# SheffieldML/GPy

Hardware: AMD Instinct MI355X
Metric: exact-GP log_lik+grad iters/sec (higher is better)
Workload: dtype f64; 1 GPU; BASELINE configs[2]: matern52 ARD exact GP, one GPRegression.parameters_changed, N=16384 D=32 Dy=1 per GPU; N=16384, D=32, kernel=matern52, ARD=True, parallelism=replicas x1

## Files before the change

gpy_amd/_lib.py:

```python
import ctypes
import os
import subprocess

import numpy as np
from numpy.ctypeslib import ndpointer

_HERE = os.path.dirname(os.path.abspath(__file__))
LIB_PATH = os.environ.get("MI355GP_LIB") or os.path.join(_HERE, "libmi355gp.so")
CSRC = os.path.join(_HERE, "csrc")

KIND_IDS = {"rbf": 0, "matern52": 1, "matern32": 2, "exponential": 3, "white": 4, "bias": 5, "ratquad": 6, "stdperiodic": 7,
            "coregionalize": 8, "linear": 9, "mlp": 10, "poly": 11}


def ard_id(kind, ARD):
    if kind == "coregionalize":
        return int(ARD)
    return int(ARD) & 3 if kind == "stdperiodic" else int(bool(ARD))


class Part(ctypes.Structure):
    _fields_ = [("kind", ctypes.c_int), ("ard", ctypes.c_int), ("n_active", ctypes.c_int),
                ("active_dims", ctypes.POINTER(ctypes.c_int)), ("theta", ctypes.POINTER(ctypes.c_double)),
                ("term", ctypes.c_int)]


def make_parts(specs):
    arr = (Part * len(specs))()
    keep, ntheta = [], 0
    for i, spec in enumerate(specs):
        kind, ARD, theta, dims = spec[:4]
        arr[i].term = int(spec[4]) if len(spec) > 4 else 0
        th = np.ascontiguousarray(theta, dtype=np.float64)
        keep.append(th)
        arr[i].kind = KIND_IDS[kind]
        arr[i].ard = ard_id(kind, ARD)
        arr[i].theta = th.ctypes.data_as(ctypes.POINTER(ctypes.c_double))
        if dims is None:
            arr[i].n_active = 0
            arr[i].active_dims = None
        else:
            d = np.ascontiguousarray(dims, dtype=np.int32)
            keep.append(d)
            arr[i].n_active = d.size
            arr[i].active_dims = d.ctypes.data_as(ctypes.POINTER(ctypes.c_int))
        ntheta += th.size
    return arr, keep, ntheta
FETCH_L, FETCH_KINV, FETCH_DLDK, FETCH_K = 0, 1, 2, 3
EP_BERNOULLI_PROBIT = 0
OUT_LML, OUT_LOGDET, OUT_DATAFIT, OUT_DNOISE, OUT_TRKINV, NUM_OUT = 0, 1, 2, 3, 4, 8
STAGE_NAMES = ("kbuild", "potrf", "trtri", "lauum", "solve", "grad", "total")
NUM_T = 8
PROFILE_FAMILIES = ("update_nt", "trtri", "lauum", "diag128", "trsm128", "update_nt64", "potrf_persist", "trtri_early")

_lib = None


class MI355GPError(RuntimeError):
    pass


DIAG_LIB_PATH = os.path.join(_HERE, "libmi355gp_diag.so")


def build(force=False):
    srcs = [os.path.join(CSRC, f) for f in os.listdir(CSRC) if f.endswith((".hip", ".h")) or f == "Makefile"]
    srcs.append(os.path.join(_HERE, "..", "include", "mi355gp.h"))
    srcs.append(os.path.join(_HERE, "..", "include", "mi355gp_debug.h"))
    product = os.path.join(_HERE, "libmi355gp.so")
    if not force and os.path.exists(product) and os.path.exists(DIAG_LIB_PATH):
        t = min(os.path.getmtime(product), os.path.getmtime(DIAG_LIB_PATH))
        if all(os.path.getmtime(s) <= t for s in srcs if os.path.exists(s)):
            return product
    r = subprocess.run(["make", "-C", CSRC, "-j8", "all", "diag"], capture_output=True, text=True)
    if r.returncode != 0 or not os.path.exists(product) or not os.path.exists(DIAG_LIB_PATH):
        raise MI355GPError("building libmi355gp.so failed:\n" + r.stdout[-4000:] + r.stderr[-4000:])
    return product


_dp = ndpointer(dtype=np.float64, flags="C_CONTIGUOUS")
_c_dp = ctypes.POINTER(ctypes.c_double)


def _opt(a):
    return None if a is None else a.ctypes.data_as(_c_dp)


def lib():
    global _lib
    if _lib is not None:
        return _lib
    if not os.path.exists(LIB_PATH):
        build()
    L = ctypes.CDLL(LIB_PATH)
    i64, ci, cd, vp = ctypes.c_int64, ctypes.c_int, ctypes.c_double, ctypes.c_void_p
    L.mi355gp_last_error.restype = ctypes.c_char_p
    L.mi355gp_version.restype = ctypes.c_char_p
    L.mi355gp_device_count.argtypes = [ctypes.POINTER(ci)]
    L.mi355gp_device_synchronize.argtypes = [ci]
    L.mi355gp_create.argtypes = [ci, ctypes.POINTER(vp)]
    L.mi355gp_destroy.argtypes = [vp]
    L.mi355gp_set_data.argtypes = [vp, _dp, i64, ci, _dp, ci]
    L.mi355gp_set_targets.argtypes = [vp, _dp, ci]
    L.mi355gp_kern_K.argtypes = [ci, ci, ci, _dp, _dp, i64, _c_dp, i64, ci, _dp]
    L.mi355gp_kern_Kdiag.argtypes = [ci, _dp, i64, _dp]
    L.mi355gp_update_gradients_full.argtypes = [ci, ci, ci, _dp, _dp, _dp, i64, _c_dp, i64, ci, _dp]
    L.mi355gp_gradients_X.argtypes = [ci, ci, ci, _dp, _dp, _dp, i64, _c_dp, i64, ci, _dp]
    L.mi355gp_exact_inference.argtypes = [vp, ci, ci, _dp, _dp, i64, cd, cd, _dp, _c_dp, _c_dp, _c_dp, _c_dp]
    L.mi355gp_exact_inference_sum.argtypes = [vp, ci, ctypes.POINTER(Part), _dp, i64, cd, cd, _dp, _c_dp, _c_dp, _c_dp,
                                              _c_dp]
    L.mi355gp_exact_studentt_sum.argtypes = [vp, ci, ctypes.POINTER(Part), cd, cd, cd, _dp, _c_dp, _c_dp, _c_dp]
    L.mi355gp_covariance_between_points.argtypes = [vp, ci, ctypes.POINTER(Part), _dp, i64, _dp, i64, _dp]
    L.mi355gp_predictive_gradients_sum.argtypes = [vp, ci, ctypes.POINTER(Part), _dp, i64, _c_dp, _c_dp]
    L.mi355gp_predict_sum.argtypes = [vp, ci, ctypes.POINTER(Part), _dp, i64, _c_dp, _c_dp, ci]
    L.mi355gp_laplace_begin.argtypes = [vp, ci, ctypes.POINTER(Part)]
    L.mi355gp_laplace_newton.argtypes = [vp, _dp, _dp, cd, _dp, _dp, _c_dp]
    L.mi355gp_laplace_finish.argtypes = [vp, _dp, cd, _dp, _c_dp]
    L.mi355gp_laplace_gradients.argtypes = [vp, _dp, _dp, _dp]
    L.mi355gp_laplace_implicit.argtypes = [vp, _dp, _dp]
    L.mi355gp_laplace_predict.argtypes = [vp, ci, ctypes.POINTER(Part), _dp, i64, _dp, _c_dp, _c_dp, ci]
    L.mi355gp_ep_recompute.argtypes = [vp, _dp, _dp, cd, cd, ci, _dp, _dp, _c_dp, _c_dp]
    L.mi355gp_ep_sweep.argtypes = [vp, ci, ndpointer(dtype=np.int64, flags="C_CONTIGUOUS"), _dp, cd, cd, _dp, _dp, _dp, _dp, _dp, _dp,
                                   _dp, _c_dp]
    L.mi355gp_inference_given_K.argtypes = [vp, _dp, _dp, i64, cd, cd, _dp, _c_dp, _c_dp, _c_dp]
    L.mi355gp_fetch.argtypes = [vp, ci, _dp, ci]
    L.mi355gp_predict.argtypes = [vp, ci, ci, _dp, _dp, i64, _c_dp, _c_dp, ci]
    L.mi355gp_potrf.argtypes = [ci, _dp, i64, _c_dp]
    L.mi355gp_pdinv.argtypes = [ci, _dp, i64, _c_dp, _c_dp, _c_dp, _c_dp]
    L.mi355gp_pdinv_full.argtypes = [ci, _dp, i64, _c_dp, _c_dp, _c_dp, _c_dp, _c_dp]
    L.mi355gp_set_option.argtypes = [vp, ci, ci]
    L.mi355gp_get_option.argtypes = [vp, ci, ctypes.POINTER(ci)]
    L.mi355gp_sparse_get_profile.argtypes = [vp, _dp]
    L.mi355gp_dbg_comm_selftest.argtypes = [ci, ctypes.c_char_p, ci, ci, ci, ci, i64, ci, _dp]
    L.mi355gp_dbg_comm_selftest.restype = ci
    L.mi355gp_bench_factor.argtypes = [ci, i64, ci, _c_dp, _c_dp, _c_dp]
    L.mi355gp_bench_factor.restype = ci
    L.mi355gp_get_profile.argtypes = [vp, _dp, _dp, ndpointer(dtype=np.int32, flags="C_CONTIGUOUS")]
    L.mi355gp_grid_unique_id.argtypes = [ctypes.c_char_p]
    L.mi355gp_grid_create.argtypes = [ci, ci, ci, ci, ci, ci, ctypes.c_char_p, ctypes.POINTER(vp)]
    L.mi355gp_grid_destroy.argtypes = [vp]
    L.mi355gp_grid_set_data.argtypes = [vp, _dp, i64, ci, _dp, ci]
    L.mi355gp_grid_exact_inference.argtypes = [vp, ci, ci, _dp, _dp, i64, cd, cd, _dp, _c_dp, _c_dp, _c_dp, _c_dp]
    L.mi355gp_grid_fetch.argtypes = [vp, ci, _dp]
    L.mi355gp_grid_set_option.argtypes = [vp, ci, ci]
    L.mi355gp_grid_coll_log.argtypes = [vp, ci, _dp]
    L.mi355gp_grid_coll_log.restype = ci
    L.mi355gp_dbg_grid_multi.argtypes = [ci, ci, ci, ci, _dp]
    L.mi355gp_dbg_update_nt.argtypes = [ci, ci, ctypes.POINTER(ci), ci, ci, _dp]
    L.mi355gp_dbg_update_rect.argtypes = [ci, ci, ci, ctypes.POINTER(ci), ci, ci, _dp]
    L.mi355gp_grid_get_option.argtypes = [vp, ci, ctypes.POINTER(ci)]
    L.mi355gp_sparse_create.argtypes = [ci, ctypes.POINTER(vp)]
    L.mi355gp_sparse_destroy.argtypes = [vp]
    L.mi355gp_sparse_set_data.argtypes = [vp, _dp, i64, ci, _dp, ci]
    L.mi355gp_vardtc_inference.argtypes = [vp, ci, ci, _dp, _dp, i64, cd, cd, _dp, _c_dp, _c_dp, _c_dp, _c_dp]
    L.mi355gp_sparse_fetch.argtypes = [vp, ci, _dp]
    L.mi355gp_vardtc_inference_sum.argtypes = [vp, ci, ctypes.POINTER(Part), _dp, i64, _dp, i64, cd, _dp, _c_dp, _c_dp, _c_dp,
                                               _c_dp, _c_dp, _c_dp]
    L.mi355gp_sparse_set_input_variance.argtypes = [vp, _dp, i64, ci]
    L.mi355gp_vardtc_inference_uncertain.argtypes = [vp, ci, ctypes.POINTER(Part), _dp, i64, _dp, i64, cd, _dp, _c_dp, _c_dp,
                                                     _c_dp, _c_dp, _c_dp, _c_dp]
    L.mi355gp_sparse_predict.argtypes = [vp, ci, ctypes.POINTER(Part), _dp, i64, _c_dp, _c_dp, ci]
    L.mi355gp_sparse_fetch_dLdKnm.argtypes = [vp, i64, i64, _dp]
    L.mi355gp_sparse_attach_loopback.argtypes = [vp, ci, ci, ci]
    L.mi355gp_sparse_attach_comm.argtypes = [vp, ci, ci, ctypes.c_char_p]
    L.mi355gp_rbf_psi.argtypes = [ci, cd, _dp, ci, _dp, i64, _dp, _dp, i64, ci, _c_dp, _c_dp, _c_dp]
    L.mi355gp_rbf_psi_grad.argtypes = [ci, cd, _dp, ci, _dp, i64, _dp, _dp, i64, ci, _c_dp, _c_dp, _c_dp, _c_dp, _dp, _dp, _dp,
                                       _dp, _dp]
    L.mi355gp_dbg_mfma.argtypes = [ci, _dp, _dp, _dp]
    L.mi355gp_dbg_gemm.argtypes = [ci, ci, ci, i64, i64, i64, _dp, _dp, _dp, cd, cd, ci, _c_dp]
    L.mi355gp_dbg_peaks.argtypes = [ci, _dp]
    L.mi355gp_dbg_pipe_share.argtypes = [ci, _dp]
    L.mi355gp_dbg_graph_factor.argtypes = [ci, i64, ci, _dp]
    L.mi355gp_dbg_gemm_clock.argtypes = [_c_dp, _c_dp]
    L.mi355gp_dbg_mask_probe.argtypes = [ci, ci, ci, _dp]
    L.mi355gp_dbg_lauum_plan.argtypes = [ci, ctypes.POINTER(ci), ci, ctypes.POINTER(ci)]
    L.mi355gp_dbg_lauum_plan.restype = ci
    L.mi355gp_dbg_persist_owners.argtypes = [ci, ci, ci, ctypes.POINTER(ci), ctypes.POINTER(ci)]
    L.mi355gp_dbg_persist_owners.restype = ci
    L.mi355gp_dbg_persist.argtypes = [ci, i64, ci, ci, _dp]
    L.mi355gp_dbg_ipc_selftest.argtypes = [ctypes.c_char_p, ci, ci, ci, ci, i64, _dp]
    for name in ("device_count", "create", "destroy", "set_data", "set_targets", "kern_K", "kern_Kdiag",
                 "update_gradients_full", "exact_inference", "inference_given_K", "fetch", "predict", "potrf",
                 "pdinv", "dbg_mfma", "dbg_gemm", "dbg_peaks", "set_option", "get_profile", "grid_unique_id",
                 "grid_create", "grid_destroy", "grid_set_data", "grid_exact_inference", "grid_fetch", "grid_set_option",
                 "grid_get_option", "sparse_create",
                 "sparse_destroy", "sparse_set_data", "vardtc_inference", "sparse_fetch", "gradients_X", "sparse_attach_comm", "exact_inference_sum",
                 "predict_sum", "dbg_gemm_clock", "covariance_between_points", "exact_studentt_sum", "dbg_mask_probe",
                 "vardtc_inference_sum", "sparse_predict", "sparse_fetch_dLdKnm", "sparse_attach_loopback",
                 "predictive_gradients_sum", "dbg_pipe_share", "pdinv_full", "dbg_graph_factor", "get_option",
                 "sparse_get_profile", "dbg_persist", "dbg_grid_multi", "dbg_update_nt", "dbg_update_rect",
                 "dbg_ipc_selftest", "laplace_begin", "laplace_newton", "laplace_finish", "laplace_gradients",
                 "laplace_implicit", "laplace_predict", "ep_recompute", "ep_sweep", "rbf_psi", "rbf_psi_grad",
                 "sparse_set_input_variance", "vardtc_inference_uncertain"):
        getattr(L, "mi355gp_" + name).restype = ci
    _lib = L
    return L


EXPORTED = ("mi355gp_last_error", "mi355gp_version", "mi355gp_device_count", "mi355gp_device_synchronize", "mi355gp_create", "mi355gp_destroy",
            "mi355gp_set_data", "mi355gp_set_targets", "mi355gp_kern_K", "mi355gp_kern_Kdiag",
            "mi355gp_update_gradients_full", "mi355gp_exact_inference", "mi355gp_inference_given_K",
            "mi355gp_fetch", "mi355gp_predict", "mi355gp_potrf", "mi355gp_pdinv", "mi355gp_bench_factor",
            "mi355gp_set_option", "mi355gp_get_profile", "mi355gp_grid_unique_id", "mi355gp_grid_create",
            "mi355gp_grid_destroy", "mi355gp_grid_set_data", "mi355gp_grid_exact_inference", "mi355gp_grid_fetch",
            "mi355gp_grid_set_option", "mi355gp_grid_get_option",
            "mi355gp_sparse_create", "mi355gp_sparse_destroy", "mi355gp_sparse_set_data", "mi355gp_vardtc_inference",
            "mi355gp_sparse_fetch", "mi355gp_gradients_X", "mi355gp_sparse_attach_comm",
            "mi355gp_exact_inference_sum", "mi355gp_predict_sum", "mi355gp_dbg_gemm_clock",
            "mi355gp_covariance_between_points", "mi355gp_exact_studentt_sum", "mi355gp_vardtc_inference_sum",
            "mi355gp_sparse_predict", "mi355gp_sparse_fetch_dLdKnm", "mi355gp_sparse_attach_loopback",
            "mi355gp_predictive_gradients_sum", "mi355gp_dbg_pipe_share", "mi355gp_pdinv_full", "mi355gp_dbg_graph_factor",
            "mi355gp_dbg_mfma", "mi355gp_dbg_gemm", "mi355gp_dbg_peaks", "mi355gp_dbg_mask_probe", "mi355gp_get_option",
            "mi355gp_sparse_get_profile", "mi355gp_dbg_persist", "mi355gp_dbg_grid_multi", "mi355gp_dbg_update_nt", "mi355gp_dbg_update_rect",
            "mi355gp_dbg_ipc_selftest", "mi355gp_grid_coll_log", "mi355gp_dbg_lauum_plan", "mi355gp_dbg_persist_owners",
            "mi355gp_laplace_begin", "mi355gp_laplace_newton", "mi355gp_laplace_finish", "mi355gp_laplace_gradients",
            "mi355gp_laplace_implicit", "mi355gp_laplace_predict", "mi355gp_ep_recompute", "mi355gp_ep_sweep",
            "mi355gp_rbf_psi", "mi355gp_rbf_psi_grad", "mi355gp_sparse_set_input_variance",
            "mi355gp_vardtc_inference_uncertain")


OPTIONS = {"profile": 0, "lookahead": 1, "tri_overlap": 2, "tri_min_nt": 3, "tri_h": 4, "tri_wgs": 5, "tri_half": 6,
           "part1_on_panel": 7, "nbo": 8, "solve_overlap": 9, "diag_excl_first": 10, "graph": 11, "persist": 12, "agg2": 13,
           "persist_test": 14, "persist_aborts": 15, "persist_skip": 16, "persist_sched": 17}


def last_error():
    return lib().mi355gp_last_error().decode()


def check(rc, what):
    if rc < 0:
        raise MI355GPError("%s failed (rc=%d): %s" % (what, rc, last_error()))
    return rc


def device_count():
    n = ctypes.c_int(0)
    lib().mi355gp_device_count(ctypes.byref(n))
    return n.value


def device_synchronize(device=0):
    require_device(device)
    check(lib().mi355gp_device_synchronize(int(device)), "mi355gp_device_synchronize")


def require_device(device=0):
    n = device_count()
    if device >= n:
        raise MI355GPError("no MI355X visible to HIP (device %d requested, %d present): the gpy_amd backend has "
                           "no CPU fallback" % (device, n))


def f64(a):
    return np.ascontiguousarray(a, dtype=np.float64)


def theta_vec(variance, lengthscale, ARD, D):
    ls = np.atleast_1d(np.asarray(lengthscale, dtype=np.float64)).ravel()
    if ARD:
        if ls.size == 1:
            ls = np.full(D, ls[0])
        assert ls.size == D, "ARD kernel needs one lengthscale per input dimension"
    else:
        assert ls.size == 1, "isotropic kernel has a single lengthscale"
    return np.concatenate([[float(np.asarray(variance).ravel()[0])], ls])


def _exact_result(out, ms, **arrays):
    res = dict(lml=out[OUT_LML], logdet=out[OUT_LOGDET], datafit=out[OUT_DATAFIT], dnoise=out[OUT_DNOISE],
               trKinv=out[OUT_TRKINV], **arrays)
    if ms is not None:
        res["stage_ms"] = dict(zip(STAGE_NAMES, ms[:len(STAGE_NAMES)]))
    return res


def _predict(entry, head, Xnew, D, Dy, full_cov, want_var, between=()):
    Xnew = f64(Xnew)
    M = Xnew.shape[0]
    assert Xnew.shape[1] == D
    mu = np.empty((M, Dy))
    var = (np.empty((M, M)) if full_cov else np.empty(M)) if want_var else None
    check(getattr(lib(), entry)(*(tuple(head) + (Xnew, M) + tuple(between) + (mu.ctypes.data_as(_c_dp), _opt(var),
                                                                              int(bool(full_cov))))), entry)
    if var is not None and not full_cov:
        var = var[:, None]
    return mu, var


class Context(object):

    def __init__(self, device=0):
        require_device(device)
        self._h = ctypes.c_void_p()
        check(lib().mi355gp_create(device, ctypes.byref(self._h)), "mi355gp_create")
        self.device = device
        self.N = self.D = self.Dy = 0

    def close(self):
        if getattr(self, "_h", None) is not None and self._h.value:
            lib().mi355gp_destroy(self._h)
            self._h = ctypes.c_void_p()

    def __del__(self):
        try:
            self.close()
        except Exception:
            pass

    def set_data(self, X, R):
        X, R = f64(X), f64(R)
        assert X.ndim == 2 and R.ndim == 2 and X.shape[0] == R.shape[0]
        self.N, self.D = X.shape
        self.Dy = R.shape[1]
        check(lib().mi355gp_set_data(self._h, X, self.N, self.D, R, self.Dy), "mi355gp_set_data")

    def set_targets(self, R):
        R = f64(R)
        check(lib().mi355gp_set_targets(self._h, R, R.shape[1]), "mi355gp_set_targets")

    def _exact(self, entry, head, ntheta, noise, jitter, extra_jitter, want_alpha, want_diag, want_stage_ms):
        noise = f64(np.atleast_1d(noise))
        out = np.zeros(NUM_OUT)
        alpha = np.empty((self.N, self.Dy)) if want_alpha else None
        dtheta = np.zeros(ntheta)
        diag = np.empty(self.N) if want_diag else None
        ms = np.zeros(NUM_T) if want_stage_ms else None
        rc = check(getattr(lib(), entry)(self._h, *(tuple(head) + (noise, noise.size, jitter, extra_jitter, out, _opt(alpha),
                                                                   _opt(dtheta), _opt(diag), _opt(ms)))), entry)
        return rc, _exact_result(out, ms, alpha=alpha, dtheta=dtheta, diag_dL_dK=diag)

    def exact_inference(self, kind, ARD, theta, noise, jitter=1e-8, extra_jitter=0.0, want_alpha=True,
                        want_diag=False, want_stage_ms=False):
        theta = f64(theta)
        return self._exact("mi355gp_exact_inference", (KIND_IDS[kind], ard_id(kind, ARD), theta), theta.size, noise, jitter,
                           extra_jitter, want_alpha, want_diag, want_stage_ms)

    def exact_inference_sum(self, specs, noise, jitter=1e-8, extra_jitter=0.0, want_alpha=True, want_diag=False,
                            want_stage_ms=False):
        arr, keep, ntheta = make_parts(specs)
        return self._exact("mi355gp_exact_inference_sum", (len(specs), arr), ntheta, noise, jitter, extra_jitter, want_alpha,
                           want_diag, want_stage_ms)

    def predict_sum(self, specs, Xnew, full_cov=False, want_var=True):
        arr, keep, _ = make_parts(specs)
        return _predict("mi355gp_predict_sum", (self._h, len(specs), arr), Xnew, self.D, self.Dy, full_cov, want_var)

    def exact_studentt_sum(self, specs, nu, jitter=1e-8, extra_jitter=0.0):
        arr, keep, ntheta = make_parts(specs)
        out = np.zeros(NUM_OUT)
        alpha = np.empty((self.N, self.Dy))
        dtheta = np.zeros(ntheta)
        rc = check(lib().mi355gp_exact_studentt_sum(self._h, len(specs), arr, float(nu), jitter, extra_jitter, out,
                                                    _opt(alpha), _opt(dtheta), None), "mi355gp_exact_studentt_sum")
        return rc, dict(lml=out[OUT_LML], logdet=out[OUT_LOGDET], beta=out[OUT_DATAFIT], scale=out[5], alpha=alpha,
                        dtheta=dtheta)

    def predictive_gradients(self, specs, Xnew, want_var=True):
        arr, keep, _ = make_parts(specs)
        Xnew = f64(Xnew)
        M = Xnew.shape[0]
        assert Xnew.shape[1] == self.D
        dmu = np.empty((M, self.D, self.Dy))
        dvar = np.empty((M, self.D)) if want_var else None
        check(lib().mi355gp_predictive_gradients_sum(self._h, len(specs), arr, Xnew, M, dmu.ctypes.data_as(_c_dp), _opt(dvar)),
              "mi355gp_predictive_gradients_sum")
        return dmu, dvar

    def covariance_between_points(self, specs, X1, X2):
        arr, keep, _ = make_parts(specs)
        X1, X2 = f64(X1), f64(X2)
        out = np.empty((X1.shape[0], X2.shape[0]))
        check(lib().mi355gp_covariance_between_points(self._h, len(specs), arr, X1, X1.shape[0], X2, X2.shape[0], out),
              "mi355gp_covariance_between_points")
        return out

# ... 254 lines not shown
    if X2 is None:
        M, p2 = N, None
    else:
        X2 = f64(X2)
        M, p2 = X2.shape[0], X2.ctypes.data_as(_c_dp)
    G = f64(dL_dK)
    assert G.shape == (N, M), "dL_dK must be N x M"
    theta = f64(theta)
    out = np.zeros(theta.size)
    check(lib().mi355gp_update_gradients_full(device, KIND_IDS[kind], ard_id(kind, ARD), theta, G, X, N, p2, M, D, out),
          "mi355gp_update_gradients_full")
    return out


def gradients_X(kind, ARD, theta, dL_dK, X, X2=None, device=0):
    require_device(device)
    X = f64(X)
    N, D = X.shape
    if X2 is None:
        M, p2 = N, None
    else:
        X2 = f64(X2)
        M, p2 = X2.shape[0], X2.ctypes.data_as(_c_dp)
    G = f64(dL_dK)
    assert G.shape == (N, M), "dL_dK must be N x M"
    out = np.zeros((N, D))
    check(lib().mi355gp_gradients_X(device, KIND_IDS[kind], ard_id(kind, ARD), f64(theta), G, X, N, p2, M, D, out),
          "mi355gp_gradients_X")
    return out


def _psi_args(variance, lengthscale, ARD, Z, mu, S, weights):
    Z, mu, S = f64(Z), f64(mu), f64(S)
    N, D = mu.shape
    assert S.shape == mu.shape and Z.ndim == 2 and Z.shape[1] == D, "Z is M x D, mu and S are N x D"
    ls = theta_vec(variance, lengthscale, ARD, D)[1:]
    w = None if weights is None else f64(np.ravel(weights))
    assert w is None or w.size == N
    return (float(np.ravel(variance)[0]), f64(ls), int(bool(ARD)), Z, Z.shape[0], mu, S, N, D, _opt(w)), w


def rbf_psi(variance, lengthscale, ARD, Z, mu, S, weights=None, want_psi1=True, want_psi2=True, device=0):
    require_device(device)
    args, keep = _psi_args(variance, lengthscale, ARD, Z, mu, S, weights)
    M, N = args[4], args[7]
    p1 = np.empty((N, M)) if want_psi1 else None
    p2 = np.empty((M, M)) if want_psi2 else None
    check(lib().mi355gp_rbf_psi(device, *(args + (_opt(p1), _opt(p2)))), "mi355gp_rbf_psi")
    return p1, p2


def rbf_psi_grad(variance, lengthscale, ARD, Z, mu, S, dL_dpsi0=None, dL_dpsi1=None, dL_dpsi2=None, weights=None, device=0):
    require_device(device)
    args, keep = _psi_args(variance, lengthscale, ARD, Z, mu, S, weights)
    M, N, D = args[4], args[7], args[8]
    d0 = None if dL_dpsi0 is None else f64(np.ravel(dL_dpsi0))
    d1 = None if dL_dpsi1 is None else f64(dL_dpsi1)
    d2 = None if dL_dpsi2 is None else f64(dL_dpsi2)
    assert d0 is None or d0.size == N
    assert d1 is None or d1.shape == (N, M), "dL_dpsi1 must be N x M"
    assert d2 is None or d2.shape == (M, M), "dL_dpsi2 must be M x M"
    dvar, dl = np.zeros(1), np.zeros(D if ARD else 1)
    dZ, dmu, dS = np.zeros((M, D)), np.zeros((N, D)), np.zeros((N, D))
    check(lib().mi355gp_rbf_psi_grad(device, *(args + (_opt(d0), _opt(d1), _opt(d2), dvar, dl, dZ, dmu, dS))),
          "mi355gp_rbf_psi_grad")
    return dvar[0], dl, dZ, dmu, dS


def potrf(A, device=0):
    require_device(device)
    L = f64(A).copy()
    ms = ctypes.c_double(0.0)
    info = check(lib().mi355gp_potrf(device, L, L.shape[0], ctypes.byref(ms)), "mi355gp_potrf")
    return L, info, ms.value


def pdinv(A, device=0):
    require_device(device)
    A = f64(A)
    n = A.shape[0]
    Ai, L = np.empty((n, n)), np.empty((n, n))
    ld, ms = ctypes.c_double(0.0), ctypes.c_double(0.0)
    info = check(lib().mi355gp_pdinv(device, A, n, Ai.ctypes.data_as(_c_dp), L.ctypes.data_as(_c_dp),
                                     ctypes.byref(ld), ctypes.byref(ms)), "mi355gp_pdinv")
    return Ai, L, ld.value, info, ms.value


def pdinv_full(A, device=0):
    require_device(device)
    A = f64(A)
    n = A.shape[0]
    Ai, L, Li = np.empty((n, n)), np.empty((n, n)), np.empty((n, n))
    ld, ms = ctypes.c_double(0.0), ctypes.c_double(0.0)
    info = check(lib().mi355gp_pdinv_full(device, A, n, Ai.ctypes.data_as(_c_dp), L.ctypes.data_as(_c_dp),
                                          Li.ctypes.data_as(_c_dp), ctypes.byref(ld), ctypes.byref(ms)), "mi355gp_pdinv_full")
    return Ai, L, Li, ld.value, info


def bench_factor(N, reps=3, device=0):
    require_device(device)
    p, t, l = ctypes.c_double(0.0), ctypes.c_double(0.0), ctypes.c_double(0.0)
    check(lib().mi355gp_bench_factor(device, N, reps, ctypes.byref(p), ctypes.byref(t), ctypes.byref(l)),
          "mi355gp_bench_factor")
    fl = float(N) ** 3 / 3.0
    return {"potrf_ms": p.value, "trtri_ms": t.value, "lauum_ms": l.value,
            "potrf_tflops": fl / p.value / 1e9, "trtri_tflops": fl / t.value / 1e9, "lauum_tflops": fl / l.value / 1e9}


def dbg_persist(N, reps=3, kcap=0, device=0):
    require_device(device)
    nt = (int(N) + 127) // 128
    out = np.zeros(8 + 32 * nt)
    check(lib().mi355gp_dbg_persist(device, int(N), int(reps), int(kcap), out), "mi355gp_dbg_persist")
    st = out[8:8 + 8 * nt].reshape(nt, 8)
    near = out[8 + 8 * nt:8 + 20 * nt].reshape(nt, 3, 4)
    far = out[8 + 20 * nt:].reshape(nt, 12)
    return dict(ms_steps=out[0], ms_persist=out[1], mismatches=int(out[2]), info=int(out[3]), abort=int(out[4]), nt=nt,
                steps=(st - st[0, 0]) / 100.0, near=(near - st[0, 0]) / 100.0, far=(far - st[0, 0]) / 100.0)


def dbg_mask_probe(pct=75, order=0, device=0):
    require_device(device)
    out = np.zeros(3)
    check(lib().mi355gp_dbg_mask_probe(device, pct, order, out), "mi355gp_dbg_mask_probe")
    return out


def dbg_mfma(a, b, device=0):
    require_device(device)
    d = np.zeros(256)
    check(lib().mi355gp_dbg_mfma(device, f64(a), f64(b), d), "dbg_mfma")
    return d.reshape(64, 4)


def dbg_gemm(A, B, C, a_mcontig, b_ncontig, alpha=1.0, beta=0.0, reps=0, device=0):
    require_device(device)
    A, B, C = f64(A), f64(B), f64(C).copy()
    M, K = (A.shape[1], A.shape[0]) if a_mcontig else A.shape
    N = B.shape[1] if b_ncontig else B.shape[0]
    ms = ctypes.c_double(0.0)
    check(lib().mi355gp_dbg_gemm(device, int(a_mcontig), int(b_ncontig), M, N, K, A, B, C, alpha, beta, reps,
                                 ctypes.byref(ms)), "dbg_gemm")
    return C, ms.value


def dbg_gemm_clock():
    mhz, cyc = ctypes.c_double(0.0), ctypes.c_double(0.0)
    check(lib().mi355gp_dbg_gemm_clock(ctypes.byref(mhz), ctypes.byref(cyc)), "dbg_gemm_clock")
    return mhz.value, cyc.value


def dbg_peaks(device=0):
    require_device(device)
    out = np.zeros(8)
    check(lib().mi355gp_dbg_peaks(device, out), "dbg_peaks")
    return dict(mfma_f64_tflops=out[0], valu_f64_tflops=out[1], hbm_copy_gbs=out[2], hbm_fill_gbs=out[3],
                mfma_cycles_per_inst_1wave=out[4], shader_mhz_under_load=out[5], mfma_1wave_tflops=out[6],
                mfma_cycles_per_inst_loaded=out[7])


def dbg_grid_multi(T, nb=512, reps=3, device=0):
    require_device(device)
    out = np.zeros(5)
    check(lib().mi355gp_dbg_grid_multi(device, int(T), int(nb), int(reps), out), "mi355gp_dbg_grid_multi")
    return out


def dbg_update_nt(nt, ks, reps=5, device=0):
    require_device(device)
    ka = (ctypes.c_int * len(ks))(*[int(k) for k in ks])
    out = np.zeros(len(ks))
    check(lib().mi355gp_dbg_update_nt(device, int(nt), ka, len(ks), int(reps), out), "mi355gp_dbg_update_nt")
    return out


def dbg_update_rect(ntr, ntc, ks, reps=5, device=0):
    require_device(device)
    ka = (ctypes.c_int * len(ks))(*[int(k) for k in ks])
    out = np.zeros(len(ks))
    check(lib().mi355gp_dbg_update_rect(device, int(ntr), int(ntc), ka, len(ks), int(reps), out), "mi355gp_dbg_update_rect")
    return out


def persist_owners(nt, nw, tune=0):
    owner = (ctypes.c_int * (nt * nt))()
    out4 = (ctypes.c_int * 4)()
    dup = lib().mi355gp_dbg_persist_owners(nt, nw, tune, owner, out4)
    return np.frombuffer(owner, dtype=np.int32, count=nt * nt).reshape(nt, nt).copy(), out4[0], out4[1], out4[2], out4[3], dup


def lauum_plan(nt):
    out4 = (ctypes.c_int * 4)()
    lib().mi355gp_dbg_lauum_plan(nt, None, 0, out4)
    n = out4[0]
    buf = (ctypes.c_int * (6 * max(n, 1)))()
    check(lib().mi355gp_dbg_lauum_plan(nt, buf, n, out4), "mi355gp_dbg_lauum_plan")
    return np.frombuffer(buf, dtype=np.int32, count=6 * n).reshape(n, 6).copy(), out4[1], out4[2], out4[3]
```

gpy_amd/csrc/api.hip:

```cpp
#include <functional>
#include <algorithm>
#include <cmath>
#include <cstdarg>
#include <cstdio>
#include <climits>
#include <cstring>
#include <string>
#include <vector>

#include "../../include/mi355gp.h"
#include "../../include/mi355gp_debug.h"
#include "internal.h"
#include "parts.h"

int run_peaks(int device, double* out4);

static thread_local std::string g_err;

void mi355gp_set_error(const char* fmt, ...) {
    char buf[1024];
    va_list ap;
    va_start(ap, fmt);
    vsnprintf(buf, sizeof(buf), fmt, ap);
    va_end(ap);
    g_err = buf;
}

#define LOG_2_PI 1.8378770664093454836

#include "ctx.h"

static void apply_options(mi355gp_ctx* c) {
    FactorWs& w = c->ws;
    auto set = [&](int o, int* field) { if (c->opt[o] != INT_MIN) *field = c->opt[o]; };
    set(MI355GP_OPT_LOOKAHEAD, &w.lookahead);
    set(MI355GP_OPT_TRI_OVERLAP, &w.tri_overlap);
    set(MI355GP_OPT_TRI_MIN_NT, &w.tri_min_nt);
    set(MI355GP_OPT_TRI_H, &w.tri_h_override);
    set(MI355GP_OPT_TRI_WGS, &w.tri_wgs);
    set(MI355GP_OPT_TRI_HALF, &w.tri_half_ok);
    set(MI355GP_OPT_PART1_ON_PANEL, &w.part1_on_panel);
    set(MI355GP_OPT_NBO, &w.nbo_override);
    set(MI355GP_OPT_SOLVE_OVERLAP, &w.solve_overlap);
    set(MI355GP_OPT_DIAG_EXCL_FIRST, &w.diag_excl_first);
    set(MI355GP_OPT_PERSIST, &w.persist);
    set(MI355GP_OPT_AGG2, &w.agg2);
    if (c->opt[MI355GP_OPT_GRAPH] != INT_MIN) c->graph_enabled = c->opt[MI355GP_OPT_GRAPH] ? 1 : 0;
}

static void drop_graph(mi355gp_ctx* c) {
    if (c->fgraph) (void)hipGraphExecDestroy(c->fgraph);
    c->fgraph = nullptr;
    c->fgraph_calls = 0;
}

static void free_data(mi355gp_ctx* c) {
    drop_graph(c);
    c->parts.clear();
    double** ptrs[] = {&c->dX, &c->dR, &c->dNoise, &c->A, &c->B, &c->C, &c->Mbuf,
                       &c->dTmp, &c->dTrmvPart, &c->dGradPart, &c->dGradOut, &c->dPack, &c->dCoregPart};
    for (auto p : ptrs) {
        if (*p) (void)hipFree(*p);
        *p = nullptr;
    }
    if (c->hPack) (void)hipHostFree(c->hPack);
    c->hPack = nullptr;
    c->dAlpha = c->dScal = c->dDiag = c->dGradOutAll = nullptr;
    c->hIdx.clear();
    c->hIdxCol = -1;
    laplace_session_free(c->lap);
    c->lap = nullptr;
    c->lap_stage = 0;
    factor_ws_free(&c->ws);
    c->have_factor = c->have_kernel = false;
}

extern "C" {

const char* mi355gp_last_error(void) { return g_err.c_str(); }
const char* mi355gp_version(void) { return "mi355gp 0.1 (gfx950)"; }

int mi355gp_device_synchronize(int device) {
    HIP_CHECK(hipSetDevice(device));
    HIP_CHECK(hipDeviceSynchronize());
    return 0;
}

int mi355gp_device_count(int* count) {
    int n = 0;
    hipError_t e = hipGetDeviceCount(&n);
    if (e != hipSuccess) {
        (void)hipGetLastError();
        n = 0;
    }
    *count = n;
    return 0;
}

int mi355gp_create(int device, mi355gp_ctx** out) {
    int n = 0;
    mi355gp_device_count(&n);
    if (device < 0 || device >= n) {
        mi355gp_set_error("mi355gp_create: device %d not available (%d HIP devices visible)", device, n);
        return -2;
    }
    HIP_CHECK(hipSetDevice(device));
    mi355gp_ctx* c = new mi355gp_ctx();
    c->device = device;
    for (int& o : c->opt) o = INT_MIN;
    if (factor_engine(device, &c->st, nullptr, nullptr) != 0) return -2;
    for (auto& e : c->ev) HIP_CHECK(hipEventCreate(&e));
    {
        const char* e = PRODUCT_ENV("GRAPH");
        if (e && *e) c->graph_enabled = atoi(e) ? 1 : 0;
    }
    *out = c;
    return 0;
}

int mi355gp_destroy(mi355gp_ctx* c) {
    if (!c) return 0;
    (void)hipSetDevice(c->device);
    (void)hipStreamSynchronize(c->st);
    free_data(c);
    for (auto& e : c->ev)
        if (e) (void)hipEventDestroy(e);
    if (c->st) (void)hipStreamSynchronize(c->st);
    delete c;
    return 0;
}

int mi355gp_set_data(mi355gp_ctx* c, const double* X, int64_t N, int D, const double* R, int Dy) {
    ARG_CHECK(c && X && R && N > 0 && D > 0 && Dy > 0, "mi355gp_set_data: bad arguments");
    HIP_CHECK(hipSetDevice(c->device));
    EngineShared gate(c->device);
    HIP_CHECK(hipStreamSynchronize(c->st));
    free_data(c);
    c->n = N;
    c->npad = round_up(N, NB);
    c->D = D;
    c->Dy = Dy;
    const long np = c->npad;
    HIP_CHECK(hipMalloc(&c->dX, sizeof(double) * N * D));
    HIP_CHECK(hipMalloc(&c->dR, sizeof(double) * N * Dy));
    HIP_CHECK(hipMalloc(&c->dNoise, sizeof(double) * N));
    HIP_CHECK(hipMalloc(&c->A, sizeof(double) * np * np));
    HIP_CHECK(hipMalloc(&c->B, sizeof(double) * np * np));
    HIP_CHECK(hipMalloc(&c->C, sizeof(double) * np * np));
    if (factor_ws_alloc(&c->ws, np) != 0) return -3;
    c->ws.can_calibrate = 1;
    {
        const int lookahead = c->ws.lookahead;
        const char* e = PRODUCT_ENV("GRAPH");
        c->graph_enabled = (e && *e) ? (atoi(e) ? 1 : 0) : 1;
        apply_options(c);
        if (c->opt[MI355GP_OPT_LOOKAHEAD] == INT_MIN) c->ws.lookahead = lookahead;
    }
    HIP_CHECK(hipMalloc(&c->dTmp, sizeof(double) * N * Dy));
    const long nchunks = (N + trmv_chunk_rows(N) - 1) / trmv_chunk_rows(N);
    HIP_CHECK(hipMalloc(&c->dTrmvPart, sizeof(double) * nchunks * N * Dy));
    const int groups = (D + 31) / 32;
    c->gradPartDoubles = 2L * groups * 2048 * GP_STRIDE;
    HIP_CHECK(hipMalloc(&c->dGradPart, sizeof(double) * c->gradPartDoubles));
    HIP_CHECK(hipMalloc(&c->dGradOut, sizeof(double) * groups * GP_STRIDE));
    c->offGrad = 8;
    c->offExt = c->offGrad + (size_t)16 * groups * GP_STRIDE;
    c->offAlpha = c->offExt + (size_t)16 * groups * GP_STRIDE;
    c->offDiag = c->offAlpha + (size_t)N * Dy;
    c->offCoreg = c->offDiag + (size_t)N;
    c->packDoubles = c->offCoreg + (size_t)16 * COREG_REC;
    HIP_CHECK(hipMalloc(&c->dPack, sizeof(double) * c->packDoubles));
    HIP_CHECK(hipHostMalloc(&c->hPack, sizeof(double) * c->packDoubles, hipHostMallocDefault));
    c->dScal = c->dPack;
    c->dGradOutAll = c->dPack + c->offGrad;
    c->dAlpha = c->dPack + c->offAlpha;
    c->dDiag = c->dPack + c->offDiag;
    HIP_CHECK(hipMemcpy(c->dX, X, sizeof(double) * N * D, hipMemcpyHostToDevice));
    HIP_CHECK(hipMemcpy(c->dR, R, sizeof(double) * N * Dy, hipMemcpyHostToDevice));
    return 0;
}

int mi355gp_set_targets(mi355gp_ctx* c, const double* R, int Dy) {
    ARG_CHECK(c && R && c->n > 0 && Dy == c->Dy, "mi355gp_set_targets: set_data first / Dy mismatch");
    HIP_CHECK(hipSetDevice(c->device));
    EngineShared gate(c->device);
    HIP_CHECK(hipStreamSynchronize(c->st));
    HIP_CHECK(hipMemcpy(c->dR, R, sizeof(double) * c->n * Dy, hipMemcpyHostToDevice));
    return 0;
}

}

static int run_pipeline(mi355gp_ctx* c, EngineShared* gate, bool with_kernel_grads, double* out_scalars, double* alpha_out,
                        double* dtheta_out, double* diag_out, double* stage_ms,
                        const std::function<int()>& rebuild, double studentt_nu = 0.0, int attempt = 0) {
    hipStream_t st = c->st;
    const long n = c->n, np = c->npad;
    c->lap_stage = 0;
    c->ws.prof.reset();
// ... 754 lines not shown
    HIP_CHECK(dPart.alloc(2 * 2048 * GP_STRIDE * ((D + 31) / 32)));
    HIP_CHECK(dCol.alloc(64 * mp * (D + 1)));
    HIP_CHECK(dHX.alloc(mp * (D + 1)));
    if (dvar_out) {
        HIP_CHECK(hipMemsetAsync(dU, 0, sizeof(double) * np * mp, st));
        emit_cross(st, c->parts, c->terms, training_points(c), xs, dU, mp, nullptr, true, 0);
        launch_trmm_lower(st, c->B, np, dU, mp, dT, mp, (int)(np / NB), (int)(mp / NB));
        launch_trmm_lower_T(st, c->B, np, dT, mp, dU, mp, (int)(np / NB), (int)(mp / NB));
    }
    const size_t hx = (size_t)M * (D + 1);
    std::vector<double> HX(hx);
    const int npass = (dmu_out ? (int)Dy : 0) + (dvar_out ? 1 : 0);
    if (dmu_out) std::fill(dmu_out, dmu_out + (size_t)M * D * Dy, 0.0);
    if (dvar_out) std::fill(dvar_out, dvar_out + (size_t)M * D, 0.0);
    for (int pass = 0; pass < npass; ++pass) {
        const bool is_var = dvar_out && pass == npass - 1;
        const double* W = dU;
        if (!is_var) {
            const long cnt = n * M;
            hipLaunchKernelGGL(k_fill_rows, dim3((unsigned)((cnt + 255) / 256)), dim3(256), 0, st, (double*)dG, mp, n, (long)M,
                               c->dAlpha + pass, (int)Dy);
            W = dG;
        }
        auto add = [&](long m, int q, double g) {
            if (is_var) dvar_out[m * D + q] += -2.0 * g;
            else dmu_out[((size_t)m * D + q) * Dy + pass] += g;
        };
        for (size_t pi = 0; pi < c->parts.size(); ++pi) {
            const mi355gp_ctx::Part& pt = c->parts[pi];
            if (pt.is_static()) continue;
            if (pt.linear()) {
                const int ns = launch_colreduce_multi(st, W, mp, n, M, pt.dXt, 1, np, (int)D, 0, dCol);
                launch_sum_splits(st, dCol, (long)M * D, ns, 0, dHX);
                HIP_CHECK(hipMemcpyAsync(HX.data(), dHX, sizeof(double) * M * D, hipMemcpyDeviceToHost, st));
                HIP_CHECK(hipStreamSynchronize(st));
                gradx_linear(pt.inv_ls, M, (int)D, HX.data(), add);
                if (is_var)
                    for (long m = 0; m < M; ++m)
                        for (size_t a = 0; a < pt.dims.size(); ++a)
                            dvar_out[m * D + pt.dims[a]] += 2.0 * pt.theta[pt.kp.ard ? a : 0] * Xnew[m * D + pt.dims[a]];
                continue;
            }
            const double* xt = xs.points(st, pt);
            if (pt.kp.kind == MI355GP_STDPERIODIC) {
                launch_periodic_gradx(st, pt.kp, xt, xs.ld, M, pt.dXt, np, n, W, mp, 1, dHX);
                HIP_CHECK(hipMemcpyAsync(HX.data(), dHX, sizeof(double) * M * D, hipMemcpyDeviceToHost, st));
                HIP_CHECK(hipStreamSynchronize(st));
                gradx_periodic(pt.pw, M, (int)D, HX.data(), add);
                continue;
            }
            launch_grad_generic(st, pt.kp, pt.dXt, np, n, xt, xs.ld, M, 0, W, mp, dPart, GP_STRIDE, dH, mp);
            const int ns = launch_colreduce_multi(st, dH, mp, n, M, pt.dXt, 1, np, (int)D, 1, dCol);
            launch_sum_splits(st, dCol, (long)hx, ns, 0, dHX);
            HIP_CHECK(hipMemcpyAsync(HX.data(), dHX, sizeof(double) * hx, hipMemcpyDeviceToHost, st));
            HIP_CHECK(hipStreamSynchronize(st));
            if (pt.mlp()) {
                gradx_mlp(Xnew, M, (int)D, pt.inv_ls, pt.kp.bias, HX.data(), add);
                if (is_var)
                    for (long m = 0; m < M; ++m) {
                        const double cd = mlp_dkdiag_factor(pt, Xnew + m * D);
                        for (size_t a = 0; a < pt.dims.size(); ++a)
                            dvar_out[m * D + pt.dims[a]] += 2.0 * cd * pt.theta[1 + (pt.kp.ard ? a : 0)] * Xnew[m * D + pt.dims[a]];
                    }
                continue;
            }
            gradx_stationary(Xnew, M, (int)D, pt.inv_ls, HX.data(), add);
        }
    }
    HIP_CHECK(hipStreamSynchronize(st));
    HIP_CHECK(hipGetLastError());
    return 0;
}

int mi355gp_covariance_between_points(mi355gp_ctx* c, int nparts, const mi355gp_part* parts, const double* X1,
                                      int64_t M1, const double* X2, int64_t M2, double* out) {
    ARG_CHECK(c && c->n > 0 && c->have_factor, "mi355gp_covariance_between_points: run an inference call first");
    ARG_CHECK(X1 && X2 && M1 > 0 && M2 > 0 && out, "mi355gp_covariance_between_points: bad arguments");
    HIP_CHECK(hipSetDevice(c->device));
    EngineShared gate(c->device);
    if (int rc = prepare_parts(c, nparts, parts)) return rc;
    if (int rc = coreg_check_points(c, X1, M1, "X1")) return rc;
    if (int rc = coreg_check_points(c, X2, M2, "X2")) return rc;
    hipStream_t st = c->st;
    const long np = c->npad, m1p = round_up(M1, NB), m2p = round_up(M2, NB);
    c->have_kernel = true;
    scale_parts(c);
    PointSet x1, x2;
    DevBuf dK1, dK2, dT1, dT2, dC;
    if (int rc = x1.load(st, X1, M1, c->D)) return rc;
    if (int rc = x2.load(st, X2, M2, c->D)) return rc;
    HIP_CHECK(dK1.alloc(np * m1p));
    HIP_CHECK(dK2.alloc(np * m2p));
    HIP_CHECK(dT1.alloc(np * m1p));
    HIP_CHECK(dT2.alloc(np * m2p));
    HIP_CHECK(dC.alloc(m1p * m2p));
    HIP_CHECK(hipMemsetAsync(dK1, 0, sizeof(double) * np * m1p, st));
    HIP_CHECK(hipMemsetAsync(dK2, 0, sizeof(double) * np * m2p, st));
    HIP_CHECK(hipMemsetAsync(dC, 0, sizeof(double) * m1p * m2p, st));
    DevBuf dS1, dS2, dS3;
    if (has_product(c->terms)) {
        HIP_CHECK(dS1.alloc(np * m1p));
        HIP_CHECK(dS2.alloc(np * m2p));
        HIP_CHECK(dS3.alloc(m1p * m2p));
    }
    emit_cross(st, c->parts, c->terms, training_points(c), x1, dK1, m1p, dS1, true, 0);
    emit_cross(st, c->parts, c->terms, training_points(c), x2, dK2, m2p, dS2, true, 0);
    emit_cross(st, c->parts, c->terms, x1, x2, dC, m2p, dS3, true, 0);
    launch_trmm_lower(st, c->B, np, dK1, m1p, dT1, m1p, (int)(np / NB), (int)(m1p / NB));
    launch_trmm_lower(st, c->B, np, dK2, m2p, dT2, m2p, (int)(np / NB), (int)(m2p / NB));
    launch_gemm(st, 1, 1, m1p, m2p, np, dT1, m1p, dT2, m2p, dC, m2p, -1.0, 1.0);
    HIP_CHECK(hipMemcpy2DAsync(out, sizeof(double) * M2, dC, sizeof(double) * m2p, sizeof(double) * M2, M1,
                               hipMemcpyDeviceToHost, st));
    HIP_CHECK(hipStreamSynchronize(st));
    HIP_CHECK(hipGetLastError());
    return 0;
}

int mi355gp_predict(mi355gp_ctx* c, int kind, int ard, const double* theta, const double* Xnew, int64_t M,
                    double* mu_out, double* var_out, int full_cov) {
    if (int rc = check_kind(kind, KS_STATIONARY | KS_EXT | KS_LINEAR | KS_DOT, "mi355gp_predict")) return rc;
    const mi355gp_part part{kind, ard, 0, nullptr, theta};
    return mi355gp_predict_sum(c, 1, &part, Xnew, M, mu_out, var_out, full_cov);
}

int mi355gp_set_option(mi355gp_ctx* c, int option, int value) {
    ARG_CHECK(c != nullptr, "mi355gp_set_option: NULL context");
    if (option == MI355GP_OPT_PROFILE) {
        c->ws.prof.on = (value != 0);
        c->ws.prof.mask = (value == 1) ? 0xffu : (unsigned)value >> 1;
        return 0;
    }
    if (option == MI355GP_OPT_PERSIST_TEST) {
#ifndef MI355GP_DIAG
        if (value != 0) {
            mi355gp_set_error("mi355gp_set_option: MI355GP_OPT_PERSIST_TEST is a test hook of the diagnostics build (libmi355gp_diag.so)");
            return -1;
        }
#endif
        c->ws.persist_test = value;
        if (value) c->ws.persist_skip = 0;
        drop_graph(c);
        return 0;
    }
    if (option < 0 || option >= MI355GP_OPT_NUM || option == MI355GP_OPT_PERSIST_ABORTS || option == MI355GP_OPT_PERSIST_SKIP ||
        option == MI355GP_OPT_PERSIST_SCHED) {
        mi355gp_set_error("mi355gp_set_option: unknown or read-only option %d", option);
        return -1;
    }
    if (option == MI355GP_OPT_LOOKAHEAD) value = (value == 0) ? 0 : 1;
    if (option == MI355GP_OPT_NBO && value > 0 && value % NB != 0) {
        mi355gp_set_error("mi355gp_set_option: NBO must be a multiple of %d", NB);
        return -1;
    }
    c->opt[option] = (value < 0) ? INT_MIN : value;
    if (value < 0) {
        FactorWs d;
#define env(name, dflt) diag_env_int(DIAG_ENV(name), dflt)
#define penv(name, dflt) diag_env_int(PRODUCT_ENV(name), dflt)
        switch (option) {
            case MI355GP_OPT_LOOKAHEAD: c->ws.lookahead = d.lookahead; break;
            case MI355GP_OPT_TRI_OVERLAP: c->ws.tri_overlap = penv("TRI_OVERLAP", d.tri_overlap) ? 1 : 0; break;
            case MI355GP_OPT_TRI_MIN_NT: c->ws.tri_min_nt = env("TRI_MIN_NT", d.tri_min_nt); break;
            case MI355GP_OPT_TRI_H: c->ws.tri_h_override = env("TRI_H", d.tri_h_override); break;
            case MI355GP_OPT_TRI_WGS: c->ws.tri_wgs = env("TRI_WGS", d.tri_wgs); break;
            case MI355GP_OPT_TRI_HALF: c->ws.tri_half_ok = env("TRI_HALF", d.tri_half_ok) ? 1 : 0; break;
            case MI355GP_OPT_PART1_ON_PANEL: c->ws.part1_on_panel = env("PART1_ON_PANEL", d.part1_on_panel) ? 1 : 0; break;
            case MI355GP_OPT_NBO: c->ws.nbo_override = env("NBO", d.nbo_override); break;
            case MI355GP_OPT_SOLVE_OVERLAP: c->ws.solve_overlap = env("SOLVE_OVERLAP", d.solve_overlap) ? 1 : 0; break;
            case MI355GP_OPT_DIAG_EXCL_FIRST: c->ws.diag_excl_first = env("DIAG_EXCL_FIRST", d.diag_excl_first) ? 1 : 0; break;
            case MI355GP_OPT_PERSIST: c->ws.persist = penv("PERSIST", d.persist); break;
            case MI355GP_OPT_AGG2: c->ws.agg2 = env("AGG2", d.agg2) ? 1 : 0; break;
            case MI355GP_OPT_GRAPH: c->graph_enabled = penv("GRAPH", 1) ? 1 : 0; break;
            default: break;
        }
#undef env
#undef penv
    }
    if (option == MI355GP_OPT_PERSIST) {
        c->ws.persist_auto_off = 0;
        c->ws.sched_force_steps = 0;
        c->ws.sched_np = c->ws.sched_ns = 0;
        c->ws.sched_state = (value < 0) ? 0 : 2;
    }
    apply_options(c);
    drop_graph(c);
    return 0;
}

int mi355gp_get_option(mi355gp_ctx* c, int option, int* value) {
    ARG_CHECK(c && value && option > MI355GP_OPT_PROFILE && option < MI355GP_OPT_NUM, "mi355gp_get_option: bad arguments");
    const FactorWs& w = c->ws;
    const int v[MI355GP_OPT_NUM] = {0, w.lookahead, w.tri_overlap, w.tri_min_nt, w.tri_h_override, w.tri_wgs, w.tri_half_ok,
                                    w.part1_on_panel, w.nbo_override, w.solve_overlap, w.diag_excl_first, c->graph_enabled,
                                    w.persist, w.agg2, w.persist_test, w.persist_aborts, w.persist_skip,
                                    w.sched_state == 2 ? ((w.persist_auto_off || !w.persist) ? 2 : 1) : 0};
    *value = v[option];
    return 0;
}

int mi355gp_get_profile(mi355gp_ctx* c, double* ms, double* flops, int* launches) {
    ARG_CHECK(c && ms && flops && launches, "mi355gp_get_profile: NULL argument");
    HIP_CHECK(hipSetDevice(c->device));
    HIP_CHECK(hipStreamSynchronize(c->st));
    if (c->ws.st_panel) HIP_CHECK(hipStreamSynchronize(c->ws.st_panel));
    if (c->ws.prof.collect(ms, flops, launches) != 0) {
        mi355gp_set_error("mi355gp_get_profile: event timing failed");
        return -5;
    }
    return 0;
}

int mi355gp_bench_factor(int device, int64_t N, int reps, double* ms_potrf, double* ms_trtri, double* ms_lauum) {
    ARG_CHECK(N >= NB && reps >= 1 && ms_potrf && ms_trtri && ms_lauum, "mi355gp_bench_factor: N >= 128, reps >= 1");
    HIP_CHECK(hipSetDevice(device));
    const long np = round_up(N, NB);
    const int D = 4;
    std::vector<double> X((size_t)N * D);
    unsigned long long state = 0x9E3779B97F4A7C15ull;
    for (double& v : X) {
        state = state * 6364136223846793005ull + 1442695040888963407ull;
        v = ((double)(state >> 11) / 9007199254740992.0 - 0.5) * 4.0;
    }
    DevBuf dX, dXt, dIl, dNoise, A, B, C;
    HIP_CHECK(dX.alloc(N * D));
    HIP_CHECK(dXt.alloc(D * np));
    HIP_CHECK(dIl.alloc(D));
    HIP_CHECK(dNoise.alloc(1));
    HIP_CHECK(A.alloc(np * np));
    HIP_CHECK(B.alloc(np * np));
    HIP_CHECK(C.alloc(np * np));
    const double il[4] = {0.7, 0.7, 0.7, 0.7}, noise = 0.1;
    HIP_CHECK(hipMemcpy(dX, X.data(), sizeof(double) * N * D, hipMemcpyHostToDevice));
    HIP_CHECK(hipMemcpy(dIl, il, sizeof(il), hipMemcpyHostToDevice));
    HIP_CHECK(hipMemcpy(dNoise, &noise, sizeof(double), hipMemcpyHostToDevice));
    hipStream_t st;
    if (factor_engine(device, &st, nullptr, nullptr) != 0) return -2;
    FactorWs ws;
    if (factor_ws_alloc(&ws, np) != 0) return -3;
    ws.scratchX = B;
    ws.scratchT = C;
    hipEvent_t e[4];
    for (auto& ev : e) HIP_CHECK(hipEventCreate(&ev));
    const KernParams kp{MI355GP_RBF, 0, D, 1.0};
    launch_scale_inputs(st, dX, N, D, dIl, 0, dXt, np);
    double acc[3] = {0.0, 0.0, 0.0};
    int info = 0, first_info = 0, redone = 0;
    for (int r = -1; r < reps; ++r) {
        launch_kbuild_sym(st, kp, dXt, np, N, np, A, dNoise, 1, 1e-8, 1, 1);
        HIP_CHECK(hipEventRecord(e[0], st));
        potrf_device(st, A, np, &ws);
        HIP_CHECK(hipEventRecord(e[1], st));
        trtri_device(st, A, B, C, np, &ws);
        HIP_CHECK(hipEventRecord(e[2], st));
        lauum_device(st, B, C, np, &ws);
        HIP_CHECK(hipEventRecord(e[3], st));
        HIP_CHECK(hipStreamSynchronize(st));
        HIP_CHECK(hipMemcpy(&info, ws.info, sizeof(int), hipMemcpyDeviceToHost));
        bool clean = false;
        if (potrf_persist_aborted(info, &ws, &clean)) {
            if (++redone > reps + 2) {
                mi355gp_set_error("mi355gp_bench_factor: the persistent launch kept being called off");
                for (auto& ev : e) (void)hipEventDestroy(ev);
                factor_ws_free(&ws);
                return -6;
            }
            --r;
            continue;
        }
        if (info > 0 && first_info == 0) first_info = info;
        if (r < 0) continue;
        for (int i = 0; i < 3; ++i) {
            float ms;
            HIP_CHECK(hipEventElapsedTime(&ms, e[i], e[i + 1]));
            acc[i] += ms;
        }
    }
    info = first_info;
    *ms_potrf = acc[0] / reps;
    *ms_trtri = acc[1] / reps;
    *ms_lauum = acc[2] / reps;
    for (auto& ev : e) (void)hipEventDestroy(ev);
    factor_ws_free(&ws);
    HIP_CHECK(hipGetLastError());
    return info > 0 ? info : 0;
}

__global__ void k_count_lower_mismatch(const double* __restrict__ a, const double* __restrict__ b, long n, long ld,
                                       unsigned long long* __restrict__ count) {
    unsigned long long c = 0;
    for (long idx = (long)blockIdx.x * blockDim.x + threadIdx.x; idx < n * n; idx += (long)gridDim.x * blockDim.x) {
        const long i = idx / n, j = idx - i * n;
        if (j <= i && __double_as_longlong(a[i * ld + j]) != __double_as_longlong(b[i * ld + j])) ++c;
    }
    if (c) atomicAdd(count, c);
}

int mi355gp_dbg_persist(int device, int64_t N, int reps, int kcap, double* out) {
    ARG_CHECK(N >= 2 * NB && reps >= 1 && out, "mi355gp_dbg_persist: N >= 256, reps >= 1");
    HIP_CHECK(hipSetDevice(device));
    const long np = round_up(N, NB);
    const int nt = (int)(np / NB), D = 4;
    std::vector<double> X((size_t)N * D);
    unsigned long long state = 0x9E3779B97F4A7C15ull;
    for (double& v : X) {
        state = state * 6364136223846793005ull + 1442695040888963407ull;
        v = ((double)(state >> 11) / 9007199254740992.0 - 0.5) * 4.0;
    }
    DevBuf dX, dXt, dIl, dNoise, A, B, dStamp, dCount;
    HIP_CHECK(dX.alloc(N * D));
    HIP_CHECK(dXt.alloc(D * np));
    HIP_CHECK(dIl.alloc(D));
    HIP_CHECK(dNoise.alloc(1));
    HIP_CHECK(A.alloc(np * np));
    HIP_CHECK(B.alloc(np * np));
    HIP_CHECK(dStamp.alloc(32 * nt));
    HIP_CHECK(dCount.alloc(1));
    const double il[4] = {0.7, 0.7, 0.7, 0.7}, noise = 0.1;
    HIP_CHECK(hipMemcpy(dX, X.data(), sizeof(double) * N * D, hipMemcpyHostToDevice));
    HIP_CHECK(hipMemcpy(dIl, il, sizeof(il), hipMemcpyHostToDevice));
    HIP_CHECK(hipMemcpy(dNoise, &noise, sizeof(double), hipMemcpyHostToDevice));
    HIP_CHECK(hipMemset(dStamp, 0, sizeof(double) * 32 * nt));
    HIP_CHECK(hipMemset(dCount, 0, sizeof(double)));
    hipStream_t st;
    if (factor_engine(device, &st, nullptr, nullptr) != 0) return -2;
    EngineShared gate(device);
    FactorWs ws;
    if (factor_ws_alloc(&ws, np) != 0) return -3;
    ws.tri_overlap = 0;
    if (kcap > 0) ws.persist_kcap = kcap;
    ws.persist_max_nt = 64;
    hipEvent_t e[2];
    ws.persist = 1;
    for (auto& ev : e) HIP_CHECK(hipEventCreate(&ev));
    const KernParams kp{MI355GP_RBF, 0, D, 1.0};
    launch_scale_inputs(st, dX, N, D, dIl, 0, dXt, np);
    for (int i = 0; i < 8 + 32 * nt; ++i) out[i] = 0.0;
    int info[4] = {0, 0, 0, 0};
    for (int mode = 0; mode < 2; ++mode) {
        double* M = mode == 0 ? (double*)B : (double*)A;
        ws.persist = mode;
        if (mode == 1 && !potrf_persist_eligible(np, &ws)) {
            mi355gp_set_error("mi355gp_dbg_persist: N = %ld is not eligible for the persistent factorisation", (long)N);
            for (auto& ev : e) (void)hipEventDestroy(ev);
            factor_ws_free(&ws);
            return -1;
        }
        double acc = 0.0;
        for (int r = -1; r < reps; ++r) {
// ... 284 lines not shown
```

gpy_amd/csrc/common.h:

```cpp
#pragma once
#include <hip/hip_runtime.h>
#include <stdint.h>

typedef double d4 __attribute__((ext_vector_type(4)));
typedef double d2 __attribute__((ext_vector_type(2)));

#define NB 128
#define NBO 512
#define FACTOR_NBO_SMALL_N 0
#define FACTOR_NBO_SMALL 256
#define FACTOR_DEFAULT_TRI_OVERLAP 1
#define FACTOR_DEFAULT_PERSIST 1
#define FACTOR_PERSIST_MAX_NT 64
#define PS_ABORT_INFO (1 << 30)
#define PS_ABORT_CLEAN ((1 << 30) + 1)
#define PS_SKIP_AFTER_CLEAN 16
#define FACTOR_DEFAULT_DIAG_EXCL_FIRST 1
#define GEMM_DEFAULT_TRI64_MAX 512
#define GEMM_DEFAULT_LAUUM64_MAX 528
#define LAUUM_SPLIT_MAX_NT 44
#define GEMM_DEFAULT_UPD64_MAX 128

__device__ __forceinline__ d4 mfma_f64(double a, double b, d4 c) {
    return __builtin_amdgcn_mfma_f64_16x16x4f64(a, b, c, 0, 0, 0);
}

void mi355gp_set_error(const char* fmt, ...);
#define HIP_CHECK(expr)                                                                          \
    do {                                                                                         \
        hipError_t _e = (expr);                                                                  \
        if (_e != hipSuccess) {                                                                  \
            mi355gp_set_error("%s failed: %s (%s:%d)", #expr, hipGetErrorString(_e), __FILE__,  \
                              __LINE__);                                                         \
            return -(1000 + (int)_e);                                                            \
        }                                                                                        \
    } while (0)
#define ARG_CHECK(cond, msg)              \
    do {                                  \
        if (!(cond)) {                    \
            mi355gp_set_error("%s", msg); \
            return -1;                    \
        }                                 \
    } while (0)

struct DevBuf {
    double* p = nullptr;
    DevBuf() = default;
    DevBuf(DevBuf&& o) noexcept : p(o.p) { o.p = nullptr; }
    DevBuf(const DevBuf&) = delete;
    DevBuf& operator=(const DevBuf&) = delete;
    ~DevBuf() {
        if (p) (void)hipFree(p);
    }
    hipError_t alloc(size_t doubles) { return hipMalloc(&p, sizeof(double) * (doubles ? doubles : 1)); }
    operator double*() const { return p; }
};

static inline int64_t round_up(int64_t n, int64_t m) { return (n + m - 1) / m * m; }

#include <cstdlib>
#define PRODUCT_ENV(name) getenv("MI355GP_" name)
#ifdef MI355GP_DIAG
#define DIAG_ENV(name) getenv("MI355GP_" name)
#else
#define DIAG_ENV(name) ((const char*)nullptr)
#endif
static inline int diag_env_int(const char* v, int dflt) { return (v && *v) ? atoi(v) : dflt; }
```

gpy_amd/csrc/factor.hip:

```cpp
#include <cstdlib>
#include <mutex>
#include <vector>

#include "internal.h"

void KernelProf::begin(hipStream_t st, int fam, double flops) {
    open = on && ((mask >> fam) & 1u);
    if (!open) return;
    const size_t e0 = 2 * recs.size();
    while (pool.size() < e0 + 2) {
        hipEvent_t e;
        (void)hipEventCreate(&e);
        pool.push_back(e);
    }
    recs.push_back(Rec{fam, flops, e0});
    (void)hipEventRecord(pool[e0], st);
}

void KernelProf::end(hipStream_t st) {
    if (!open) return;
    open = false;
    (void)hipEventRecord(pool[recs.back().e0 + 1], st);
}

int KernelProf::collect(double* ms, double* flops, int* launches) {
    for (int f = 0; f < PF_NUM; ++f) { ms[f] = 0.0; flops[f] = 0.0; launches[f] = 0; }
    for (const Rec& r : recs) {
        float t = 0.f;
        if (hipEventElapsedTime(&t, pool[r.e0], pool[r.e0 + 1]) != hipSuccess) return -1;
        ms[r.fam] += t;
        flops[r.fam] += r.flops;
        launches[r.fam] += 1;
    }
    return 0;
}

void KernelProf::destroy() {
    for (hipEvent_t e : pool) (void)hipEventDestroy(e);
    pool.clear();
    recs.clear();
}

struct FactorEngine {
    hipStream_t main = nullptr, panel = nullptr, tri = nullptr, tri_half = nullptr;
    int tri_pct = 0;
    bool ready = false;
};
static FactorEngine g_engine[16];
static std::mutex g_engine_mutex;
static std::shared_mutex g_engine_gate[16];
std::shared_mutex& engine_gate(int device) { return g_engine_gate[device & 15]; }

int factor_engine(int device, hipStream_t* main, hipStream_t* panel, hipStream_t* tri, hipStream_t* tri_half) {
    if (device < 0 || device >= 16) return -1;
    std::lock_guard<std::mutex> lock(g_engine_mutex);
    FactorEngine& e = g_engine[device];
    if (!e.ready) {
        int least = 0, greatest = 0;
        HIP_CHECK(hipDeviceGetStreamPriorityRange(&least, &greatest));
        HIP_CHECK(hipStreamCreateWithFlags(&e.main, hipStreamNonBlocking));
        HIP_CHECK(hipStreamCreateWithPriority(&e.panel, hipStreamNonBlocking, greatest));
        const char* envc = DIAG_ENV("TRI_CU_PCT");
        e.tri_pct = (envc && *envc) ? atoi(envc) : 75;
        hipDeviceProp_t prop;
        HIP_CHECK(hipGetDeviceProperties(&prop, device));
        const int ncu = prop.multiProcessorCount, nx = 8;
        if (e.tri_pct > 0 && e.tri_pct < 100 && ncu % nx == 0) {
            const int per = ncu / nx, keep = (per * e.tri_pct + 50) / 100;
            std::vector<uint32_t> mask((size_t)(ncu + 31) / 32, 0u);
            const char* envm = DIAG_ENV("TRI_MASK_MODE");
            const int mode = (envm && *envm) ? atoi(envm) : 0;
            for (int cu = 0; cu < ncu; ++cu) {
                const int idx = cu / nx;
                bool on = idx < keep;
                if (mode == 1) on = (idx % 4) != 3;
                if (mode == 2) on = idx >= per - keep;
                if (on) mask[cu / 32] |= 1u << (cu % 32);
            }
            if (hipExtStreamCreateWithCUMask(&e.tri, (uint32_t)mask.size(), mask.data()) != hipSuccess) {
                (void)hipGetLastError();
                e.tri = nullptr;
            }
        }
        if (!e.tri) HIP_CHECK(hipStreamCreateWithPriority(&e.tri, hipStreamNonBlocking, least));
        if (ncu % nx == 0) {
            const int per = ncu / nx, keep = per / 2;
            std::vector<uint32_t> mask((size_t)(ncu + 31) / 32, 0u);
            for (int cu = 0; cu < ncu; ++cu)
                if (cu / nx < keep) mask[cu / 32] |= 1u << (cu % 32);
            if (hipExtStreamCreateWithCUMask(&e.tri_half, (uint32_t)mask.size(), mask.data()) != hipSuccess) {
                (void)hipGetLastError();
                e.tri_half = nullptr;
            }
        }
        {
            void* touch = nullptr;
            if (hipMalloc(&touch, 256) == hipSuccess) {
                hipStream_t order[4] = {e.main, e.panel, e.tri, e.tri_half};
                for (hipStream_t s : order)
                    if (s) {
                        (void)hipMemsetAsync(touch, 0, 256, s);
                        (void)hipStreamSynchronize(s);
                    }
                (void)hipFree(touch);
            }
        }
        e.ready = true;
    }
    if (main) *main = e.main;
    if (panel) *panel = e.panel;
    if (tri) *tri = e.tri;
    if (tri_half) *tri_half = e.tri_half;
    return 0;
}

static bool lauum_plan_wanted(const FactorWs* ws, int nt);
static bool lauum_plan_build(FactorWs* ws, int nt);
int factor_ws_alloc(FactorWs* ws, long npad) {
    ws->nblk = npad / NB;
    HIP_CHECK(hipMalloc(&ws->dinv, sizeof(double) * ws->nblk * 8 * 256));
    HIP_CHECK(hipMalloc(&ws->logsum, sizeof(double) * ws->nblk));
    HIP_CHECK(hipMalloc(&ws->info, sizeof(int) * 4));
    int least = 0, greatest = 0;
    HIP_CHECK(hipDeviceGetStreamPriorityRange(&least, &greatest));
    int dev = 0;
    HIP_CHECK(hipGetDevice(&dev));
    if (factor_engine(dev, nullptr, &ws->st_panel, &ws->st_tri, &ws->st_tri_half) != 0) return -1;
    {
        const char* envo = PRODUCT_ENV("TRI_OVERLAP");
        if (envo && *envo) ws->tri_overlap = atoi(envo) ? 1 : 0;
        const char* envn2 = DIAG_ENV("TRI_MIN_NT");
        if (envn2 && *envn2) ws->tri_min_nt = atoi(envn2);
        const char* envw2 = DIAG_ENV("TRI_WGS");
        if (envw2 && *envw2) ws->tri_wgs = atoi(envw2);
        ws->tri_cu_pct = g_engine[dev].tri_pct > 0 && g_engine[dev].tri_pct <= 100 ? g_engine[dev].tri_pct : 75;
        HIP_CHECK(hipEventCreateWithFlags(&ws->ev_tri, hipEventDisableTiming));
        HIP_CHECK(hipEventCreateWithFlags(&ws->ev_tri_lead, hipEventDisableTiming));
        HIP_CHECK(hipMalloc(&ws->tri_counter, sizeof(int) * 4));
        const char* envh = DIAG_ENV("TRI_H");
        if (envh && *envh) ws->tri_h_override = atoi(envh);
    }
    const char* envp1 = DIAG_ENV("PART1_ON_PANEL");
    if (envp1 && *envp1) ws->part1_on_panel = atoi(envp1) ? 1 : 0;
    ws->sched_state = ws->sched_force_steps = ws->persist_auto_off = 0;
    ws->sched_np = ws->sched_ns = 0;
    ws->evals_done = ws->early_pending = 0;
    const char* envpa = PRODUCT_ENV("PERSIST_AUTO");
    if (envpa && *envpa) ws->persist_auto = atoi(envpa) ? 1 : 0;
    const char* envls = DIAG_ENV("LAUUM_SPLIT");
    if (envls && *envls) ws->lauum_split = atoi(envls) > 0 ? atoi(envls) : 0;
    const char* envptri = DIAG_ENV("PERSIST_TRI");
    if (envptri && *envptri) ws->persist_tri = atoi(envptri) ? 1 : 0;
    const char* envptn = DIAG_ENV("PERSIST_TRI_MIN_NT");
    if (envptn && *envptn) ws->persist_tri_min_nt = atoi(envptn);
#ifdef MI355GP_DIAG
    const char* envuq = DIAG_ENV("DBG_UPD_QUEUE");
    if (envuq && *envuq && atoi(envuq)) {
        ws->upd_queue_probe = 1;
        HIP_CHECK(hipMalloc(&ws->upd_tasks, sizeof(UpdTask) * 64 + 64));
    }
#endif
    const char* envag = DIAG_ENV("AGG2");
    if (envag && *envag) ws->agg2 = atoi(envag) ? 1 : 0;
    const char* envnbo = DIAG_ENV("NBO");
    if (envnbo && *envnbo) ws->nbo_override = atoi(envnbo);
    const char* envso = DIAG_ENV("SOLVE_OVERLAP");
    if (envso && *envso) ws->solve_overlap = atoi(envso) ? 1 : 0;
    const char* envth = DIAG_ENV("TRI_HALF");
    if (envth && *envth) ws->tri_half_ok = atoi(envth) ? 1 : 0;
    const char* envps = PRODUCT_ENV("PERSIST");
    if (envps && *envps) ws->persist = atoi(envps);
    const char* envpm = DIAG_ENV("PERSIST_MAX_NT");
    if (envpm && *envpm) ws->persist_max_nt = atoi(envpm);
    const char* envpt = DIAG_ENV("PERSIST_TUNE");
    if (envpt && *envpt) ws->persist_tune = atoi(envpt);
    const char* envpk = DIAG_ENV("PERSIST_KCAP");
    if (envpk && *envpk) ws->persist_kcap = atoi(envpk) > 0 ? atoi(envpk) : 1;
    {
        hipDeviceProp_t prop;
        HIP_CHECK(hipGetDeviceProperties(&prop, dev));
        ws->persist_cus = prop.multiProcessorCount;
        const char* envpc = DIAG_ENV("PERSIST_WGS");
        if (envpc && *envpc && atoi(envpc) >= 2 && atoi(envpc) <= ws->persist_cus) ws->persist_cus = atoi(envpc);
        HIP_CHECK(hipMalloc(&ws->persist_sync, sizeof(int) * potrf_persist_sync_ints()));
        HIP_CHECK(hipMalloc(&ws->persist_hs, sizeof(double) * (size_t)(ws->nblk < 64 ? ws->nblk : 64) * NB * NB));
    }
    const char* envx = DIAG_ENV("DIAG_EXCL_FIRST");
    if (envx && *envx) ws->diag_excl_first = atoi(envx) ? 1 : 0;
    HIP_CHECK(hipEventCreateWithFlags(&ws->ev_fork, hipEventDisableTiming));
    HIP_CHECK(hipEventCreateWithFlags(&ws->ev_early_pre, hipEventDisableTiming));
    if (lauum_plan_wanted(ws, (int)ws->nblk)) (void)lauum_plan_build(ws, (int)ws->nblk);
    const size_t nouter = (size_t)(npad + NB - 1) / NB + 2;
    ws->ev_panel.resize(nouter);
    ws->ev_cols.resize(nouter);
    for (size_t i = 0; i < nouter; ++i) {
        HIP_CHECK(hipEventCreateWithFlags(&ws->ev_panel[i], hipEventDisableTiming));
        HIP_CHECK(hipEventCreateWithFlags(&ws->ev_cols[i], hipEventDisableTiming));
    }
    return 0;
}

void factor_ws_free(FactorWs* ws) {
    if (ws->dinv) (void)hipFree(ws->dinv);
    if (ws->logsum) (void)hipFree(ws->logsum);
    if (ws->info) (void)hipFree(ws->info);
    ws->dinv = ws->logsum = nullptr;
    ws->info = nullptr;
    for (hipEvent_t e : ws->ev_panel) (void)hipEventDestroy(e);
    for (hipEvent_t e : ws->ev_cols) (void)hipEventDestroy(e);
    ws->ev_panel.clear();
    ws->ev_cols.clear();
    if (ws->ev_fork) (void)hipEventDestroy(ws->ev_fork);
    ws->ev_fork = nullptr;
    if (ws->ev_early_pre) (void)hipEventDestroy(ws->ev_early_pre);
    ws->ev_early_pre = nullptr;
    ws->st_panel = nullptr;
    ws->st_tri = nullptr;
    ws->st_tri_half = ws->st_tri_cur = nullptr;
    if (ws->ev_tri) (void)hipEventDestroy(ws->ev_tri);
    ws->ev_tri = nullptr;
    if (ws->ev_tri_lead) (void)hipEventDestroy(ws->ev_tri_lead);
    ws->ev_tri_lead = nullptr;
    if (ws->tri_counter) (void)hipFree(ws->tri_counter);
    ws->tri_counter = nullptr;
    if (ws->upd_tasks) (void)hipFree(ws->upd_tasks);
    ws->upd_tasks = nullptr;
    if (ws->lauum_plan_dev) (void)hipFree(ws->lauum_plan_dev);
    ws->lauum_plan_dev = nullptr;
    if (ws->lauum_part) (void)hipFree(ws->lauum_part);
    ws->lauum_part = nullptr;
    ws->lauum_plan_nt = 0;
    if (ws->persist_sync) (void)hipFree(ws->persist_sync);
    ws->persist_sync = nullptr;
    if (ws->persist_hs) (void)hipFree(ws->persist_hs);
    ws->persist_hs = nullptr;
    ws->prof.destroy();
}

static double syrk_flops(double n, double K) { return K * n * (n + 1.0); }
static double gemm_flops(double m, double n, double K) { return 2.0 * m * n * K; }

static void factor_panel(hipStream_t s, double* A, long npad, long K0, long W, FactorWs* ws) {
    const long ld = npad;
    for (long j = 0; j < W; j += NB) {
        const long c = K0 + j, blk = c / NB;
        double* dv = ws->dinv + blk * 8 * 256;
        ws->prof.begin(s, PF_DIAG, (double)NB * NB * NB / 3.0);
        launch_diag128(s, A, ld, c, dv, ws->logsum + blk, ws->info,
                       ws->diag_excl_first && c == K0 && ws->lookahead == 1 && ws->excl_first_ok);
        ws->prof.end(s);
        const long below = npad - (c + NB);
        if (below <= 0) continue;
        ws->prof.begin(s, PF_TRSM, (double)below * NB * NB);
        launch_trsm128(s, A, ld, c, c + NB, below, dv);
        ws->prof.end(s);
        const long cd = c + NB, ncols = K0 + W - cd;
        if (ncols <= 0) continue;
        const double* P = A + cd * ld + c;
        ws->prof.begin(s, update_nt_uses_64((int)(below / NB), (int)(ncols / NB), (int)(cd / NB), (int)(cd / NB)) ? PF_UPDATE64 : PF_UPDATE,
                       syrk_flops((double)ncols, (double)NB) + gemm_flops((double)(below - ncols), (double)ncols, (double)NB));
        launch_update_nt(s, A + cd * ld + cd, ld, P, ld, P, ld, NB, (int)(below / NB), (int)(ncols / NB), (int)(cd / NB), (int)(cd / NB));
        ws->prof.end(s);
    }
}

static void update_cols(hipStream_t s, double* A, long npad, long K0, long W, long c0, long c1, FactorWs* ws) {
    if (c1 <= c0) return;
    const long ld = npad, rows = npad - c0, cols = c1 - c0;
    const double* P = A + c0 * ld + K0;
    ws->prof.begin(s, update_nt_uses_64((int)(rows / NB), (int)(cols / NB), (int)(c0 / NB), (int)(c0 / NB)) ? PF_UPDATE64 : PF_UPDATE,
                   syrk_flops((double)cols, (double)W) + gemm_flops((double)(rows - cols), (double)cols, (double)W));
    launch_update_nt(s, A + c0 * ld + c0, ld, P, ld, P, ld, (int)W, (int)(rows / NB), (int)(cols / NB), (int)(c0 / NB),
                     (int)(c0 / NB));
    ws->prof.end(s);
}

static void potrf_serial(hipStream_t st, double* A, long npad, FactorWs* ws) {
    (void)hipMemsetAsync(ws->info, 0, sizeof(int) * 4, st);
    const long nbo = ws->nbo_for(npad);
    const long P = (npad + nbo - 1) / nbo;
    auto pcol = [&](long p) { return (p * nbo < npad) ? p * nbo : npad; };
    for (long p = 0; p < P; ++p) {
        factor_panel(st, A, npad, pcol(p), pcol(p + 1) - pcol(p), ws);
        update_cols(st, A, npad, pcol(p), pcol(p + 1) - pcol(p), pcol(p + 1), npad, ws);
    }
}

static void early_inverse(hipStream_t sq, double* A, long npad, int h, FactorWs* ws, bool gated, int gate_gives_up = 0) {
    const int ntl = (int)(npad / NB);
    (void)hipMemsetAsync(ws->tri_counter, 0, sizeof(int) * 4, sq);
    if (gated) launch_wait_persist_rows(sq, ws, 0, h, 0, gate_gives_up);
    ws->prof.begin(sq, PF_TRTRI_EARLY, 0.0);
    launch_inv128(sq, A, ws->scratchX, npad, h, ws->dinv);
// ... 76 lines not shown
            const double t_lead = lead * lead * lead / 3.0 / 45e12;
            const double t_tail = rest * rest * rest / 3.0 / 50e12 + rest / (double)nbo * 0.45e-3 * ((double)nbo / NBO);
            if (t_lead <= t_tail) break;
        }
        if (ws->tri_h_override > 0) h = ws->tri_h_override;
        if (h >= 8 && h < ntl && (h & (h - 1)) == 0) ovl_h = h;
        if (ovl_h > 0) {
            const double lead = (double)ovl_h * NB, rest = (double)npad - lead, right = rest < lead ? rest : lead;
            const double t_early = (lead * lead * lead / 3.0 + lead * lead * right) / 60e12;
            const double t_tail = rest * rest * rest / 3.0 / 50e12 + rest / (double)nbo * 0.45e-3 * ((double)nbo / NBO);
            ws->st_tri_cur = (ws->st_tri_half && ws->tri_half_ok && t_early < 0.8 * t_tail) ? ws->st_tri_half : ws->st_tri;
            ws->tri_cur_pct = (ws->st_tri_cur == ws->st_tri_half) ? 50 : ws->tri_cu_pct;
        }
    }
    ws->ovl_h = 0;
    ws->excl_first_ok = (ovl_h == 0 && ntl < ws->tri_min_nt) ? 1 : 0;
#ifdef MI355GP_DIAG
    const bool uq = ws->upd_queue_probe && ws->upd_tasks && ws->part1_on_panel && ntl >= ws->tri_min_nt && !ws->agg2 && P <= 64;
#else
    const bool uq = false;
#endif
#ifdef MI355GP_DIAG
    if (uq) {
        std::vector<UpdTask> tasks;
        for (long p = 0; p + 2 < P; ++p) {
            const long c0 = pcol(p + 2), ntr = (npad - c0) / NB;
            tasks.push_back(UpdTask{c0 * npad + c0, c0 * npad + pcol(p), ntr * (ntr + 1) / 2, (int)(pcol(p + 1) - pcol(p)), (int)ntr});
        }
        int* counter = reinterpret_cast<int*>(ws->upd_tasks + 64);
        (void)hipMemcpyAsync(ws->upd_tasks, tasks.data(), sizeof(UpdTask) * tasks.size(), hipMemcpyHostToDevice, su);
        (void)hipMemsetAsync(counter, 0, sizeof(int), su);
        ws->prof.begin(su, PF_UPDATE, 0.0);
        launch_update_nt_queue(su, A, npad, ws->upd_tasks, (int)tasks.size(), counter, 512);
        ws->prof.end(su);
    }
#endif
    for (long p = 0; p + 1 < P; ++p) {
        const long K0 = pcol(p), W = pcol(p + 1) - K0;
        (void)hipEventRecord(ws->ev_panel[p], sp);
        if (ovl_h > 0 && pcol(p + 1) == (long)ovl_h * NB) {
            hipStream_t sq = ws->st_tri_cur ? ws->st_tri_cur : ws->st_tri;
            (void)hipStreamWaitEvent(sq, ws->ev_panel[p], 0);
            early_inverse(sq, A, npad, ovl_h, ws, false);
            ws->ovl_h = ovl_h;
        }
        if (ws->part1_on_panel && ntl >= ws->tri_min_nt) {
            if (p > 0 && !uq) (void)hipStreamWaitEvent(sp, ws->ev_cols[p], 0);
            update_cols(sp, A, npad, K0, W, pcol(p + 1), pcol(p + 2), ws);
            factor_panel(sp, A, npad, pcol(p + 1), pcol(p + 2) - pcol(p + 1), ws);
            if (uq) continue;
            (void)hipStreamWaitEvent(su, ws->ev_panel[p], 0);
            if (!ws->agg2) {
                update_cols(su, A, npad, K0, W, pcol(p + 2), npad, ws);
                (void)hipEventRecord(ws->ev_cols[p + 1], su);
                continue;
            }
            if ((p & 1) == 0) {
                if (p + 2 < P) {
                    update_cols(su, A, npad, K0, W, pcol(p + 2), pcol(p + 3), ws);
                } else {
                    update_cols(su, A, npad, K0, W, pcol(p + 2), npad, ws);
                }
                (void)hipEventRecord(ws->ev_cols[p + 1], su);
            } else {
                const long K1 = pcol(p - 1), W2 = pcol(p + 1) - K1;
                update_cols(su, A, npad, K1, W2, pcol(p + 2), pcol(p + 3), ws);
                (void)hipEventRecord(ws->ev_cols[p + 1], su);
                update_cols(su, A, npad, K1, W2, pcol(p + 3), npad, ws);
            }
            continue;
        }
        (void)hipStreamWaitEvent(su, ws->ev_panel[p], 0);
        update_cols(su, A, npad, K0, W, pcol(p + 1), pcol(p + 2), ws);
        (void)hipEventRecord(ws->ev_cols[p + 1], su);
        (void)hipStreamWaitEvent(sp, ws->ev_cols[p + 1], 0);
        factor_panel(sp, A, npad, pcol(p + 1), pcol(p + 2) - pcol(p + 1), ws);
        update_cols(su, A, npad, K0, W, pcol(p + 2), npad, ws);
    }
    (void)hipEventRecord(ws->ev_panel[P], sp);
    (void)hipStreamWaitEvent(st, ws->ev_panel[P], 0);
}

void trtri_device(hipStream_t st, const double* L, double* X, double* T, long npad, FactorWs* ws) {
    const int nt = (int)(npad / NB);
    ws->prof.begin(st, PF_TRTRI, (double)npad * npad * npad / 3.0);
    const int h = ws->ovl_h;
    ws->ovl_h = 0;
    ws->evals_done += 1;
    ws->early_pending = 0;
    if (h > 0 && X == ws->scratchX && T == ws->scratchT && h < nt) {
        int lev = 0;
        while ((1 << lev) < h) ++lev;
        const long off = (long)h * NB * npad + (long)h * NB;
        launch_inv128(st, L + off, X + off, npad, nt - h, ws->dinv + (long)h * 8 * 256);
        for (int level = 0; level < lev; ++level) launch_trtri_level(st, L + off, X + off, T + off, npad, nt - h, level);
        if (nt > 2 * h) {
            const long off2 = (long)2 * h * NB * npad + (long)2 * h * NB;
            launch_trtri_level(st, L + off2, X + off2, T + off2, npad, nt - 2 * h, lev);
        }
        const int nt_pair = nt < 2 * h ? nt : 2 * h;
        (void)hipStreamWaitEvent(st, ws->ev_tri_lead, 0);
        launch_trtri_stage1_steal(st, L, X, T, npad, nt_pair, lev, ws->tri_counter, 512);
        (void)hipStreamWaitEvent(st, ws->ev_tri, 0);
        launch_trtri_level(st, L, X, T, npad, nt_pair, lev, 2);
        for (int level = lev + 1; (1 << level) < nt; ++level) launch_trtri_level(st, L, X, T, npad, nt, level);
    } else {
        if (h > 0) (void)hipStreamWaitEvent(st, ws->ev_tri, 0);
        launch_inv128(st, L, X, npad, nt, ws->dinv);
        for (int level = 0; (1 << level) < nt; ++level) launch_trtri_level(st, L, X, T, npad, nt, level);
    }
    ws->prof.end(st);
}

static bool lauum_plan_wanted(const FactorWs* ws, int nt) {
    return ws->lauum_split && nt <= (ws->lauum_split > 1 ? ws->lauum_split : LAUUM_SPLIT_MAX_NT) && (long)nt * NB > 1024;
}
static bool lauum_plan_build(FactorWs* ws, int nt) {
    std::vector<LauumItem> items;
    std::vector<LauumSum> sums;
    int nparts = 0;
    lauum_split_plan(nt, items, sums, &nparts);
    if (ws->lauum_plan_dev) (void)hipFree(ws->lauum_plan_dev);
    if (ws->lauum_part) (void)hipFree(ws->lauum_part);
    ws->lauum_plan_dev = nullptr;
    ws->lauum_part = nullptr;
    ws->lauum_plan_nt = 0;
    const size_t bi = sizeof(LauumItem) * items.size(), bs = sizeof(LauumSum) * sums.size();
    if (hipMalloc(&ws->lauum_plan_dev, bi + bs + 16) == hipSuccess &&
        hipMalloc(&ws->lauum_part, sizeof(double) * (size_t)lauum_split_tile(nt) * lauum_split_tile(nt) * (size_t)(nparts + 1)) ==
            hipSuccess) {
        (void)hipMemcpy(ws->lauum_plan_dev, items.data(), bi, hipMemcpyHostToDevice);
        if (bs) (void)hipMemcpy((char*)ws->lauum_plan_dev + bi, sums.data(), bs, hipMemcpyHostToDevice);
        ws->lauum_plan_nt = nt;
        ws->lauum_nitems = (int)items.size();
        ws->lauum_nsums = (int)sums.size();
        return true;
    }
    (void)hipGetLastError();
    return false;
}

void lauum_device(hipStream_t st, const double* X, double* W, long npad, FactorWs* ws) {
    const int nt = (int)(npad / NB);
    ws->prof.begin(st, PF_LAUUM, (double)npad * npad * npad / 3.0);
    bool split = lauum_plan_wanted(ws, nt);
    if (split && ws->lauum_plan_nt != nt) {
        hipStreamCaptureStatus cap = hipStreamCaptureStatusNone;
        if (hipStreamIsCapturing(st, &cap) != hipSuccess) (void)hipGetLastError();
        split = (cap == hipStreamCaptureStatusNone) && lauum_plan_build(ws, nt);
    }
    if (split && ws->lauum_plan_nt == nt)
        launch_lauum_split(st, X, W, npad, nt, (const LauumItem*)ws->lauum_plan_dev, ws->lauum_nitems,
                           (const LauumSum*)((const char*)ws->lauum_plan_dev + sizeof(LauumItem) * ws->lauum_nitems), ws->lauum_nsums,
                           ws->lauum_part);
    else
        launch_lauum(st, X, W, npad, nt);
    ws->prof.end(st);
}
```

gpy_amd/csrc/gemm.hip:

```cpp
#include "gemm_tile.h"
#include "internal.h"

#define LDS_OPT_IN(kernel)                                                                              \
    do {                                                                                                \
        static bool done = false;                                                                       \
        if (!done) {                                                                                    \
            (void)hipFuncSetAttribute(reinterpret_cast<const void*>(kernel),                            \
                                      hipFuncAttributeMaxDynamicSharedMemorySize, GT_LDS_BYTES);        \
            done = true;                                                                                \
        }                                                                                               \
    } while (0)

#include <algorithm>
#include <cstdlib>
#include <vector>
#define env_int(name, dflt) diag_env_int(DIAG_ENV(name), dflt)
#define LB(NW) __launch_bounds__((NW) * 64, (NW) / 2)

template <int NW, bool PRE>
__global__ LB(NW) void k_update_nt(double* __restrict__ C, long ldc,
                                                      const double* __restrict__ A, long lda,
                                                      const double* __restrict__ B, long ldb, int K, int ntc,
                                                      int row0t, int col0t, int tri, long ntiles) {
    extern __shared__ __attribute__((aligned(16))) double smem[];
    for (long bid = blockIdx.x; bid < ntiles; bid += gridDim.x) {
        int ti, tj;
        if (tri) {
            ti = (int)((sqrtf(8.0f * (float)bid + 1.0f) - 1.0f) * 0.5f);
            while ((long)ti * (ti + 1) / 2 > bid) --ti;
            while ((long)(ti + 1) * (ti + 2) / 2 <= bid) ++ti;
            tj = (int)(bid - (long)ti * (ti + 1) / 2);
        } else {
            ti = (int)(bid / ntc);
            tj = (int)(bid - (long)ti * ntc);
            if (col0t + tj > row0t + ti) continue;
        }
        d4 acc[4][GTCfg<NW>::NI];
        double* Ct = C + (long)ti * NB * ldc + (long)tj * NB;
        if (PRE) {
            gt_load_buf<NW>(Ct, ldc, acc);
            gemm_tile_128<true, true, NW, true>(A + (long)ti * NB * lda, lda, B + (long)tj * NB * ldb, ldb, K, acc, smem);
            gt_store<0, NW>(Ct, ldc, acc);
        } else {
            gt_zero<NW>(acc);
            gemm_tile_128<true, true, NW>(A + (long)ti * NB * lda, lda, B + (long)tj * NB * ldb, ldb, K, acc, smem);
            gt_store<2, NW>(Ct, ldc, acc);
        }
    }
}

__global__ __launch_bounds__(256) void k_update_nt64(double* __restrict__ C, long ldc, const double* __restrict__ A, long lda,
                                                     const double* __restrict__ B, long ldb, int K, int ntc, int row0t,
                                                     int col0t, int tri) {
    extern __shared__ __attribute__((aligned(16))) double smem[];
    const long bid = blockIdx.x >> 2;
    const int qi = (blockIdx.x >> 1) & 1, qj = blockIdx.x & 1;
    int ti, tj;
    if (tri) {
        ti = (int)((sqrtf(8.0f * (float)bid + 1.0f) - 1.0f) * 0.5f);
        while ((long)ti * (ti + 1) / 2 > bid) --ti;
        while ((long)(ti + 1) * (ti + 2) / 2 <= bid) ++ti;
        tj = (int)(bid - (long)ti * (ti + 1) / 2);
    } else {
        ti = (int)(bid / ntc);
        tj = (int)(bid - (long)ti * ntc);
        if (col0t + tj > row0t + ti) return;
    }
    d4 acc[2][2];
    double* Ct = C + ((long)ti * NB + qi * 64) * ldc + (long)tj * NB + qj * 64;
    gt64_load(Ct, ldc, acc);
    gemm_tile_64_v3<true, true, true>(A + ((long)ti * NB + qi * 64) * lda, lda, B + ((long)tj * NB + qj * 64) * ldb, ldb, K,
                                      acc, smem);
    gt64_store<0>(Ct, ldc, acc);
}

bool update_nt_uses_64(int ntr, int ntc, int row0t, int col0t) {
    static const int upd64_max = env_int("UPD64_MAX", GEMM_DEFAULT_UPD64_MAX);
    const int tri = (row0t == col0t && ntr == ntc) ? 1 : 0;
    const long nblocks = tri ? (long)ntr * (ntr + 1) / 2 : (long)ntr * ntc;
    return nblocks <= upd64_max;
}

void launch_update_nt(hipStream_t st, double* C, long ldc, const double* A, long lda, const double* B, long ldb,
                      int K, int ntr, int ntc, int row0t, int col0t) {
    if (ntr <= 0 || ntc <= 0) return;
    const int tri = (row0t == col0t && ntr == ntc) ? 1 : 0;
    const long nblocks = tri ? (long)ntr * (ntr + 1) / 2 : (long)ntr * ntc;
    if (update_nt_uses_64(ntr, ntc, row0t, col0t)) {
        hipLaunchKernelGGL(k_update_nt64, dim3((unsigned)(4 * nblocks)), dim3(256), GT64_LDS_BYTES, st, C, ldc, A, lda, B, ldb,
                           K, ntc, row0t, col0t, tri);
        return;
    }
    LDS_OPT_IN((k_update_nt<4, true>));
    hipLaunchKernelGGL((k_update_nt<4, true>), dim3((unsigned)nblocks), dim3(256), GT_LDS_BYTES, st, C, ldc, A, lda, B, ldb, K,
                       ntc, row0t, col0t, tri, nblocks);
}

#ifdef MI355GP_DIAG
__global__ LB(4) void k_update_nt_queue(double* __restrict__ A, long ld, const UpdTask* __restrict__ tasks, int ntasks,
                                        int* __restrict__ counter) {
    extern __shared__ __attribute__((aligned(16))) double smem[];
    __shared__ long s_tile;
    for (;;) {
        __syncthreads();
        if (threadIdx.x == 0) s_tile = (long)atomicAdd(counter, 1);
        __syncthreads();
        long bid = s_tile;
        int q = 0;
        while (q < ntasks && bid >= tasks[q].ntiles) bid -= tasks[q++].ntiles;
        if (q >= ntasks) return;
        const UpdTask tk = tasks[q];
        int ti = (int)((sqrtf(8.0f * (float)bid + 1.0f) - 1.0f) * 0.5f);
        while ((long)ti * (ti + 1) / 2 > bid) --ti;
        while ((long)(ti + 1) * (ti + 2) / 2 <= bid) ++ti;
        const int tj = (int)(bid - (long)ti * (ti + 1) / 2);
        d4 acc[4][GTCfg<4>::NI];
        double* Ct = A + tk.c_off + (long)ti * NB * ld + (long)tj * NB;
        const double* P = A + tk.p_off;
        gt_load_buf<4>(Ct, ld, acc);
        gemm_tile_128<true, true, 4, true>(P + (long)ti * NB * ld, ld, P + (long)tj * NB * ld, ld, tk.K, acc, smem);
        gt_store<0, 4>(Ct, ld, acc);
    }
}

void launch_update_nt_queue(hipStream_t st, double* A, long ld, const UpdTask* tasks_dev, int ntasks, int* counter, int wgs) {
    LDS_OPT_IN(k_update_nt_queue);
    hipLaunchKernelGGL(k_update_nt_queue, dim3((unsigned)wgs), dim3(256), GT_LDS_BYTES, st, A, ld, tasks_dev, ntasks, counter);
}
#endif

__host__ __device__ __forceinline__ int trtri_rows_last(int nt, int nbt) {
    const int pairs = (nt + 2 * nbt - 1) / (2 * nbt), right0 = (2 * (pairs - 1) + 1) * nbt;
    const int rows = nt - right0;
    return rows < 0 ? 0 : (rows > nbt ? nbt : rows);
}
__host__ __device__ __forceinline__ long trtri_level_tiles(int nt, int nbt) {
    const int pairs = (nt + 2 * nbt - 1) / (2 * nbt);
    return (long)(pairs - 1) * nbt * nbt + (long)nbt * trtri_rows_last(nt, nbt);
}
template <int STAGE>
__device__ __forceinline__ void trtri_map(int bid, int nt, int nbt, int& p, int& ri, int& cj) {
    const int per = nbt * nbt, pairs = (nt + 2 * nbt - 1) / (2 * nbt), full = (pairs - 1) * per;
    if (bid < full) {
        p = bid / per;
        const int rem = bid - p * per;
        if (STAGE == 1) {
            cj = rem / nbt;
            ri = rem - cj * nbt;
        } else {
            ri = nbt - 1 - rem / nbt;
            cj = rem % nbt;
        }
    } else {
        p = pairs - 1;
        const int rem = bid - full, rows = trtri_rows_last(nt, nbt);
        if (STAGE == 1) {
            cj = rem / rows;
            ri = rem - cj * rows;
        } else {
            ri = rows - 1 - rem / nbt;
            cj = rem % nbt;
        }
    }
}

template <int STAGE, int NW>
__device__ __forceinline__ void trtri_stage_tile(int bid, const double* __restrict__ L, double* __restrict__ X,
                                                 double* __restrict__ T, long ld, int nt, int nbt, double* smem) {
    int p, ri, cj;
    trtri_map<STAGE>(bid, nt, nbt, p, ri, cj);
    const int left0 = 2 * p * nbt, right0 = left0 + nbt;
    const int ti = right0 + ri, tj = left0 + cj;
    if (ti >= nt) return;
    d4 acc[4][GTCfg<NW>::NI];
    gt_zero<NW>(acc);
    if (STAGE == 1) {
        const int K = (right0 - tj) * NB;
        gemm_tile_128<true, false, NW>(L + (long)ti * NB * ld + (long)tj * NB, ld,
                                   X + (long)tj * NB * ld + (long)tj * NB, ld, K, acc, smem);
        gt_store<0, NW>(T + (long)ti * NB * ld + (long)tj * NB, ld, acc);
    } else {
        const int K = (ti - right0 + 1) * NB;
        gemm_tile_128<true, false, NW>(X + (long)ti * NB * ld + (long)right0 * NB, ld,
                                   T + (long)right0 * NB * ld + (long)tj * NB, ld, K, acc, smem);
        gt_store<1, NW>(X + (long)ti * NB * ld + (long)tj * NB, ld, acc);
    }
}

template <int STAGE>
__global__ __launch_bounds__(256) void k_trtri_stage64(const double* __restrict__ L, double* __restrict__ X,
                                                       double* __restrict__ T, long ld, int nt, int nbt) {
    extern __shared__ __attribute__((aligned(16))) double smem[];
    const int bid = blockIdx.x >> 2, qi = (blockIdx.x >> 1) & 1, qj = blockIdx.x & 1;
    int p, ri, cj;
    trtri_map<STAGE>(bid, nt, nbt, p, ri, cj);
    const int left0 = 2 * p * nbt, right0 = left0 + nbt;
    const int ti = right0 + ri, tj = left0 + cj;
    if (ti >= nt) return;
    d4 acc[2][2];
    gt64_zero(acc);
    const long r0 = (long)ti * NB + qi * 64, c0 = (long)tj * NB + qj * 64;
    if (STAGE == 1) {
        const int K = (right0 - tj) * NB;
        gemm_tile_64_v3<true, false>(L + r0 * ld + (long)tj * NB, ld, X + (long)tj * NB * ld + c0, ld, K, acc, smem);
        gt64_store<0>(T + r0 * ld + c0, ld, acc);
    } else {
        const int K = (ti - right0 + 1) * NB;
        gemm_tile_64_v3<true, false>(X + r0 * ld + (long)right0 * NB, ld, T + (long)right0 * NB * ld + c0, ld, K, acc, smem);
        gt64_store<1>(X + r0 * ld + c0, ld, acc);
    }
}

template <int STAGE, int NW>
__global__ LB(NW) void k_trtri_stage(const double* __restrict__ L, double* __restrict__ X,
                                                        double* __restrict__ T, long ld, int nt, int nbt) {
    extern __shared__ __attribute__((aligned(16))) double smem[];
    trtri_stage_tile<STAGE, NW>((int)blockIdx.x, L, X, T, ld, nt, nbt, smem);
}

__global__ LB(4) void k_trtri_stage1_steal(const double* __restrict__ L, double* __restrict__ X, double* __restrict__ T,
                                           long ld, int nt, int nbt, int* __restrict__ counter, int nblocks) {
    extern __shared__ __attribute__((aligned(16))) double smem[];
    __shared__ int s_bid;
    for (;;) {
        if (threadIdx.x == 0) s_bid = atomicAdd(counter, 1);
        __syncthreads();
        const int bid = s_bid;
        __syncthreads();
        if (bid >= nblocks) return;
        trtri_stage_tile<1, 4>(bid, L, X, T, ld, nt, nbt, smem);
    }
}

void launch_trtri_stage1_steal(hipStream_t st, const double* L, double* X, double* T, long ld, int nt, int level,
                               int* counter, int grid) {
    const int nbt = 1 << level;
    if (nbt >= nt) return;
    const int nblocks = (int)trtri_level_tiles(nt, nbt);
    if (nblocks <= 0) return;
    LDS_OPT_IN(k_trtri_stage1_steal);
    if (grid > nblocks) grid = nblocks;
    hipLaunchKernelGGL(k_trtri_stage1_steal, dim3((unsigned)grid), dim3(256), GT_LDS_BYTES, st, L, X, T, ld, nt, nbt,
                       counter, nblocks);
}

template <int NW>
static void launch_trtri_level_t(hipStream_t st, long nblocks, const double* L, double* X, double* T, long ld, int nt,
                                 int nbt, int stages) {
    LDS_OPT_IN((k_trtri_stage<1, NW>));
    LDS_OPT_IN((k_trtri_stage<2, NW>));
    if (stages & 1)
        hipLaunchKernelGGL((k_trtri_stage<1, NW>), dim3((unsigned)nblocks), dim3(NW * 64), GT_LDS_BYTES, st, L, X, T, ld, nt, nbt);
    if (stages & 2)
        hipLaunchKernelGGL((k_trtri_stage<2, NW>), dim3((unsigned)nblocks), dim3(NW * 64), GT_LDS_BYTES, st, L, X, T, ld, nt, nbt);
}

void launch_trtri_level(hipStream_t st, const double* L, double* X, double* T, long ld, int nt, int level, int stages) {
    const int nbt = 1 << level;
    if (nbt >= nt) return;
    const long nblocks = trtri_level_tiles(nt, nbt);
    if (nblocks <= 0) return;
    static const int tri64_max = env_int("TRI64_MAX", GEMM_DEFAULT_TRI64_MAX);
    if (nblocks <= tri64_max) {
        if (stages & 1)
            hipLaunchKernelGGL((k_trtri_stage64<1>), dim3((unsigned)(4 * nblocks)), dim3(256), GT64_LDS_BYTES, st, L, X, T, ld, nt, nbt);
        if (stages & 2)
            hipLaunchKernelGGL((k_trtri_stage64<2>), dim3((unsigned)(4 * nblocks)), dim3(256), GT64_LDS_BYTES, st, L, X, T, ld, nt, nbt);
        return;
    }
    launch_trtri_level_t<4>(st, nblocks, L, X, T, ld, nt, nbt, stages);
}

template <int NW>
__global__ LB(NW) void k_lauum(const double* __restrict__ X, double* __restrict__ W, long ld, int nt) {
    extern __shared__ __attribute__((aligned(16))) double smem[];
    const int bid = blockIdx.x;
    int ti = (int)((sqrtf(8.0f * (float)bid + 1.0f) - 1.0f) * 0.5f);
    while ((long)ti * (ti + 1) / 2 > bid) --ti;
    while ((long)(ti + 1) * (ti + 2) / 2 <= bid) ++ti;
    const int tj = bid - (int)((long)ti * (ti + 1) / 2);
    d4 acc[4][GTCfg<NW>::NI];
    gt_zero<NW>(acc);
    const int K = (nt - ti) * NB;
    gemm_tile_128<false, false, NW>(X + (long)ti * NB * ld + (long)ti * NB, ld, X + (long)ti * NB * ld + (long)tj * NB, ld,
                                K, acc, smem);
    gt_store<0, NW>(W + (long)ti * NB * ld + (long)tj * NB, ld, acc);
}

__global__ __launch_bounds__(256) void k_lauum64(const double* __restrict__ X, double* __restrict__ W, long ld, int nt) {
    extern __shared__ __attribute__((aligned(16))) double smem[];
    const int bid = blockIdx.x >> 2, qi = (blockIdx.x >> 1) & 1, qj = blockIdx.x & 1;
    int ti = (int)((sqrtf(8.0f * (float)bid + 1.0f) - 1.0f) * 0.5f);
    while ((long)ti * (ti + 1) / 2 > bid) --ti;
    while ((long)(ti + 1) * (ti + 2) / 2 <= bid) ++ti;
    const int tj = bid - (int)((long)ti * (ti + 1) / 2);
    d4 acc[2][2];
    gt64_zero(acc);
    const int K = (nt - ti) * NB;
    const long r0 = (long)ti * NB + qi * 64, c0 = (long)tj * NB + qj * 64;
    gemm_tile_64_v3<false, false>(X + (long)ti * NB * ld + r0, ld, X + (long)ti * NB * ld + c0, ld, K, acc, smem);
    gt64_store<0>(W + r0 * ld + c0, ld, acc);
}

#define LAUUM_KC 1024
#define LAUUM_T128_MIN_NT 24
static int lauum_kc_rows_128(int nt) {
    static const int forced = env_int("LAUUM_KC", 0);
    if (forced >= NB) return forced / NB * NB;
    int best = LAUUM_KC;
    double best_us = 1e30;
    for (int kc = 2; kc <= 32 && kc <= nt; ++kc) {
        std::vector<int> len;
        long parts = 0;
        for (int ti = 0; ti < nt; ++ti) {
            const int K = nt - ti, nch = (K + kc - 1) / kc;
            for (int tj = 0; tj <= ti; ++tj)
                for (int c = 0; c < nch; ++c) len.push_back(c + 1 < nch ? kc : K - c * kc);
            if (nch > 1) parts += (long)nch * (ti + 1);
        }
        std::sort(len.begin(), len.end(), [](int a, int b) { return a > b; });
        std::vector<double> slot(512, 0.0);
        std::make_heap(slot.begin(), slot.end(), [](double a, double b) { return a > b; });
        double end = 0.0;
        for (int l : len) {
            std::pop_heap(slot.begin(), slot.end(), [](double a, double b) { return a > b; });
            const double t = slot.back() + 27.4 * l + 8.0;
            slot.back() = t;
            if (t > end) end = t;
            std::push_heap(slot.begin(), slot.end(), [](double a, double b) { return a > b; });
        }
        const double us = end + (double)parts * (NB * NB * 8.0) / 3.0e6;
        if (us < best_us - 0.5) {
            best_us = us;
            best = kc * NB;
        }
    }
    return best;
}
__global__ __launch_bounds__(256) void k_lauum64_items(const double* __restrict__ X, double* __restrict__ W, long ld,
                                                       const LauumItem* __restrict__ items, double* __restrict__ part) {
    extern __shared__ __attribute__((aligned(16))) double smem[];
    const LauumItem it = items[blockIdx.x];
    d4 acc[2][2];
    gt64_zero(acc);
    const long r0 = (long)it.ti * NB + (it.q >> 1) * 64, c0 = (long)it.tj * NB + (it.q & 1) * 64;
    gemm_tile_64_v3<false, false>(X + (long)it.k0 * ld + r0, ld, X + (long)it.k0 * ld + c0, ld, it.klen, acc, smem);
    if (it.part < 0) gt64_store<0>(W + r0 * ld + c0, ld, acc);
    else gt64_store<0>(part + (long)it.part * 4096, 64, acc);
}

__global__ LB(4) void k_lauum128_items(const double* __restrict__ X, double* __restrict__ W, long ld,
                                       const LauumItem* __restrict__ items, double* __restrict__ part) {
    extern __shared__ __attribute__((aligned(16))) double smem[];
    const LauumItem it = items[blockIdx.x];
    d4 acc[4][GTCfg<4>::NI];
    gt_zero<4>(acc);
    const long r0 = (long)it.ti * NB, c0 = (long)it.tj * NB;
    gemm_tile_128<false, false, 4>(X + (long)it.k0 * ld + r0, ld, X + (long)it.k0 * ld + c0, ld, it.klen, acc, smem);
    if (it.part < 0) gt_store<0, 4>(W + r0 * ld + c0, ld, acc);
    else gt_store<0, 4>(part + (long)it.part * (NB * NB), NB, acc);
}

__global__ __launch_bounds__(256) void k_lauum128_reduce(double* __restrict__ W, long ld, const LauumSum* __restrict__ sums,
                                                         const double* __restrict__ part) {
    const LauumSum sm = sums[blockIdx.x];
    const long r0 = (long)sm.ti * NB, c0 = (long)sm.tj * NB;
    for (int e = threadIdx.x; e < NB * NB / 2; e += 256) {
        const int i = e >> 6, j = 2 * (e & 63);
        d2 s = *reinterpret_cast<const d2*>(part + (long)sm.first * (NB * NB) + i * NB + j);
        for (int c = 1; c < sm.n; ++c) s += *reinterpret_cast<const d2*>(part + (long)(sm.first + c) * (NB * NB) + i * NB + j);
        *reinterpret_cast<d2*>(W + (r0 + i) * ld + c0 + j) = s;
    }
}

__global__ __launch_bounds__(256) void k_lauum64_reduce(double* __restrict__ W, long ld, const LauumSum* __restrict__ sums,
                                                        const double* __restrict__ part) {
    const LauumSum sm = sums[blockIdx.x];
    const long r0 = (long)sm.ti * NB + (sm.q >> 1) * 64, c0 = (long)sm.tj * NB + (sm.q & 1) * 64;
    for (int e = threadIdx.x; e < 2048; e += 256) {
        const int i = e >> 5, j = 2 * (e & 31);
        d2 s = *reinterpret_cast<const d2*>(part + (long)sm.first * 4096 + i * 64 + j);
        for (int c = 1; c < sm.n; ++c) s += *reinterpret_cast<const d2*>(part + (long)(sm.first + c) * 4096 + i * 64 + j);
        *reinterpret_cast<d2*>(W + (r0 + i) * ld + c0 + j) = s;
    }
}

int lauum_split_tile(int nt) { return nt >= LAUUM_T128_MIN_NT ? 128 : 64; }

void lauum_split_plan(int nt, std::vector<LauumItem>& items, std::vector<LauumSum>& sums, int* nparts) {
    items.clear();
    sums.clear();
    int np = 0;
    const int nq = lauum_split_tile(nt) == 128 ? 1 : 4;
    static const int kc64 = env_int("LAUUM_KC64", 0) / NB * NB;
    const int kc = (nq == 1) ? lauum_kc_rows_128(nt) : (kc64 >= NB ? kc64 : (nt <= 16 ? 512 : LAUUM_KC));
    for (int ti = 0; ti < nt; ++ti)
        for (int tj = 0; tj <= ti; ++tj)
            for (int q = 0; q < nq; ++q) {
                const int k0 = ti * NB, K = (nt - ti) * NB, nch = (K + kc - 1) / kc;
                if (nch > 1) sums.push_back(LauumSum{ti, tj, q, np, nch});
                for (int c = 0; c < nch; ++c) {
                    const int len = (c + 1 < nch) ? kc : K - c * kc;
                    items.push_back(LauumItem{ti, tj, q, k0 + c * kc, len, nch > 1 ? np++ : -1});
                }
            }
    std::stable_sort(items.begin(), items.end(), [](const LauumItem& a, const LauumItem& b) { return a.klen > b.klen; });
    *nparts = np;
}

void launch_lauum_split(hipStream_t st, const double* X, double* W, long ld, int nt, const LauumItem* items_dev, int nitems,
                        const LauumSum* sums_dev, int nsums, double* part) {
    if (lauum_split_tile(nt) == 128) {
        LDS_OPT_IN(k_lauum128_items);
        hipLaunchKernelGGL(k_lauum128_items, dim3((unsigned)nitems), dim3(256), GT_LDS_BYTES, st, X, W, ld, items_dev, part);
        if (nsums > 0) hipLaunchKernelGGL(k_lauum128_reduce, dim3((unsigned)nsums), dim3(256), 0, st, W, ld, sums_dev, part);
        return;
    }
    hipLaunchKernelGGL(k_lauum64_items, dim3((unsigned)nitems), dim3(256), GT64_LDS_BYTES, st, X, W, ld, items_dev, part);
    if (nsums > 0) hipLaunchKernelGGL(k_lauum64_reduce, dim3((unsigned)nsums), dim3(256), 0, st, W, ld, sums_dev, part);
}

template <int NW>
static void launch_lauum_t(hipStream_t st, long nblocks, const double* X, double* W, long ld, int nt) {
    LDS_OPT_IN((k_lauum<NW>));
    hipLaunchKernelGGL((k_lauum<NW>), dim3((unsigned)nblocks), dim3(NW * 64), GT_LDS_BYTES, st, X, W, ld, nt);
}

bool lauum_uses_64(int nt) {
    static const int lauum64_max = env_int("LAUUM64_MAX", GEMM_DEFAULT_LAUUM64_MAX);
    return (long)nt * (nt + 1) / 2 <= lauum64_max;
}

void launch_lauum(hipStream_t st, const double* X, double* W, long ld, int nt) {
    const long nblocks = (long)nt * (nt + 1) / 2;
    static const int lauum64_max = env_int("LAUUM64_MAX", GEMM_DEFAULT_LAUUM64_MAX);
    if (nblocks <= lauum64_max) {
        hipLaunchKernelGGL(k_lauum64, dim3((unsigned)(4 * nblocks)), dim3(256), GT64_LDS_BYTES, st, X, W, ld, nt);
        return;
    }
    launch_lauum_t<4>(st, nblocks, X, W, ld, nt);
}

template <int NW>
__global__ LB(NW) void k_trmm_lower(const double* __restrict__ X, long ldx,
                                                       const double* __restrict__ B, long ldb,
                                                       double* __restrict__ Out, long ldo, int ntc) {
    extern __shared__ __attribute__((aligned(16))) double smem[];
    const int ti = (int)(gridDim.x / ntc) - 1 - (int)(blockIdx.x / ntc), tj = blockIdx.x % ntc;
    d4 acc[4][GTCfg<NW>::NI];
    gt_zero<NW>(acc);
    gemm_tile_128<true, false, NW>(X + (long)ti * NB * ldx, ldx, B + (long)tj * NB, ldb, (ti + 1) * NB, acc, smem);
    gt_store<0, NW>(Out + (long)ti * NB * ldo + (long)tj * NB, ldo, acc);
}

template <int NW>
__global__ LB(NW) void k_trmm_lower_T(const double* __restrict__ X, long ldx, const double* __restrict__ B, long ldb,
                                      double* __restrict__ Out, long ldo, int ntc, int nt) {
    extern __shared__ __attribute__((aligned(16))) double smem[];
    const int ti = blockIdx.x / ntc, tj = blockIdx.x % ntc;
    d4 acc[4][GTCfg<NW>::NI];
    gt_zero<NW>(acc);
    gemm_tile_128<false, false, NW>(X + (long)ti * NB * ldx + (long)ti * NB, ldx, B + (long)ti * NB * ldb + (long)tj * NB, ldb,
                                    (nt - ti) * NB, acc, smem);
    gt_store<0, NW>(Out + (long)ti * NB * ldo + (long)tj * NB, ldo, acc);
}

void launch_trmm_lower_T(hipStream_t st, const double* X, long ldx, const double* B, long ldb, double* Out, long ldo,
                         int ntr, int ntc) {
    LDS_OPT_IN((k_trmm_lower_T<4>));
    hipLaunchKernelGGL((k_trmm_lower_T<4>), dim3((unsigned)(ntr * ntc)), dim3(256), GT_LDS_BYTES, st, X, ldx, B, ldb, Out,
                       ldo, ntc, ntr);
}

template <int NW>
static void launch_trmm_lower_t(hipStream_t st, const double* X, long ldx, const double* B, long ldb, double* Out,
                                long ldo, int ntr, int ntc) {
    LDS_OPT_IN((k_trmm_lower<NW>));
    hipLaunchKernelGGL((k_trmm_lower<NW>), dim3((unsigned)(ntr * ntc)), dim3(NW * 64), GT_LDS_BYTES, st, X, ldx, B, ldb,
                       Out, ldo, ntc);
}

void launch_trmm_lower(hipStream_t st, const double* X, long ldx, const double* B, long ldb, double* Out, long ldo,
                       int ntr, int ntc) {
    launch_trmm_lower_t<4>(st, X, ldx, B, ldb, Out, ldo, ntr, ntc);
}

template <int MODE>
__global__ __launch_bounds__(256) void k_trmm64(const double* __restrict__ X, long ldx, const double* __restrict__ B, long ldb,
                                                double* __restrict__ Out, long ldo, int nt, int ntother, double alpha) {
    extern __shared__ __attribute__((aligned(16))) double smem[];
    const int q = blockIdx.x & 3, qi = q >> 1, qj = q & 1, bid = blockIdx.x >> 2;
    int ti, tj;
    if (MODE == 0) { ti = nt - 1 - bid / ntother; tj = bid % ntother; }
    else if (MODE == 1) { ti = bid / ntother; tj = bid % ntother; }
    else if (MODE == 2) { tj = nt - 1 - bid / ntother; ti = bid % ntother; }
    else { tj = bid / ntother; ti = bid % ntother; }
    const long r0 = (long)ti * NB + qi * 64, c0 = (long)tj * NB + qj * 64;
    d4 acc[2][2];
    gt64_zero(acc);
    if (MODE == 0) gemm_tile_64_v3<true, false>(X + r0 * ldx, ldx, B + c0, ldb, (ti + 1) * NB, acc, smem);
    else if (MODE == 1) gemm_tile_64_v3<false, false>(X + (long)ti * NB * ldx + r0, ldx, B + (long)ti * NB * ldb + c0, ldb, (nt - ti) * NB, acc, smem);
    else if (MODE == 2) gemm_tile_64_v3<true, true>(B + r0 * ldb, ldb, X + c0 * ldx, ldx, (tj + 1) * NB, acc, smem);
    else gemm_tile_64_v3<true, false>(B + r0 * ldb + (long)tj * NB, ldb, X + (long)tj * NB * ldx + c0, ldx, (nt - tj) * NB, acc, smem);
#pragma unroll
    for (int mi = 0; mi < 2; ++mi)
#pragma unroll
        for (int ni = 0; ni < 2; ++ni) acc[mi][ni] *= alpha;
    gt64_store<0>(Out + r0 * ldo + c0, ldo, acc);
}

void launch_trmm64(hipStream_t st, int mode, const double* X, long ldx, const double* B, long ldb, double* Out, long ldo, int nt,
                   int ntother, double alpha) {
    const unsigned grid = (unsigned)(4 * nt * ntother);
    switch (mode) {
        case 0: hipLaunchKernelGGL((k_trmm64<0>), dim3(grid), dim3(256), GT64_LDS_BYTES, st, X, ldx, B, ldb, Out, ldo, nt, ntother, alpha); break;
        case 1: hipLaunchKernelGGL((k_trmm64<1>), dim3(grid), dim3(256), GT64_LDS_BYTES, st, X, ldx, B, ldb, Out, ldo, nt, ntother, alpha); break;
        case 2: hipLaunchKernelGGL((k_trmm64<2>), dim3(grid), dim3(256), GT64_LDS_BYTES, st, X, ldx, B, ldb, Out, ldo, nt, ntother, alpha); break;
        default: hipLaunchKernelGGL((k_trmm64<3>), dim3(grid), dim3(256), GT64_LDS_BYTES, st, X, ldx, B, ldb, Out, ldo, nt, ntother, alpha); break;
    }
}

void launch_gemm_tn_sq(hipStream_t st, const double* A, long lda, long K, double* C, long ldc, int nt, double alpha,
                       double beta);

__device__ long long g_gemm_clk[2];

template <bool AK, bool BK, int NW>
__global__ LB(NW) void k_gemm_full(const double* __restrict__ A, long lda,
                                                      const double* __restrict__ B, long ldb, double* __restrict__ C,
                                                      long ldc, int K, int ntc, double alpha, double beta, int swz) {
    extern __shared__ __attribute__((aligned(16))) double smem[];
    int bid = blockIdx.x;
    if (swz & 1) {
        const int xcd = bid & 7, loc = bid >> 3;
        const int stiles = ntc >> 3;
        const int sidx = (loc >> 6) * 8 + xcd;
        const int in = loc & 63;
        bid = ((sidx / stiles) * 8 + (in >> 3)) * ntc + (sidx % stiles) * 8 + (in & 7);
    }
    const int ti = bid / ntc, tj = bid % ntc;
    d4 acc[4][GTCfg<NW>::NI];
    gt_zero<NW>(acc);
    const double* Ap = AK ? A + (long)ti * NB * lda : A + (long)ti * NB;
    const double* Bp = BK ? B + (long)tj * NB * ldb : B + (long)tj * NB;
    const long long c0 = clock64(), w0 = wall_clock64();
    gemm_tile_128<AK, BK, NW>(Ap, lda, Bp, ldb, K, acc, smem);
    if (blockIdx.x == 0 && threadIdx.x == 0) {
        g_gemm_clk[0] = clock64() - c0;
        g_gemm_clk[1] = wall_clock64() - w0;
    }
    double* Ct = C + (long)ti * NB * ldc + (long)tj * NB;
    if (beta == 0.0) {
#pragma unroll
        for (int mi = 0; mi < 4; ++mi)
#pragma unroll
            for (int ni = 0; ni < GTCfg<NW>::NI; ++ni) acc[mi][ni] *= alpha;
        gt_store<0, NW>(Ct, ldc, acc);
    } else {
        gt_store<3, NW>(Ct, ldc, acc, alpha, beta);
    }
}

template <bool AK, bool BK>
static void launch_gemm_full(hipStream_t st, unsigned nblocks, const double* A, long lda, const double* B, long ldb,
                             double* C, long ldc, int K, int ntc, double alpha, double beta) {
    static const int dbg_ld0 = env_int("DBG_LD0", 0), dbg_swz = env_int("DBG_SWZ", 0);
    if (dbg_ld0) lda = ldb = 0;
    static const int dbg_1wg = env_int("DBG_1WG", 0);
    const int swz = (dbg_swz && (ntc % 8 == 0) && ((nblocks / ntc) % 8 == 0)) ? 1 : 0;
    const size_t lds = dbg_1wg ? 100 * 1024 : GT_LDS_BYTES;
    (void)hipFuncSetAttribute(reinterpret_cast<const void*>(k_gemm_full<AK, BK, 4>),
                              hipFuncAttributeMaxDynamicSharedMemorySize, (int)lds);
    hipLaunchKernelGGL((k_gemm_full<AK, BK, 4>), dim3(nblocks), dim3(256), lds, st, A, lda, B, ldb, C, ldc, K,
                       ntc, alpha, beta, swz);
}

void launch_dbg_gemm(hipStream_t st, int a_mcontig, int b_ncontig, long M, long N, long K, const double* A,
                     const double* B, double* C, double alpha, double beta) {
    const int ntr = (int)(M / NB), ntc = (int)(N / NB);
    const unsigned grid = (unsigned)(ntr * ntc);
    const long lda = a_mcontig ? M : K, ldb = b_ncontig ? N : K;
    if (!a_mcontig && !b_ncontig) launch_gemm_full<true, true>(st, grid, A, lda, B, ldb, C, N, (int)K, ntc, alpha, beta);
    else if (!a_mcontig && b_ncontig) launch_gemm_full<true, false>(st, grid, A, lda, B, ldb, C, N, (int)K, ntc, alpha, beta);
    else if (a_mcontig && b_ncontig) launch_gemm_full<false, false>(st, grid, A, lda, B, ldb, C, N, (int)K, ntc, alpha, beta);
    else launch_gemm_full<false, true>(st, grid, A, lda, B, ldb, C, N, (int)K, ntc, alpha, beta);
}

void launch_gemm_tn_sq(hipStream_t st, const double* A, long lda, long K, double* C, long ldc, int nt, double alpha,
                       double beta) {
    launch_gemm_full<false, false>(st, (unsigned)(nt * nt), A, lda, A, lda, C, ldc, (int)K, nt, alpha, beta);
}

int gemm_last_clock(double* mhz, double* cycles) {
// ... 43 lines not shown
```

gpy_amd/csrc/gemm_tile.h:

```cpp
#pragma once
#include "common.h"

#define GT_LDS_BYTES 73728

template <int NW>
struct GTCfg {
    static_assert(NW == 4, "the tile kernels run 4-wave workgroups");
    static constexpr int NTHR = NW * 64;
    static constexpr int NI = 4;
    static constexpr int WCOLS = NI * 16;
    static constexpr int WPR = 128 / WCOLS;
};

template <bool AK, bool BK, bool NEGA = false>
__device__ __forceinline__ void gemm_tile_128_v3(const double* __restrict__ A, long lda, const double* __restrict__ B,
                                                 long ldb, int K, d4 (&acc)[4][4], double* smem);

template <bool AK, bool BK, int NW, bool NEGA = false>
__device__ __forceinline__ void gemm_tile_128(const double* __restrict__ A, long lda,
                                              const double* __restrict__ B, long ldb, int K,
                                              d4 (&acc)[4][GTCfg<NW>::NI], double* smem) {
    gemm_tile_128_v3<AK, BK, NEGA>(A, lda, B, ldb, K, acc, smem);
}

template <int NW>
__device__ __forceinline__ void gt_zero(d4 (&acc)[4][GTCfg<NW>::NI]) {
#pragma unroll
    for (int mi = 0; mi < 4; ++mi)
#pragma unroll
        for (int ni = 0; ni < GTCfg<NW>::NI; ++ni) acc[mi][ni] = (d4){0.0, 0.0, 0.0, 0.0};
}

template <int NW>
__device__ __forceinline__ double* gt_cbase(double* C, long ldc) {
    const int t = threadIdx.x, lane = t & 63, w = t >> 6, wr = w / GTCfg<NW>::WPR, wc = w % GTCfg<NW>::WPR;
    return C + (long)(wr * 64 + (lane >> 4)) * ldc + wc * GTCfg<NW>::WCOLS + (lane & 15);
}

template <int NW>
__device__ __forceinline__ void gt_load_buf(const double* Ct, long ldc, d4 (&acc)[4][GTCfg<NW>::NI]) {
    typedef unsigned int u2 __attribute__((ext_vector_type(2)));
    const int t = threadIdx.x, lane = t & 63, w = t >> 6, wr = w / GTCfg<NW>::WPR, wc = w % GTCfg<NW>::WPR;
    __amdgpu_buffer_rsrc_t rs = __builtin_amdgcn_make_buffer_rsrc(const_cast<double*>(Ct), 0, 0x7fffffff, 0x00020000);
    const int ldb = (int)ldc * 8;
    const int voff = (wr * 64 + (lane >> 4)) * ldb + (wc * GTCfg<NW>::WCOLS + (lane & 15)) * 8;
#pragma unroll
    for (int mi = 0; mi < 4; ++mi)
#pragma unroll
        for (int r = 0; r < 4; ++r) {
            const int soff = (mi * 16 + 4 * r) * ldb;
#pragma unroll
            for (int ni = 0; ni < GTCfg<NW>::NI; ++ni) {
                const u2 v = __builtin_amdgcn_raw_buffer_load_b64(rs, voff + ni * 128, soff, 0);
                acc[mi][ni][r] = __builtin_bit_cast(double, v);
            }
        }
}

template <int NW>
__device__ __forceinline__ void gt_load_neg(const double* __restrict__ C, long ldc, d4 (&acc)[4][GTCfg<NW>::NI]) {
    const double* base = gt_cbase<NW>(const_cast<double*>(C), ldc);
#pragma unroll
    for (int mi = 0; mi < 4; ++mi)
#pragma unroll
        for (int ni = 0; ni < GTCfg<NW>::NI; ++ni)
#pragma unroll
            for (int r = 0; r < 4; ++r) acc[mi][ni][r] = -base[(long)(mi * 16 + 4 * r) * ldc + ni * 16];
}

template <int MODE, int NW>
__device__ __forceinline__ void gt_store(double* __restrict__ C, long ldc, const d4 (&acc)[4][GTCfg<NW>::NI],
                                         double alpha = 1.0, double beta = 0.0) {
    constexpr int NI = GTCfg<NW>::NI;
    double* base = gt_cbase<NW>(C, ldc);
#pragma unroll
    for (int mi = 0; mi < 4; ++mi) {
        double old[NI][4];
        if (MODE >= 2) {
#pragma unroll
            for (int ni = 0; ni < NI; ++ni)
#pragma unroll
                for (int r = 0; r < 4; ++r) old[ni][r] = base[(long)(mi * 16 + 4 * r) * ldc + ni * 16];
        }
#pragma unroll
        for (int ni = 0; ni < NI; ++ni)
#pragma unroll
            for (int r = 0; r < 4; ++r) {
                double* p = base + (long)(mi * 16 + 4 * r) * ldc + ni * 16;
                const double v = acc[mi][ni][r];
                if (MODE == 0) *p = v;
                else if (MODE == 1) *p = -v;
                else if (MODE == 2) *p = old[ni][r] - v;
                else *p = alpha * v + beta * old[ni][r];
            }
    }
}

#define GT3_SMN 132
#define GT3_OP 2176
#define GT3_LDS_BYTES (2 * 2 * GT3_OP * 8)

__device__ __forceinline__ int gt3_h(int r) { return ((r >> 1) & 7) ^ ((((r & 15) >= 4) && ((r & 15) <= 11)) ? 2 : 0); }

template <bool KC>
__device__ __forceinline__ void gt3_src_offsets(long ld, int lane, int w, int (&voff)[4]) {
#pragma unroll
    for (int ii = 0; ii < 4; ++ii) {
        const int i = 4 * w + ii;
        if (KC) {
            const int row = 8 * i + (lane >> 3), g = (lane & 7) ^ gt3_h(row);
            voff[ii] = (int)((row * ld + 2 * g) * 8);
        } else {
            voff[ii] = (int)((i * ld + 2 * lane) * 8);
        }
    }
}

template <bool KC>
__device__ __forceinline__ void gt3_issue(__amdgpu_buffer_rsrc_t rs, const int (&voff)[4], int soff, double* sdst, int w) {
#pragma unroll
    for (int ii = 0; ii < 4; ++ii) {
        const int i = 4 * w + ii;
        double* d = KC ? sdst + i * 128 : sdst + i * GT3_SMN;
        __builtin_amdgcn_raw_ptr_buffer_load_lds(rs, d, 16, voff[ii], soff, 0, 0);
    }
}

template <bool AK, bool BK, bool NEGA>
__device__ __forceinline__ void gemm_tile_128_v3(const double* __restrict__ A, long lda,
                                                 const double* __restrict__ B, long ldb, int K, d4 (&acc)[4][4],
                                                 double* smem) {
    const int t = threadIdx.x, lane = t & 63, w = t >> 6, wr = w >> 1, wc = w & 1;
    const int nk = K / 16;
    const int arow = wr * 64 + (lane & 15), bcol = wc * 64 + (lane & 15), kq = lane >> 4;
    auto rsrc = [](const double* p) {
        return __builtin_amdgcn_make_buffer_rsrc(const_cast<double*>(p), 0, 0x7fffffff, 0x00020000);
    };
    int va[4], vb[4];
    gt3_src_offsets<AK>(lda, lane, w, va);
    gt3_src_offsets<BK>(ldb, lane, w, vb);
    const long sa = AK ? 16 : 16 * lda, sb = BK ? 16 : 16 * ldb;
    int fa0[4], fb0[4];
#pragma unroll
    for (int mi = 0; mi < 4; ++mi) {
        const int r = arow + mi * 16, c = bcol + mi * 16;
        fa0[mi] = AK ? r * 16 : r;
        fb0[mi] = BK ? c * 16 : c;
    }
    const int ha = gt3_h(arow), hb = gt3_h(bcol);
    gt3_issue<AK>(rsrc(A), va, 0, smem, w);
    gt3_issue<BK>(rsrc(B), vb, 0, smem + GT3_OP, w);
    __builtin_amdgcn_s_waitcnt(0x0F70);
    __syncthreads();
    for (int kt = 0; kt < nk; ++kt) {
        const int cur = kt & 1;
        if (kt + 1 < nk) {
            double* nxt = smem + (cur ^ 1) * 2 * GT3_OP;
            gt3_issue<AK>(rsrc(A + (kt + 1) * sa), va, 0, nxt, w);
            gt3_issue<BK>(rsrc(B + (kt + 1) * sb), vb, 0, nxt + GT3_OP, w);
        }
        const double* a_s = smem + cur * 2 * GT3_OP;
        const double* b_s = a_s + GT3_OP;
#pragma unroll
        for (int e = 0; e < 2; ++e) {
            d2 af[4], bf[4];
#pragma unroll
            for (int mi = 0; mi < 4; ++mi) {
                if (AK) af[mi] = *reinterpret_cast<const d2*>(a_s + fa0[mi] + 2 * ((2 * kq + e) ^ ha));
                else af[mi] = (d2){a_s[(4 * kq + 2 * e) * GT3_SMN + fa0[mi]], a_s[(4 * kq + 2 * e + 1) * GT3_SMN + fa0[mi]]};
            }
#pragma unroll
            for (int ni = 0; ni < 4; ++ni) {
                if (BK) bf[ni] = *reinterpret_cast<const d2*>(b_s + fb0[ni] + 2 * ((2 * kq + e) ^ hb));
                else bf[ni] = (d2){b_s[(4 * kq + 2 * e) * GT3_SMN + fb0[ni]], b_s[(4 * kq + 2 * e + 1) * GT3_SMN + fb0[ni]]};
            }
#pragma unroll
            for (int s = 0; s < 2; ++s)
#pragma unroll
                for (int mi = 0; mi < 4; ++mi)
#pragma unroll
                    for (int ni = 0; ni < 4; ++ni)
                        acc[mi][ni] = mfma_f64(NEGA ? -af[mi][s] : af[mi][s], bf[ni][s], acc[mi][ni]);
        }
        __builtin_amdgcn_s_waitcnt(0x0F70);
        __syncthreads();
    }
}


template <bool AK, bool BK, bool NEGA>
__device__ __forceinline__ void gemm_tile_128_v3_multi(const double* const* __restrict__ Atab, long aoff, long lda,
                                                       const double* const* __restrict__ Btab, long boff, long ldb,
                                                       int k0, int k1, int slabs, d4 (&acc)[4][4], double* smem) {
    const int t = threadIdx.x, lane = t & 63, w = t >> 6, wr = w >> 1, wc = w & 1;
    const int nk = (k1 - k0) * slabs;
    const int arow = wr * 64 + (lane & 15), bcol = wc * 64 + (lane & 15), kq = lane >> 4;
    auto rsrc = [](const double* p) {
        return __builtin_amdgcn_make_buffer_rsrc(const_cast<double*>(p), 0, 0x7fffffff, 0x00020000);
    };
    int va[4], vb[4];
    gt3_src_offsets<AK>(lda, lane, w, va);
    gt3_src_offsets<BK>(ldb, lane, w, vb);
    const long sa = AK ? 16 : 16 * lda, sb = BK ? 16 : 16 * ldb;
    int fa0[4], fb0[4];
#pragma unroll
    for (int mi = 0; mi < 4; ++mi) {
        const int r = arow + mi * 16, c = bcol + mi * 16;
        fa0[mi] = AK ? r * 16 : r;
        fb0[mi] = BK ? c * 16 : c;
    }
    const int ha = gt3_h(arow), hb = gt3_h(bcol);
    int pk = k0, ps = 0;
    const double* Ab = Atab[pk] + aoff;
    const double* Bb = Btab[pk] + boff;
    gt3_issue<AK>(rsrc(Ab), va, 0, smem, w);
    gt3_issue<BK>(rsrc(Bb), vb, 0, smem + GT3_OP, w);
    __builtin_amdgcn_s_waitcnt(0x0F70);
    __syncthreads();
    for (int kt = 0; kt < nk; ++kt) {
        const int cur = kt & 1;
        if (kt + 1 < nk) {
            if (++ps == slabs) {
                ps = 0;
                ++pk;
                Ab = Atab[pk] + aoff;
                Bb = Btab[pk] + boff;
            }
            double* nxt = smem + (cur ^ 1) * 2 * GT3_OP;
            gt3_issue<AK>(rsrc(Ab + ps * sa), va, 0, nxt, w);
            gt3_issue<BK>(rsrc(Bb + ps * sb), vb, 0, nxt + GT3_OP, w);
        }
        const double* a_s = smem + cur * 2 * GT3_OP;
        const double* b_s = a_s + GT3_OP;
#pragma unroll
        for (int e = 0; e < 2; ++e) {
            d2 af[4], bf[4];
#pragma unroll
            for (int mi = 0; mi < 4; ++mi) {
                if (AK) af[mi] = *reinterpret_cast<const d2*>(a_s + fa0[mi] + 2 * ((2 * kq + e) ^ ha));
                else af[mi] = (d2){a_s[(4 * kq + 2 * e) * GT3_SMN + fa0[mi]], a_s[(4 * kq + 2 * e + 1) * GT3_SMN + fa0[mi]]};
            }
#pragma unroll
            for (int ni = 0; ni < 4; ++ni) {
                if (BK) bf[ni] = *reinterpret_cast<const d2*>(b_s + fb0[ni] + 2 * ((2 * kq + e) ^ hb));
                else bf[ni] = (d2){b_s[(4 * kq + 2 * e) * GT3_SMN + fb0[ni]], b_s[(4 * kq + 2 * e + 1) * GT3_SMN + fb0[ni]]};
            }
#pragma unroll
            for (int s = 0; s < 2; ++s)
#pragma unroll
                for (int mi = 0; mi < 4; ++mi)
#pragma unroll
                    for (int ni = 0; ni < 4; ++ni)
                        acc[mi][ni] = mfma_f64(NEGA ? -af[mi][s] : af[mi][s], bf[ni][s], acc[mi][ni]);
        }
        __builtin_amdgcn_s_waitcnt(0x0F70);
        __syncthreads();
    }
}

#define GT64_OP 1088
#define GT64_PAIR 136
#define GT64_LDS_BYTES (2 * 2 * GT64_OP * 8)

template <bool KC>
__device__ __forceinline__ void gt64_src_offsets(long ld, int lane, int w, int (&voff)[2]) {
#pragma unroll
    for (int ii = 0; ii < 2; ++ii) {
        const int i = 2 * w + ii;
        if (KC) {
            const int row = 8 * i + (lane >> 3), g = (lane & 7) ^ gt3_h(row);
            voff[ii] = (int)((row * ld + 2 * g) * 8);
        } else {
            voff[ii] = (int)(((2 * i + (lane >> 5)) * ld + 2 * (lane & 31)) * 8);
        }
    }
}

template <bool KC>
__device__ __forceinline__ void gt64_issue(__amdgpu_buffer_rsrc_t rs, const int (&voff)[2], double* sdst, int w) {
#pragma unroll
    for (int ii = 0; ii < 2; ++ii) {
        const int i = 2 * w + ii;
        double* d = KC ? sdst + i * 128 : sdst + i * GT64_PAIR;
        __builtin_amdgcn_raw_ptr_buffer_load_lds(rs, d, 16, voff[ii], 0, 0, 0);
    }
}

template <bool AK, bool BK, bool NEGA = false>
__device__ __forceinline__ void gemm_tile_64_v3(const double* __restrict__ A, long lda, const double* __restrict__ B,
                                                long ldb, int K, d4 (&acc)[2][2], double* smem) {
    const int t = threadIdx.x, lane = t & 63, w = t >> 6, wr = w >> 1, wc = w & 1;
    const int nk = K / 16;
    const int arow = wr * 32 + (lane & 15), bcol = wc * 32 + (lane & 15), kq = lane >> 4;
    auto rsrc = [](const double* p) {
        return __builtin_amdgcn_make_buffer_rsrc(const_cast<double*>(p), 0, 0x7fffffff, 0x00020000);
    };
    int va[2], vb[2];
    gt64_src_offsets<AK>(lda, lane, w, va);
    gt64_src_offsets<BK>(ldb, lane, w, vb);
    const long sa = AK ? 16 : 16 * lda, sb = BK ? 16 : 16 * ldb;
    int fa0[2], fb0[2];
#pragma unroll
    for (int mi = 0; mi < 2; ++mi) {
        const int r = arow + mi * 16, c = bcol + mi * 16;
        fa0[mi] = AK ? r * 16 : r;
        fb0[mi] = BK ? c * 16 : c;
    }
    const int ha = gt3_h(arow), hb = gt3_h(bcol);
    gt64_issue<AK>(rsrc(A), va, smem, w);
    gt64_issue<BK>(rsrc(B), vb, smem + GT64_OP, w);
    __builtin_amdgcn_s_waitcnt(0x0F70);
    __syncthreads();
    for (int kt = 0; kt < nk; ++kt) {
        const int cur = kt & 1;
        if (kt + 1 < nk) {
            double* nxt = smem + (cur ^ 1) * 2 * GT64_OP;
            gt64_issue<AK>(rsrc(A + (kt + 1) * sa), va, nxt, w);
            gt64_issue<BK>(rsrc(B + (kt + 1) * sb), vb, nxt + GT64_OP, w);
        }
        const double* a_s = smem + cur * 2 * GT64_OP;
        const double* b_s = a_s + GT64_OP;
#pragma unroll
        for (int e = 0; e < 2; ++e) {
            d2 af[2], bf[2];
#pragma unroll
            for (int mi = 0; mi < 2; ++mi) {
                if (AK) af[mi] = *reinterpret_cast<const d2*>(a_s + fa0[mi] + 2 * ((2 * kq + e) ^ ha));
                else af[mi] = (d2){a_s[(2 * kq + e) * GT64_PAIR + fa0[mi]], a_s[(2 * kq + e) * GT64_PAIR + 64 + fa0[mi]]};
            }
#pragma unroll
            for (int ni = 0; ni < 2; ++ni) {
                if (BK) bf[ni] = *reinterpret_cast<const d2*>(b_s + fb0[ni] + 2 * ((2 * kq + e) ^ hb));
                else bf[ni] = (d2){b_s[(2 * kq + e) * GT64_PAIR + fb0[ni]], b_s[(2 * kq + e) * GT64_PAIR + 64 + fb0[ni]]};
            }
#pragma unroll
            for (int s = 0; s < 2; ++s)
#pragma unroll
                for (int mi = 0; mi < 2; ++mi)
#pragma unroll
                    for (int ni = 0; ni < 2; ++ni)
                        acc[mi][ni] = mfma_f64(NEGA ? -af[mi][s] : af[mi][s], bf[ni][s], acc[mi][ni]);
// ... 36 lines not shown
```

gpy_amd/csrc/internal.h:

```cpp
#pragma once
#include <shared_mutex>
#include <vector>

#include "common.h"

bool update_nt_uses_64(int ntr, int ntc, int row0t, int col0t);
struct UpdTask { long c_off, p_off, ntiles; int K, ntr; };
#ifdef MI355GP_DIAG
void launch_update_nt_queue(hipStream_t st, double* A, long ld, const UpdTask* tasks_dev, int ntasks, int* counter, int wgs);
#endif
void launch_update_nt(hipStream_t st, double* C, long ldc, const double* A, long lda, const double* B, long ldb,
                      int K, int ntr, int ntc, int row0t, int col0t);
void launch_trtri_level(hipStream_t st, const double* L, double* X, double* T, long ld, int nt, int level,
                        int stages = 3);
void launch_lauum(hipStream_t st, const double* X, double* W, long ld, int nt);
struct LauumItem { int ti, tj, q, k0, klen, part; };
struct LauumSum { int ti, tj, q, first, n; };
void lauum_split_plan(int nt, std::vector<LauumItem>& items, std::vector<LauumSum>& sums, int* nparts);
int lauum_split_tile(int nt);
void launch_lauum_split(hipStream_t st, const double* X, double* W, long ld, int nt, const LauumItem* items_dev, int nitems,
                        const LauumSum* sums_dev, int nsums, double* part);
bool lauum_uses_64(int nt);
void launch_trmm_lower(hipStream_t st, const double* X, long ldx, const double* B, long ldb, double* Out, long ldo,
                       int ntr, int ntc);
void launch_trmm_lower_T(hipStream_t st, const double* X, long ldx, const double* B, long ldb, double* Out, long ldo,
                         int ntr, int ntc);
void launch_trmm64(hipStream_t st, int mode, const double* X, long ldx, const double* B, long ldb, double* Out, long ldo, int nt,
                   int ntother, double alpha);
void launch_gemm_tn_sq(hipStream_t st, const double* A, long lda, long K, double* C, long ldc, int nt, double alpha,
                       double beta);
void launch_dbg_gemm(hipStream_t st, int a_mcontig, int b_ncontig, long M, long N, long K, const double* A,
                     const double* B, double* C, double alpha, double beta);

void launch_diag128(hipStream_t st, double* A, long ld, long c0, double* dinv, double* logsum, int* info,
                    int exclusive = 0);
void launch_trsm128(hipStream_t st, double* A, long ld, long c0, long r0, long mrows, const double* dinv);
void launch_trtri_stage1_steal(hipStream_t st, const double* L, double* X, double* T, long ld, int nt, int level,
                               int* counter, int grid);
void launch_inv128(hipStream_t st, const double* L, double* X, long ld, int nblk, const double* dinv_all);
void launch_dbg_mfma(hipStream_t st, const double* a, const double* b, double* d);

enum { PF_UPDATE = 0, PF_TRTRI = 1, PF_LAUUM = 2, PF_DIAG = 3, PF_TRSM = 4, PF_UPDATE64 = 5, PF_PERSIST = 6, PF_TRTRI_EARLY = 7, PF_NUM = 8 };
struct KernelProf {
    unsigned mask = 0;
    bool on = false;
    std::vector<hipEvent_t> pool;
    struct Rec { int fam; double flops; size_t e0; };
    std::vector<Rec> recs;
    bool open = false;
    void begin(hipStream_t st, int fam, double flops);
    void end(hipStream_t st);
    void reset() { recs.clear(); }
    int collect(double* ms, double* flops, int* launches);
    void destroy();
};

struct FactorWs {
    double* dinv = nullptr;
    double* logsum = nullptr;
    int* info = nullptr;
    long nblk = 0;
    hipStream_t st_panel = nullptr;
    std::vector<hipEvent_t> ev_panel;
    std::vector<hipEvent_t> ev_cols;
    hipEvent_t ev_fork = nullptr;
    hipEvent_t ev_early_pre = nullptr;
    int agg2 = 0;
    int persist_auto = 1, sched_state = 0, sched_force_steps = 0, persist_auto_off = 0;
    int sched_np = 0, sched_ns = 0;
    int can_calibrate = 0;
    float sched_ms_persist = 0.f, sched_ms_steps = 0.f;
    int evals_done = 0;
    int early_pending = 0;
    int lauum_split = 1, lauum_plan_nt = 0, lauum_nitems = 0, lauum_nsums = 0;
    void* lauum_plan_dev = nullptr;
    double* lauum_part = nullptr;
    int persist_tri = 1;
    int persist_tri_min_nt = 16;
    int upd_queue_probe = 0;
    UpdTask* upd_tasks = nullptr;
    int part1_on_panel = 1;
    int lookahead = 1;
    int nbo_override = 0;
    long nbo_for(long npad) const {
        long w = nbo_override > 0 ? nbo_override : (npad <= FACTOR_NBO_SMALL_N ? FACTOR_NBO_SMALL : NBO);
        w = (w / NB) * NB;
        return w < NB ? NB : w;
    }
    double* scratchX = nullptr;
    double* scratchT = nullptr;
    int tri_overlap = FACTOR_DEFAULT_TRI_OVERLAP, tri_cu_pct = 75, tri_min_nt = 48, tri_wgs = 0, ovl_h = 0;
    hipStream_t st_tri = nullptr, st_tri_half = nullptr, st_tri_cur = nullptr;
    int tri_half_ok = 1, tri_cur_pct = 75;
    hipEvent_t ev_tri = nullptr, ev_tri_lead = nullptr;
    int* tri_counter = nullptr;
    int tri_h_override = 0;
    int diag_excl_first = FACTOR_DEFAULT_DIAG_EXCL_FIRST, excl_first_ok = 0;
    int solve_overlap = 1;
    int persist = FACTOR_DEFAULT_PERSIST, persist_max_nt = FACTOR_PERSIST_MAX_NT, persist_kcap = 2, persist_cus = 0;
    int persist_skip = 0, persist_aborts = 0, persist_used = 0;
    hipEvent_t ev_persist_pre = nullptr;
    int persist_grid_last = 0;
    int persist_tune = 0;
    int persist_test = 0;
    int* persist_sync = nullptr;
    double* persist_hs = nullptr;
    KernelProf prof;
};
std::shared_mutex& engine_gate(int device);
struct EngineShared {
    std::shared_mutex* m;
    bool shared = true;
    explicit EngineShared(int device) : m(&engine_gate(device)) { m->lock_shared(); }
    EngineShared(const EngineShared&) = delete;
    EngineShared& operator=(const EngineShared&) = delete;
    ~EngineShared() {
        if (shared) m->unlock_shared();
        else m->unlock();
    }
    bool try_exclusive() {
        m->unlock_shared();
        if (m->try_lock()) {
            shared = false;
            return true;
        }
        m->lock_shared();
        return false;
    }
    void share() {
        m->unlock();
        m->lock_shared();
        shared = true;
    }
};
int factor_engine(int device, hipStream_t* main, hipStream_t* panel, hipStream_t* tri, hipStream_t* tri_half = nullptr);
int factor_ws_alloc(FactorWs* ws, long npad);
void factor_ws_free(FactorWs* ws);
void potrf_device(hipStream_t st, double* A, long npad, FactorWs* ws);
void trtri_device(hipStream_t st, const double* L, double* X, double* T, long npad, FactorWs* ws);
void lauum_device(hipStream_t st, const double* X, double* W, long npad, FactorWs* ws);

bool potrf_persist_eligible(long npad, const FactorWs* ws);
int persist_box_verdict(int set = -2);
bool potrf_persist_aborted(int info, FactorWs* ws, bool* clean);
int potrf_persist_sync_ints();
bool launch_potrf_persist(hipStream_t st, double* A, long npad, FactorWs* ws, long long* dbg = nullptr);
void launch_wait_persist_resident(hipStream_t st, const FactorWs* ws, int timeout_ms = 2);
int persist_early_h(long npad, const FactorWs* ws);
void launch_wait_persist_rows(hipStream_t st, const FactorWs* ws, int r0, int r1, int cols, int give_up = 0);

struct KernParams {
    int kind;
    int ard;
    int D;
    double variance;
    double power = 0.0;
    const double* pw = nullptr;
    int col = 0;
    double bias = 0.0;
};
void launch_scale_inputs(hipStream_t st, const double* X, long n, int D, const double* inv_ls, int ard,
                         double* Xt, long ldx);
void launch_kbuild_sym(hipStream_t st, KernParams kp, const double* Xt, long ldx, long n, long npad, double* A,
                       const double* noise, long noise_len, double jit, int lower_only, int add_diag,
                       int accumulate = 0, const double* mul = nullptr);
void launch_kbuild_cross(hipStream_t st, KernParams kp, const double* Xt1, long ld1, long n, const double* Xt2,
                         long ld2, long m, double* Kout, long ldk, int accumulate = 0, int diag_same = 0,
                         const double* mul = nullptr);
int launch_kbuild_cols(hipStream_t st, KernParams kp, const double* Xt1, long ld1, long n, const double* Xt2, long ld2, long m,
                       long mcols, double* Kout, long ldk, const double* V, int Dy, double* colpart);
void launch_tri_matvec(hipStream_t st, const double* X, long ld, long n, const double* R, int Dy, double* tmp,
                       double* alpha, double* partials);
struct GradOut {
    double* partials;
    int stride;
    int nblocks;
};
int grad_num_blocks(long n);
void launch_grad_fused(hipStream_t st, KernParams kp, const double* Xt, long ldx, long n, const double* W,
                       long ldw, const double* alpha, int Dy, double* partials, int stride,
                       const double* aa_scale = nullptr, const double* Mul = nullptr, long ldm = 0);
struct RankTerm {
    const double* Y;
    const double* V;
    int Dy;
    double beta, gscale;
    const double* rowscale = nullptr;
};
int launch_grad_cols(hipStream_t st, KernParams kp, const double* Xt1, long ld1, long n, const double* Xt2, long ld2,
                     long m, long mcols, const double* G, long ldg, RankTerm rk, double* partials, double* colpart,
                     int* nblocks_out);
void launch_studentt_scale(hipStream_t st, const double* scal, double nu, long n, double* out);
void launch_grad_generic(hipStream_t st, KernParams kp, const double* Xt1, long ld1, long n, const double* Xt2,
                         long ld2, long m, int symmetric, const double* G, long ldg, double* partials,
                         int stride, double* Hout = nullptr, long ldh = 0,
                         RankTerm rk = RankTerm{nullptr, nullptr, 0, 0.0, 1.0, nullptr});
void launch_periodic_gradx(hipStream_t st, KernParams kp, const double* Xt1, long ld1, long n, const double* Xt2, long ld2,
                           long m, const double* W, long ldw, int wt, double* out);
int launch_grad_coreg(hipStream_t st, bool fused, KernParams kp, const double* Xt1, long ld1, long n, const double* Xt2, long ld2,
                      long m, const double* G, long ldg, const double* alpha, int Dy, double* partials,
                      const double* aa_scale = nullptr, const double* Mul = nullptr, long ldm = 0);
void launch_col_reduce_vec(hipStream_t st, const double* M, long ld, long rows, long cols, const double* kd, double* out);
int launch_colreduce_multi(hipStream_t st, const double* M, long ld, long rows, long cols, const double* V, long sr,
                           long sc, int nvt, int ones, double* part);
void launch_sum_splits(hipStream_t st, const double* src, long cnt, int nsplit, int accumulate, double* dst);
int trmv_chunk_rows(long n);
void launch_trmv_lower(hipStream_t st, const double* X, long ld, long n, const double* R, int Dy, double* y);
void launch_trmv_lower_T(hipStream_t st, const double* X, long ld, long n, const double* y, int Dy, double* out,
                         double* partials);
int gemm_last_clock(double* mhz, double* cycles);
void launch_gemm(hipStream_t st, int a_mcontig, int b_ncontig, long M, long N, long K, const double* A, long lda,
                 const double* B, long ldb, double* C, long ldc, double alpha, double beta);
void launch_gram_splitk(hipStream_t st, const double* P, long ldp, long rows, long mp, int S, int accumulate,
                        double* part);
int grad_generic_num_blocks(long n, long m);
void launch_reduce_partials(hipStream_t st, const double* partials, int nblocks, int stride, double* out);
void launch_scalars(hipStream_t st, const double* alpha, const double* R, const double* W, long ldw, long n,
                    int Dy, const double* logsum, long nblk, double* out4, double* diag_out, const int* info = nullptr);
void launch_extract(hipStream_t st, const double* A, long ld, long n, int mode, const double* alpha, int Dy,
                    double* out, int transpose, const double* aa_scale = nullptr);
void launch_pad_from_dense(hipStream_t st, const double* src, long n, double* A, long npad, const double* noise,
                           long noise_len, double jit);
void launch_col_reduce(hipStream_t st, const double* M, long ld, long rows, long cols, const double* v, int Dy,
                       double c0, int mode, double* out);

void launch_rowdots(hipStream_t st, const double* K, const double* T, long ld, long rows, long m, const double* v, int Dy,
                    double* out_s, double* t_out);
void launch_rowscale_sqrt(hipStream_t st, const double* M, long ld, long rows, long cols, const double* w, double* Out);

void launch_laplace_B(hipStream_t st, const double* K, long npad, long n, const double* sw, double jit, double* A);
size_t symv_part_doubles(long npad);
void launch_symv_lower(hipStream_t st, const double* K, long npad, long n, const double* v0, const double* v1, double* y0,
                       double* y1, double* part);
void launch_laplace_dLdK(hipStream_t st, const double* Binv, long npad, long n, const double* sw, const double* a,
// ... 6 lines not shown
```

gpy_amd/csrc/peaks.hip:

```cpp
#include "internal.h"

__global__ __launch_bounds__(256) void k_peak_mfma(double* out, long long* clk, int iters, double seed) {
    d4 acc[8];
#pragma unroll
    for (int i = 0; i < 8; ++i) acc[i] = (d4){seed, seed + i, 0.0, 1.0};
    const double a = seed + threadIdx.x * 1e-9, b = 1.0 - threadIdx.x * 1e-9;
    const long long c0 = clock64(), w0 = wall_clock64();
    for (int it = 0; it < iters; ++it) {
#pragma unroll
        for (int i = 0; i < 8; ++i)
            asm volatile("v_mfma_f64_16x16x4_f64 %0, %1, %2, %0" : "+v"(acc[i]) : "v"(a), "v"(b));
    }
    asm volatile("s_nop 15\n s_nop 15" ::: "memory");
    const long long c1 = clock64(), w1 = wall_clock64();
    double s = 0.0;
#pragma unroll
    for (int i = 0; i < 8; ++i) s += acc[i][0] + acc[i][1] + acc[i][2] + acc[i][3];
    if (s == 12345.678) out[0] = s;
    if (blockIdx.x == 0 && threadIdx.x == 0) { clk[0] = c1 - c0; clk[1] = w1 - w0; }
}

__global__ __launch_bounds__(256) void k_peak_fma(double* out, int iters, double seed) {
    double acc[16];
#pragma unroll
    for (int i = 0; i < 16; ++i) acc[i] = seed + i;
    const double a = 1.0 + threadIdx.x * 1e-12, b = 1e-9;
    for (int it = 0; it < iters; ++it) {
#pragma unroll
        for (int i = 0; i < 16; ++i) acc[i] = fma(acc[i], a, b);
    }
    double s = 0.0;
#pragma unroll
    for (int i = 0; i < 16; ++i) s += acc[i];
    if (s == 12345.678) out[0] = s;
}

__global__ __launch_bounds__(256) void k_copy(const d2* __restrict__ src, d2* __restrict__ dst, long n2) {
    for (long i = (long)blockIdx.x * blockDim.x + threadIdx.x; i < n2; i += (long)gridDim.x * blockDim.x)
        dst[i] = src[i];
}

__global__ __launch_bounds__(256) void k_fill(d2* __restrict__ dst, long n2, double v) {
    for (long i = (long)blockIdx.x * blockDim.x + threadIdx.x; i < n2; i += (long)gridDim.x * blockDim.x)
        dst[i] = (d2){v, v + 1.0};
}

int run_peaks(int device, double* out8) {
    HIP_CHECK(hipSetDevice(device));
    hipEvent_t e0, e1;
    HIP_CHECK(hipEventCreate(&e0));
    HIP_CHECK(hipEventCreate(&e1));
    double* dummy;
    long long* dclk;
    HIP_CHECK(hipMalloc(&dummy, 1024));
    HIP_CHECK(hipMalloc(&dclk, 64));
    float ms;
    long long h[2];
    const int iters = 20000;
    for (int pass = 0; pass < 2; ++pass) {
        const int blocks = pass == 0 ? 256 : 256 * 8;
        hipLaunchKernelGGL(k_peak_mfma, dim3(blocks), dim3(256), 0, 0, dummy, dclk, 200, 0.5);
        HIP_CHECK(hipEventRecord(e0, 0));
        hipLaunchKernelGGL(k_peak_mfma, dim3(blocks), dim3(256), 0, 0, dummy, dclk, iters, 0.5);
        HIP_CHECK(hipEventRecord(e1, 0));
        HIP_CHECK(hipEventSynchronize(e1));
        HIP_CHECK(hipEventElapsedTime(&ms, e0, e1));
        HIP_CHECK(hipMemcpy(h, dclk, 16, hipMemcpyDeviceToHost));
        const double tf = (double)blocks * 4 * iters * 8 * 2048.0 / (ms * 1e-3) / 1e12;
        if (pass == 0) {
            out8[4] = (double)h[0] / ((double)iters * 8);
            out8[6] = tf;
        } else {
            out8[0] = tf;
            out8[5] = (double)h[0] / (double)h[1] * 100.0;
            out8[7] = (double)h[0] / ((double)iters * 8 * 8);
        }
    }
    const int blocks = 256 * 8;
    hipLaunchKernelGGL(k_peak_fma, dim3(blocks), dim3(256), 0, 0, dummy, 100, 0.5);
    HIP_CHECK(hipEventRecord(e0, 0));
    hipLaunchKernelGGL(k_peak_fma, dim3(blocks), dim3(256), 0, 0, dummy, iters, 0.5);
    HIP_CHECK(hipEventRecord(e1, 0));
    HIP_CHECK(hipEventSynchronize(e1));
    HIP_CHECK(hipEventElapsedTime(&ms, e0, e1));
    out8[1] = (double)blocks * 256 * iters * 16 * 2.0 / (ms * 1e-3) / 1e12;
    const long bytes = 2L << 30, n2 = bytes / 16;
    d2 *a, *b;
    HIP_CHECK(hipMalloc(&a, bytes));
    HIP_CHECK(hipMalloc(&b, bytes));
    hipLaunchKernelGGL(k_fill, dim3(2048), dim3(256), 0, 0, a, n2, 1.0);
    hipLaunchKernelGGL(k_copy, dim3(2048), dim3(256), 0, 0, a, b, n2);
    HIP_CHECK(hipEventRecord(e0, 0));
    for (int r = 0; r < 5; ++r) hipLaunchKernelGGL(k_copy, dim3(2048), dim3(256), 0, 0, a, b, n2);
    HIP_CHECK(hipEventRecord(e1, 0));
    HIP_CHECK(hipEventSynchronize(e1));
    HIP_CHECK(hipEventElapsedTime(&ms, e0, e1));
    out8[2] = 5.0 * 2.0 * bytes / (ms * 1e-3) / 1e9;
    HIP_CHECK(hipEventRecord(e0, 0));
    for (int r = 0; r < 5; ++r) hipLaunchKernelGGL(k_fill, dim3(2048), dim3(256), 0, 0, b, n2, 2.0);
    HIP_CHECK(hipEventRecord(e1, 0));
    HIP_CHECK(hipEventSynchronize(e1));
    HIP_CHECK(hipEventElapsedTime(&ms, e0, e1));
    out8[3] = 5.0 * bytes / (ms * 1e-3) / 1e9;
    (void)hipFree(a);
    (void)hipFree(b);
    (void)hipFree(dummy);
    (void)hipFree(dclk);
    (void)hipEventDestroy(e0);
    (void)hipEventDestroy(e1);
    return 0;
}


__global__ __launch_bounds__(256) void k_peak_mix(double* out, int iters, double seed, int mode) {
    const bool do_mfma = mode == 0 || (mode == 2 && (blockIdx.x & 1) == 0);
    double s = 0.0;
    if (do_mfma) {
        d4 acc[8];
#pragma unroll
        for (int i = 0; i < 8; ++i) acc[i] = (d4){seed, seed + i, 0.0, 1.0};
        const double a = seed + threadIdx.x * 1e-9, b = 1.0 - threadIdx.x * 1e-9;
        for (int it = 0; it < iters; ++it) {
#pragma unroll
            for (int i = 0; i < 8; ++i)
                asm volatile("v_mfma_f64_16x16x4_f64 %0, %1, %2, %0" : "+v"(acc[i]) : "v"(a), "v"(b));
        }
        asm volatile("s_nop 15\n s_nop 15" ::: "memory");
#pragma unroll
        for (int i = 0; i < 8; ++i) s += acc[i][0] + acc[i][1] + acc[i][2] + acc[i][3];
    } else {
        double acc[16];
#pragma unroll
        for (int i = 0; i < 16; ++i) acc[i] = seed + i;
        const double a = 1.0 + threadIdx.x * 1e-12, b = 1e-9;
        for (int it = 0; it < iters; ++it) {
#pragma unroll
            for (int r = 0; r < 8; ++r)
#pragma unroll
                for (int i = 0; i < 16; ++i) asm volatile("v_fma_f64 %0, %0, %1, %2" : "+v"(acc[i]) : "v"(a), "v"(b));
        }
#pragma unroll
        for (int i = 0; i < 16; ++i) s += acc[i];
    }
    if (s == 12345.678) out[0] = s;
}

extern "C" int mi355gp_dbg_pipe_share(int device, double* out4) {
    HIP_CHECK(hipSetDevice(device));
    hipEvent_t e0, e1;
    HIP_CHECK(hipEventCreate(&e0));
    HIP_CHECK(hipEventCreate(&e1));
    double* dummy;
    HIP_CHECK(hipMalloc(&dummy, 1024));
    const int iters = 4000, blocks = 256 * 8;
    for (int mode = 0; mode < 3; ++mode) {
        float ms;
        hipLaunchKernelGGL(k_peak_mix, dim3(blocks), dim3(256), 0, 0, dummy, 100, 0.5, mode);
        HIP_CHECK(hipEventRecord(e0, 0));
        hipLaunchKernelGGL(k_peak_mix, dim3(blocks), dim3(256), 0, 0, dummy, iters, 0.5, mode);
        HIP_CHECK(hipEventRecord(e1, 0));
        HIP_CHECK(hipEventSynchronize(e1));
        HIP_CHECK(hipEventElapsedTime(&ms, e0, e1));
        out4[mode] = ms;
    }
    out4[3] = (double)blocks * 4 * iters * 8 * 2048.0 / (out4[0] * 1e-3) / 1e12;
    (void)hipFree(dummy);
    (void)hipEventDestroy(e0);
    (void)hipEventDestroy(e1);
    return 0;
}

__global__ void k_cu_map(unsigned* __restrict__ out, int spin_ticks) {
    if (threadIdx.x == 0) {
        out[2 * blockIdx.x] = __builtin_amdgcn_s_getreg((31 << 11) | (0 << 6) | 4);
        out[2 * blockIdx.x + 1] = __builtin_amdgcn_s_getreg((3 << 11) | (0 << 6) | 20);
    }
    const long long t0 = wall_clock64();
    while (wall_clock64() - t0 < spin_ticks) __builtin_amdgcn_s_sleep(8);
}

extern "C" int mi355gp_dbg_cu_map(int device, int nwg, int mask_bit, unsigned* out) {
    HIP_CHECK(hipSetDevice(device));
    unsigned* d = nullptr;
    HIP_CHECK(hipMalloc(&d, sizeof(unsigned) * 2 * nwg));
    hipStream_t st = nullptr;
    if (mask_bit >= 0) {
        hipDeviceProp_t prop;
        HIP_CHECK(hipGetDeviceProperties(&prop, device));
        const int ncu = prop.multiProcessorCount;
        std::vector<uint32_t> mask((size_t)(ncu + 31) / 32, 0u);
        mask[mask_bit / 32] |= 1u << (mask_bit % 32);
        HIP_CHECK(hipExtStreamCreateWithCUMask(&st, (uint32_t)mask.size(), mask.data()));
    } else {
        HIP_CHECK(hipStreamCreate(&st));
    }
    hipLaunchKernelGGL(k_cu_map, dim3((unsigned)nwg), dim3(64), 0, st, d, 2000 );
    HIP_CHECK(hipStreamSynchronize(st));
    HIP_CHECK(hipMemcpy(out, d, sizeof(unsigned) * 2 * nwg, hipMemcpyDeviceToHost));
    (void)hipFree(d);
    (void)hipStreamDestroy(st);
    return 0;
}
```

include/mi355gp.h:

```cpp
#ifndef MI355GP_H
#define MI355GP_H

#include <stdint.h>

#ifdef __cplusplus
extern "C" {
#endif

typedef struct mi355gp_ctx mi355gp_ctx;

enum { MI355GP_RBF = 0, MI355GP_MATERN52 = 1, MI355GP_MATERN32 = 2, MI355GP_EXPONENTIAL = 3,
       MI355GP_WHITE = 4, MI355GP_BIAS = 5 ,
       MI355GP_RATQUAD = 6, MI355GP_STDPERIODIC = 7, MI355GP_COREGIONALIZE = 8, MI355GP_LINEAR = 9,
       MI355GP_MLP = 10, MI355GP_POLY = 11 };





typedef struct {
    int kind;
    int ard;
    int n_active;
    const int* active_dims;
    const double* theta;
    int term;
} mi355gp_part;

enum {
    MI355GP_FETCH_L = 0,
    MI355GP_FETCH_KINV = 1,
    MI355GP_FETCH_DLDK = 2,
    MI355GP_FETCH_K = 3
};

enum {
    MI355GP_OUT_LML = 0,
    MI355GP_OUT_LOGDET = 1,
    MI355GP_OUT_DATAFIT = 2,
    MI355GP_OUT_DNOISE = 3,
    MI355GP_OUT_TRKINV = 4,
    MI355GP_NUM_OUT = 8
};

enum {
    MI355GP_T_KBUILD = 0, MI355GP_T_POTRF = 1, MI355GP_T_TRTRI = 2, MI355GP_T_LAUUM = 3,
    MI355GP_T_SOLVE = 4, MI355GP_T_GRAD = 5, MI355GP_T_TOTAL = 6, MI355GP_NUM_T = 8
};

const char* mi355gp_last_error(void);
const char* mi355gp_version(void);
int mi355gp_device_count(int* count);
int mi355gp_device_synchronize(int device);

int mi355gp_create(int device, mi355gp_ctx** ctx);
int mi355gp_destroy(mi355gp_ctx* ctx);

int mi355gp_set_data(mi355gp_ctx* ctx, const double* X, int64_t N, int D, const double* R, int Dy);
int mi355gp_set_targets(mi355gp_ctx* ctx, const double* R, int Dy);

int mi355gp_kern_K(int device, int kind, int ard, const double* theta, const double* X, int64_t N,
                   const double* X2, int64_t M, int D, double* K_out);
int mi355gp_kern_Kdiag(int kind, const double* theta, int64_t N, double* out);
int mi355gp_update_gradients_full(int device, int kind, int ard, const double* theta, const double* dL_dK,
                                  const double* X, int64_t N, const double* X2, int64_t M, int D,
                                  double* dtheta_out);

int mi355gp_gradients_X(int device, int kind, int ard, const double* theta, const double* dL_dK, const double* X,
                        int64_t N, const double* X2, int64_t M, int D, double* out);

int mi355gp_exact_inference(mi355gp_ctx* ctx, int kind, int ard, const double* theta,
                            const double* noise, int64_t noise_len, double jitter, double extra_jitter,
                            double* out_scalars, double* alpha_out, double* dtheta_out,
                            double* diag_dLdK_out, double* stage_ms);

int mi355gp_exact_inference_sum(mi355gp_ctx* ctx, int nparts, const mi355gp_part* parts, const double* noise,
                                int64_t noise_len, double jitter, double extra_jitter, double* out_scalars,
                                double* alpha_out, double* dtheta_out, double* diag_dLdK_out, double* stage_ms);

int mi355gp_exact_studentt_sum(mi355gp_ctx* ctx, int nparts, const mi355gp_part* parts, double nu, double jitter,
                               double extra_jitter, double* out_scalars, double* alpha_out, double* dtheta_out,
                               double* stage_ms);

int mi355gp_inference_given_K(mi355gp_ctx* ctx, const double* K_host, const double* noise, int64_t noise_len,
                              double jitter, double extra_jitter, double* out_scalars, double* alpha_out,
                              double* diag_dLdK_out, double* stage_ms);

int mi355gp_fetch(mi355gp_ctx* ctx, int which, double* out, int fortran_order);

int mi355gp_predict(mi355gp_ctx* ctx, int kind, int ard, const double* theta, const double* Xnew, int64_t M,
                    double* mu_out, double* var_out, int full_cov);

int mi355gp_predict_sum(mi355gp_ctx* ctx, int nparts, const mi355gp_part* parts, const double* Xnew, int64_t M,
                        double* mu_out, double* var_out, int full_cov);

int mi355gp_predictive_gradients_sum(mi355gp_ctx* ctx, int nparts, const mi355gp_part* parts, const double* Xnew, int64_t M,
                                     double* dmu_out, double* dvar_out);

int mi355gp_laplace_begin(mi355gp_ctx* ctx, int nparts, const mi355gp_part* parts);
int mi355gp_laplace_newton(mi355gp_ctx* ctx, const double* W, const double* b, double extra_jitter, double* a_out,
                           double* Ka_out, double* logdet_out);
int mi355gp_laplace_finish(mi355gp_ctx* ctx, const double* W, double extra_jitter, double* diagKiWi_out, double* logdet_out);
int mi355gp_laplace_gradients(mi355gp_ctx* ctx, const double* Ki_f, const double* dL_dfhat, double* dtheta_out);
int mi355gp_laplace_implicit(mi355gp_ctx* ctx, const double* dL_dfhat, double* s_out);
int mi355gp_laplace_predict(mi355gp_ctx* ctx, int nparts, const mi355gp_part* parts, const double* Xnew, int64_t M,
                            const double* wv, double* mu_out, double* var_out, int full_cov);

enum { MI355GP_EP_BERNOULLI_PROBIT = 0 };
int mi355gp_ep_recompute(mi355gp_ctx* ctx, const double* tau, const double* v, double extra_jitter, double add_diag,
                         int want_sigma, double* mu_out, double* sigdiag_out, double* logdet_out, double* ms_out);
int mi355gp_ep_sweep(mi355gp_ctx* ctx, int lik, const int64_t* order, const double* ysign, double eta, double delta, double* tau,
                     double* v, double* cav_tau_out, double* cav_v_out, double* logZhat_out, double* mu_out, double* sigdiag_out,
                     double* ms_out);

int mi355gp_covariance_between_points(mi355gp_ctx* ctx, int nparts, const mi355gp_part* parts, const double* X1,
                                      int64_t M1, const double* X2, int64_t M2, double* out);

int mi355gp_potrf(int device, double* A, int64_t N, double* ms);
int mi355gp_pdinv(int device, const double* A, int64_t N, double* Ainv, double* L_out, double* logdet, double* ms);
int mi355gp_pdinv_full(int device, const double* A, int64_t N, double* Ainv, double* L_out, double* Li_out, double* logdet,
                       double* ms);

enum { MI355GP_OPT_PROFILE = 0, MI355GP_OPT_LOOKAHEAD = 1, MI355GP_OPT_TRI_OVERLAP = 2, MI355GP_OPT_TRI_MIN_NT = 3,
       MI355GP_OPT_TRI_H = 4, MI355GP_OPT_TRI_WGS = 5, MI355GP_OPT_TRI_HALF = 6, MI355GP_OPT_PART1_ON_PANEL = 7,
       MI355GP_OPT_NBO = 8, MI355GP_OPT_SOLVE_OVERLAP = 9, MI355GP_OPT_DIAG_EXCL_FIRST = 10, MI355GP_OPT_GRAPH = 11,
       MI355GP_OPT_PERSIST = 12, MI355GP_OPT_AGG2 = 13, MI355GP_OPT_PERSIST_TEST = 14, MI355GP_OPT_PERSIST_ABORTS = 15,
       MI355GP_OPT_PERSIST_SKIP = 16, MI355GP_OPT_PERSIST_SCHED = 17, MI355GP_OPT_NUM = 18 };
int mi355gp_set_option(mi355gp_ctx* ctx, int option, int value);
int mi355gp_get_option(mi355gp_ctx* ctx, int option, int* value);
enum { MI355GP_PF_UPDATE = 0 , MI355GP_PF_TRTRI = 1, MI355GP_PF_LAUUM = 2,
       MI355GP_PF_DIAG = 3 , MI355GP_PF_TRSM = 4 ,
       MI355GP_PF_UPDATE64 = 5 ,
       MI355GP_PF_PERSIST = 6 ,
       MI355GP_PF_TRTRI_EARLY = 7 ,
       MI355GP_PF_NUM = 8 };
int mi355gp_get_profile(mi355gp_ctx* ctx, double* ms, double* flops, int* launches);

typedef struct mi355gp_grid mi355gp_grid;
int mi355gp_grid_unique_id(void* id128);
int mi355gp_grid_create(int device, int rank, int world, int Pr, int Pc, int nb, const void* id128, mi355gp_grid** out);
int mi355gp_grid_destroy(mi355gp_grid* g);
int mi355gp_grid_set_data(mi355gp_grid* g, const double* X, int64_t N, int D, const double* R, int Dy);
int mi355gp_grid_exact_inference(mi355gp_grid* g, int kind, int ard, const double* theta, const double* noise,
                                 int64_t noise_len, double jitter, double extra_jitter, double* out_scalars,
                                 double* alpha_out, double* dtheta_out, double* diag_dLdK_out, double* stage_ms);
#define MI355GP_FETCH_LINV 100
int mi355gp_grid_fetch(mi355gp_grid* g, int which, double* out);
enum { MI355GP_GRID_OPT_LOOKAHEAD = 0, MI355GP_GRID_OPT_G = 1, MI355GP_GRID_OPT_GW = 2, MI355GP_GRID_OPT_CHECK_SEQ = 3,
       MI355GP_GRID_OPT_NUM = 4 };
int mi355gp_grid_set_option(mi355gp_grid* g, int option, int value);
int mi355gp_grid_get_option(mi355gp_grid* g, int option, int* value);
int mi355gp_grid_coll_log(mi355gp_grid* g, int rank, double* out9);
typedef struct mi355gp_sparse mi355gp_sparse;
int mi355gp_sparse_create(int device, mi355gp_sparse** out);
int mi355gp_sparse_destroy(mi355gp_sparse* s);
int mi355gp_sparse_set_data(mi355gp_sparse* s, const double* X, int64_t N, int D, const double* Y, int Dy);
int mi355gp_vardtc_inference(mi355gp_sparse* s, int kind, int ard, const double* theta, const double* Z, int64_t M,
                             double noise_var, double extra_jitter, double* out_scalars, double* dtheta_out,
                             double* dZ_out, double* wv_out, double* stage_ms);
int mi355gp_vardtc_inference_sum(mi355gp_sparse* s, int nparts, const mi355gp_part* parts, const double* Z, int64_t M,
                                 const double* noise, int64_t noise_len, double extra_jitter, double* out_scalars,
                                 double* dtheta_out, double* dZ_out, double* wv_out, double* dnoise_rows_out,
                                 double* dLdm_out, double* stage_ms);
int mi355gp_sparse_set_input_variance(mi355gp_sparse* s, const double* S, int64_t N, int D);
int mi355gp_vardtc_inference_uncertain(mi355gp_sparse* s, int nparts, const mi355gp_part* parts, const double* Z, int64_t M,
                                       const double* noise, int64_t noise_len, double extra_jitter, double* out_scalars,
                                       double* dtheta_out, double* dZ_out, double* wv_out, double* dmu_out, double* dS_out,
                                       double* stage_ms);
int mi355gp_sparse_predict(mi355gp_sparse* s, int nparts, const mi355gp_part* parts, const double* Xnew, int64_t Mn,
                           double* mu_out, double* var_out, int full_cov);
int mi355gp_sparse_fetch_dLdKnm(mi355gp_sparse* s, int64_t row0, int64_t nrows, double* out);
int mi355gp_sparse_attach_comm(mi355gp_sparse* s, int rank, int world, const void* id128);
int mi355gp_sparse_attach_loopback(mi355gp_sparse* s, int rank, int world, int group_key);
int mi355gp_sparse_fetch(mi355gp_sparse* s, int which, double* out);
int mi355gp_sparse_get_profile(mi355gp_sparse* s, double* out6);

int mi355gp_rbf_psi(int device, double variance, const double* lengthscale, int ard, const double* Z, int64_t M,
                    const double* mu, const double* S, int64_t N, int D, const double* weights, double* psi1_out,
                    double* psi2_out);
int mi355gp_rbf_psi_grad(int device, double variance, const double* lengthscale, int ard, const double* Z, int64_t M,
                         const double* mu, const double* S, int64_t N, int D, const double* weights, const double* dL_dpsi0,
                         const double* dL_dpsi1, const double* dL_dpsi2, double* dvar_out, double* dl_out, double* dZ_out,
                         double* dmu_out, double* dS_out);

#ifdef __cplusplus
}
#endif
#endif
```

include/mi355gp_debug.h:

```cpp
#ifndef MI355GP_DEBUG_H
#define MI355GP_DEBUG_H
#include "mi355gp.h"
#ifdef __cplusplus
extern "C" {
#endif

int mi355gp_bench_factor(int device, int64_t N, int reps, double* ms_potrf, double* ms_trtri, double* ms_lauum);

int mi355gp_dbg_ipc_selftest(const void* id128, int rank, int world, int Pr, int Pc, int64_t count, double* out4);
int mi355gp_dbg_comm_selftest(int device, const void* id128, int rank, int world, int Pr, int Pc, int64_t count, int rounds,
                              double* out4);
int mi355gp_dbg_grid_multi(int device, int T, int nb, int reps, double* out_ms4);
int mi355gp_dbg_update_nt(int device, int nt, const int* ks, int nk, int reps, double* out_ms);
int mi355gp_dbg_update_rect(int device, int ntr, int ntc, const int* ks, int nk, int reps, double* out_ms);

int mi355gp_dbg_mfma(int device, const double* a, const double* b, double* d);
int mi355gp_dbg_gemm(int device, int a_mcontig, int b_ncontig, int64_t M, int64_t N, int64_t K,
                     const double* A, const double* B, double* C, double alpha, double beta, int reps, double* ms);
int mi355gp_dbg_peaks(int device, double* out8);
int mi355gp_dbg_gemm_clock(double* mhz, double* cycles);
int mi355gp_dbg_cu_map(int device, int nwg, int mask_bit, unsigned* out);
int mi355gp_dbg_pipe_share(int device, double* out4);
int mi355gp_dbg_graph_factor(int device, int64_t N, int reps, double* out3);
int mi355gp_dbg_persist(int device, int64_t N, int reps, int kcap, double* out);
int mi355gp_dbg_lauum_plan(int nt, int* items, int max_items, int* out4);
int mi355gp_dbg_persist_owners(int nt, int nw, int tune, int* owner, int* out4);
int mi355gp_dbg_mask_probe(int device, int pct, int order, double* out3);

#ifdef __cplusplus
}
#endif
#endif
```

Baseline: 14.05 iters/s.

## Add single-stage LDS GEMM tile so LAUUM runs three workgroups per CU

Adds a new 128x128 f64 GEMM tile variant that keeps only one LDS stage (half the LDS footprint) and uses buffer-load-to-LDS with an in-slab refill. The LAUUM kernels, both the plain and split-item versions, are templated on workgroups-per-CU and default to the three-WG variant when the occupancy query confirms three can be resident. The aim is to hide latency through higher occupancy rather than multi-stage buffering, at the cost of more exposed load latency per workgroup. It also adds an option and debug hooks for the setting and extends the peak MFMA probe.

```diff
diff --git a/gpy_amd/_lib.py b/gpy_amd/_lib.py
--- a/gpy_amd/_lib.py
+++ b/gpy_amd/_lib.py
@@ -169,6 +169,10 @@
     L.mi355gp_dbg_mfma.argtypes = [ci, _dp, _dp, _dp]
     L.mi355gp_dbg_gemm.argtypes = [ci, ci, ci, i64, i64, i64, _dp, _dp, _dp, cd, cd, ci, _c_dp]
     L.mi355gp_dbg_peaks.argtypes = [ci, _dp]
+    L.mi355gp_set_tile_wgs_default.argtypes = [ci]
+    L.mi355gp_set_tile_wgs_default.restype = ci
+    L.mi355gp_dbg_tile_wgs_residency.argtypes = [ci, ctypes.POINTER(ci), ci]
+    L.mi355gp_dbg_tile_wgs_residency.restype = ci
     L.mi355gp_dbg_pipe_share.argtypes = [ci, _dp]
     L.mi355gp_dbg_graph_factor.argtypes = [ci, i64, ci, _dp]
     L.mi355gp_dbg_gemm_clock.argtypes = [_c_dp, _c_dp]
@@ -216,12 +220,12 @@
             "mi355gp_laplace_begin", "mi355gp_laplace_newton", "mi355gp_laplace_finish", "mi355gp_laplace_gradients",
             "mi355gp_laplace_implicit", "mi355gp_laplace_predict", "mi355gp_ep_recompute", "mi355gp_ep_sweep",
             "mi355gp_rbf_psi", "mi355gp_rbf_psi_grad", "mi355gp_sparse_set_input_variance",
-            "mi355gp_vardtc_inference_uncertain")
+            "mi355gp_vardtc_inference_uncertain", "mi355gp_set_tile_wgs_default", "mi355gp_dbg_tile_wgs_residency")
 
 
 OPTIONS = {"profile": 0, "lookahead": 1, "tri_overlap": 2, "tri_min_nt": 3, "tri_h": 4, "tri_wgs": 5, "tri_half": 6,
            "part1_on_panel": 7, "nbo": 8, "solve_overlap": 9, "diag_excl_first": 10, "graph": 11, "persist": 12, "agg2": 13,
-           "persist_test": 14, "persist_aborts": 15, "persist_skip": 16, "persist_sched": 17}
+           "persist_test": 14, "persist_aborts": 15, "persist_skip": 16, "persist_sched": 17, "tile_wgs": 18}
 
 
 def last_error():
@@ -782,11 +786,27 @@
 
 def dbg_peaks(device=0):
     require_device(device)
-    out = np.zeros(8)
+    out = np.zeros(10)
     check(lib().mi355gp_dbg_peaks(device, out), "dbg_peaks")
     return dict(mfma_f64_tflops=out[0], valu_f64_tflops=out[1], hbm_copy_gbs=out[2], hbm_fill_gbs=out[3],
                 mfma_cycles_per_inst_1wave=out[4], shader_mhz_under_load=out[5], mfma_1wave_tflops=out[6],
-                mfma_cycles_per_inst_loaded=out[7])
+                mfma_cycles_per_inst_loaded=out[7], mfma_2wave_tflops=out[8], mfma_3wave_tflops=out[9])
+
+
+def set_tile_wgs_default(value):
+    check(lib().mi355gp_set_tile_wgs_default(int(value)), "mi355gp_set_tile_wgs_default")
+
+
+TILE_WGS_KERNELS = ("k_lauum<4>", "k_lauum128_items")
+
+
+def dbg_tile_wgs_residency(device=0):
+    require_device(device)
+    out = (ctypes.c_int * 8)()
+    n = lib().mi355gp_dbg_tile_wgs_residency(device, out, 8)
+    if n < 0:
+        check(n, "mi355gp_dbg_tile_wgs_residency")
+    return {TILE_WGS_KERNELS[i]: int(out[i]) for i in range(n)}
 
 
 def dbg_grid_multi(T, nb=512, reps=3, device=0):
diff --git a/gpy_amd/csrc/api.hip b/gpy_amd/csrc/api.hip
--- a/gpy_amd/csrc/api.hip
+++ b/gpy_amd/csrc/api.hip
@@ -45,6 +45,7 @@
     set(MI355GP_OPT_DIAG_EXCL_FIRST, &w.diag_excl_first);
     set(MI355GP_OPT_PERSIST, &w.persist);
     set(MI355GP_OPT_AGG2, &w.agg2);
+    set(MI355GP_OPT_TILE_WGS, &w.tile_wgs);
     if (c->opt[MI355GP_OPT_GRAPH] != INT_MIN) c->graph_enabled = c->opt[MI355GP_OPT_GRAPH] ? 1 : 0;
 }
 
@@ -1105,6 +1106,10 @@
         mi355gp_set_error("mi355gp_set_option: NBO must be a multiple of %d", NB);
         return -1;
     }
+    if (option == MI355GP_OPT_TILE_WGS && value >= 0 && value != 2 && value != 3) {
+        mi355gp_set_error("mi355gp_set_option: TILE_WGS is 2 or 3 (-1: the process default)");
+        return -1;
+    }
     c->opt[option] = (value < 0) ? INT_MIN : value;
     if (value < 0) {
         FactorWs d;
@@ -1124,6 +1129,7 @@
             case MI355GP_OPT_PERSIST: c->ws.persist = penv("PERSIST", d.persist); break;
             case MI355GP_OPT_AGG2: c->ws.agg2 = env("AGG2", d.agg2) ? 1 : 0; break;
             case MI355GP_OPT_GRAPH: c->graph_enabled = penv("GRAPH", 1) ? 1 : 0; break;
+            case MI355GP_OPT_TILE_WGS: c->ws.tile_wgs = tile_wgs_default(); break;
             default: break;
         }
 #undef env
@@ -1138,6 +1144,18 @@
     apply_options(c);
     drop_graph(c);
     return 0;
+}
+
+int mi355gp_set_tile_wgs_default(int value) {
+    ARG_CHECK(value == 2 || value == 3 || value == -1, "mi355gp_set_tile_wgs_default: 2, 3 or -1");
+    (void)tile_wgs_default(value);
+    return 0;
+}
+
+int mi355gp_dbg_tile_wgs_residency(int device, int* out, int cap) {
+    ARG_CHECK(out && cap >= 0, "mi355gp_dbg_tile_wgs_residency: bad arguments");
+    HIP_CHECK(hipSetDevice(device));
+    return tile_wgs_residency(out, cap);
 }
 
 int mi355gp_get_option(mi355gp_ctx* c, int option, int* value) {
@@ -1146,7 +1164,7 @@
     const int v[MI355GP_OPT_NUM] = {0, w.lookahead, w.tri_overlap, w.tri_min_nt, w.tri_h_override, w.tri_wgs, w.tri_half_ok,
                                     w.part1_on_panel, w.nbo_override, w.solve_overlap, w.diag_excl_first, c->graph_enabled,
                                     w.persist, w.agg2, w.persist_test, w.persist_aborts, w.persist_skip,
-                                    w.sched_state == 2 ? ((w.persist_auto_off || !w.persist) ? 2 : 1) : 0};
+                                    w.sched_state == 2 ? ((w.persist_auto_off || !w.persist) ? 2 : 1) : 0, w.tile_wgs};
     *value = v[option];
     return 0;
 }
diff --git a/gpy_amd/csrc/common.h b/gpy_amd/csrc/common.h
--- a/gpy_amd/csrc/common.h
+++ b/gpy_amd/csrc/common.h
@@ -19,6 +19,7 @@
 #define GEMM_DEFAULT_TRI64_MAX 512
 #define GEMM_DEFAULT_LAUUM64_MAX 528
 #define LAUUM_SPLIT_MAX_NT 44
+#define GEMM_DEFAULT_TILE_WGS 3
 #define GEMM_DEFAULT_UPD64_MAX 128
 
 __device__ __forceinline__ d4 mfma_f64(double a, double b, d4 c) {
diff --git a/gpy_amd/csrc/factor.hip b/gpy_amd/csrc/factor.hip
--- a/gpy_amd/csrc/factor.hip
+++ b/gpy_amd/csrc/factor.hip
@@ -139,6 +139,11 @@
         HIP_CHECK(hipMalloc(&ws->tri_counter, sizeof(int) * 4));
         const char* envh = DIAG_ENV("TRI_H");
         if (envh && *envh) ws->tri_h_override = atoi(envh);
+    }
+    ws->tile_wgs = tile_wgs_default();
+    {
+        int res[8];
+        (void)tile_wgs_residency(res, 8);
     }
     const char* envp1 = DIAG_ENV("PART1_ON_PANEL");
     if (envp1 && *envp1) ws->part1_on_panel = atoi(envp1) ? 1 : 0;
@@ -521,8 +526,8 @@
     if (split && ws->lauum_plan_nt == nt)
         launch_lauum_split(st, X, W, npad, nt, (const LauumItem*)ws->lauum_plan_dev, ws->lauum_nitems,
                            (const LauumSum*)((const char*)ws->lauum_plan_dev + sizeof(LauumItem) * ws->lauum_nitems), ws->lauum_nsums,
-                           ws->lauum_part);
+                           ws->lauum_part, ws->tile_wgs);
     else
-        launch_lauum(st, X, W, npad, nt);
+        launch_lauum(st, X, W, npad, nt, ws->tile_wgs);
     ws->prof.end(st);
 }
diff --git a/gpy_amd/csrc/gemm.hip b/gpy_amd/csrc/gemm.hip
--- a/gpy_amd/csrc/gemm.hip
+++ b/gpy_amd/csrc/gemm.hip
@@ -16,6 +16,27 @@
 #include <vector>
 #define env_int(name, dflt) diag_env_int(DIAG_ENV(name), dflt)
 #define LB(NW) __launch_bounds__((NW) * 64, (NW) / 2)
+#define LBW(WGS) __launch_bounds__(256, WGS)
+
+static int g_tile_wgs_default = GEMM_DEFAULT_TILE_WGS;
+int tile_wgs_default(int set) {
+    if (set == 2 || set == 3) g_tile_wgs_default = set;
+    else if (set == -1) g_tile_wgs_default = GEMM_DEFAULT_TILE_WGS;
+    return g_tile_wgs_default;
+}
+static int resident_wgs(const void* kernel) {
+    int n = 0;
+    if (hipOccupancyMaxActiveBlocksPerMultiprocessor(&n, kernel, 256, GT1_LDS_BYTES) != hipSuccess) {
+        (void)hipGetLastError();
+        n = 0;
+    }
+    return n;
+}
+#define TILE_WGS3_OK(kernel)                                                    \
+    ([]() -> int {                                                              \
+        static const int n = resident_wgs(reinterpret_cast<const void*>(kernel)); \
+        return n;                                                               \
+    }())
 
 template <int NW, bool PRE>
 __global__ LB(NW) void k_update_nt(double* __restrict__ C, long ldc,
@@ -271,8 +292,8 @@
     launch_trtri_level_t<4>(st, nblocks, L, X, T, ld, nt, nbt, stages);
 }
 
-template <int NW>
-__global__ LB(NW) void k_lauum(const double* __restrict__ X, double* __restrict__ W, long ld, int nt) {
+template <int NW, int WGS = 2>
+__global__ LBW(WGS) void k_lauum(const double* __restrict__ X, double* __restrict__ W, long ld, int nt) {
     extern __shared__ __attribute__((aligned(16))) double smem[];
     const int bid = blockIdx.x;
     int ti = (int)((sqrtf(8.0f * (float)bid + 1.0f) - 1.0f) * 0.5f);
@@ -282,8 +303,8 @@
     d4 acc[4][GTCfg<NW>::NI];
     gt_zero<NW>(acc);
     const int K = (nt - ti) * NB;
-    gemm_tile_128<false, false, NW>(X + (long)ti * NB * ld + (long)ti * NB, ld, X + (long)ti * NB * ld + (long)tj * NB, ld,
-                                K, acc, smem);
+    gemm_tile_128<false, false, NW, false, WGS>(X + (long)ti * NB * ld + (long)ti * NB, ld,
+                                                X + (long)ti * NB * ld + (long)tj * NB, ld, K, acc, smem);
     gt_store<0, NW>(W + (long)ti * NB * ld + (long)tj * NB, ld, acc);
 }
 
@@ -349,14 +370,15 @@
     else gt64_store<0>(part + (long)it.part * 4096, 64, acc);
 }
 
-__global__ LB(4) void k_lauum128_items(const double* __restrict__ X, double* __restrict__ W, long ld,
-                                       const LauumItem* __restrict__ items, double* __restrict__ part) {
+template <int WGS>
+__global__ LBW(WGS) void k_lauum128_items(const double* __restrict__ X, double* __restrict__ W, long ld,
+                                          const LauumItem* __restrict__ items, double* __restrict__ part) {
     extern __shared__ __attribute__((aligned(16))) double smem[];
     const LauumItem it = items[blockIdx.x];
     d4 acc[4][GTCfg<4>::NI];
     gt_zero<4>(acc);
     const long r0 = (long)it.ti * NB, c0 = (long)it.tj * NB;
-    gemm_tile_128<false, false, 4>(X + (long)it.k0 * ld + r0, ld, X + (long)it.k0 * ld + c0, ld, it.klen, acc, smem);
+    gemm_tile_128<false, false, 4, false, WGS>(X + (long)it.k0 * ld + r0, ld, X + (long)it.k0 * ld + c0, ld, it.klen, acc, smem);
     if (it.part < 0) gt_store<0, 4>(W + r0 * ld + c0, ld, acc);
     else gt_store<0, 4>(part + (long)it.part * (NB * NB), NB, acc);
 }
@@ -409,10 +431,14 @@
 }
 
 void launch_lauum_split(hipStream_t st, const double* X, double* W, long ld, int nt, const LauumItem* items_dev, int nitems,
-                        const LauumSum* sums_dev, int nsums, double* part) {
+                        const LauumSum* sums_dev, int nsums, double* part, int wgs) {
     if (lauum_split_tile(nt) == 128) {
-        LDS_OPT_IN(k_lauum128_items);
-        hipLaunchKernelGGL(k_lauum128_items, dim3((unsigned)nitems), dim3(256), GT_LDS_BYTES, st, X, W, ld, items_dev, part);
+        if (wgs == 3 && TILE_WGS3_OK(k_lauum128_items<3>) >= 3) {
+            hipLaunchKernelGGL(k_lauum128_items<3>, dim3((unsigned)nitems), dim3(256), GT1_LDS_BYTES, st, X, W, ld, items_dev, part);
+        } else {
+            LDS_OPT_IN(k_lauum128_items<2>);
+            hipLaunchKernelGGL(k_lauum128_items<2>, dim3((unsigned)nitems), dim3(256), GT_LDS_BYTES, st, X, W, ld, items_dev, part);
+        }
         if (nsums > 0) hipLaunchKernelGGL(k_lauum128_reduce, dim3((unsigned)nsums), dim3(256), 0, st, W, ld, sums_dev, part);
         return;
     }
@@ -431,14 +457,25 @@
     return (long)nt * (nt + 1) / 2 <= lauum64_max;
 }
 
-void launch_lauum(hipStream_t st, const double* X, double* W, long ld, int nt) {
+void launch_lauum(hipStream_t st, const double* X, double* W, long ld, int nt, int wgs) {
     const long nblocks = (long)nt * (nt + 1) / 2;
     static const int lauum64_max = env_int("LAUUM64_MAX", GEMM_DEFAULT_LAUUM64_MAX);
     if (nblocks <= lauum64_max) {
         hipLaunchKernelGGL(k_lauum64, dim3((unsigned)(4 * nblocks)), dim3(256), GT64_LDS_BYTES, st, X, W, ld, nt);
         return;
     }
+    if (wgs == 3 && TILE_WGS3_OK((k_lauum<4, 3>)) >= 3) {
+        hipLaunchKernelGGL((k_lauum<4, 3>), dim3((unsigned)nblocks), dim3(256), GT1_LDS_BYTES, st, X, W, ld, nt);
+        return;
+    }
     launch_lauum_t<4>(st, nblocks, X, W, ld, nt);
+}
+
+int tile_wgs_residency(int* out, int cap) {
+    const int v[] = {TILE_WGS3_OK((k_lauum<4, 3>)), TILE_WGS3_OK(k_lauum128_items<3>)};
+    const int n = (int)(sizeof(v) / sizeof(v[0]));
+    for (int i = 0; i < n && i < cap; ++i) out[i] = v[i];
+    return n;
 }
 
 template <int NW>
diff --git a/gpy_amd/csrc/gemm_tile.h b/gpy_amd/csrc/gemm_tile.h
--- a/gpy_amd/csrc/gemm_tile.h
+++ b/gpy_amd/csrc/gemm_tile.h
@@ -1,4 +1,6 @@
 #pragma once
+#include <type_traits>
+
 #include "common.h"
 
 #define GT_LDS_BYTES 73728
@@ -15,12 +17,17 @@
 template <bool AK, bool BK, bool NEGA = false>
 __device__ __forceinline__ void gemm_tile_128_v3(const double* __restrict__ A, long lda, const double* __restrict__ B,
                                                  long ldb, int K, d4 (&acc)[4][4], double* smem);
-
-template <bool AK, bool BK, int NW, bool NEGA = false>
+template <bool AK, bool BK, bool NEGA = false>
+__device__ __forceinline__ void gemm_tile_128_s1(const double* __restrict__ A, long lda, const double* __restrict__ B,
+                                                 long ldb, int K, d4 (&acc)[4][4], double* smem);
+
+template <bool AK, bool BK, int NW, bool NEGA = false, int WGS = 2>
 __device__ __forceinline__ void gemm_tile_128(const double* __restrict__ A, long lda,
                                               const double* __restrict__ B, long ldb, int K,
                                               d4 (&acc)[4][GTCfg<NW>::NI], double* smem) {
-    gemm_tile_128_v3<AK, BK, NEGA>(A, lda, B, ldb, K, acc, smem);
+    static_assert(WGS == 2 || WGS == 3, "two or three workgroups per CU");
+    if (WGS == 3) gemm_tile_128_s1<AK, BK, NEGA>(A, lda, B, ldb, K, acc, smem);
+    else gemm_tile_128_v3<AK, BK, NEGA>(A, lda, B, ldb, K, acc, smem);
 }
 
 template <int NW>
@@ -187,6 +194,110 @@
     }
 }
 
+
+#define GT1_LDS_BYTES (2 * GT3_OP * 8)
+
+template <bool KC>
+__device__ __forceinline__ void gt1_src_offsets(long ld, int lane, int w, int (&vl)[2], int (&so)[4]) {
+    if (KC) {
+#pragma unroll
+        for (int p = 0; p < 2; ++p) {
+            const int row = 8 * p + (lane >> 3), g = (lane & 7) ^ gt3_h(row);
+            vl[p] = (int)((row * ld + 2 * g) * 8);
+        }
+#pragma unroll
+        for (int ii = 0; ii < 4; ++ii) so[ii] = (int)((32 * w + 8 * (ii & ~1)) * ld * 8);
+    } else {
+        vl[0] = vl[1] = 2 * lane * 8;
+#pragma unroll
+        for (int ii = 0; ii < 4; ++ii) so[ii] = (int)((4 * w + ii) * ld * 8);
+    }
+}
+
+template <bool KC>
+__device__ __forceinline__ void gt1_issue(__amdgpu_buffer_rsrc_t rs, const int (&vl)[2], const int (&so)[4], double* sdst, int w) {
+#pragma unroll
+    for (int ii = 0; ii < 4; ++ii) {
+        const int i = 4 * w + ii;
+        double* d = KC ? sdst + i * 128 : sdst + i * GT3_SMN;
+        __builtin_amdgcn_raw_ptr_buffer_load_lds(rs, d, 16, vl[ii & 1], so[ii], 0, 0);
+    }
+}
+
+template <bool AK, bool BK, bool NEGA>
+__device__ __forceinline__ void gemm_tile_128_s1(const double* __restrict__ A, long lda,
+                                                 const double* __restrict__ B, long ldb, int K, d4 (&acc)[4][4],
+                                                 double* smem) {
+    const int t = threadIdx.x, lane = t & 63, w = __builtin_amdgcn_readfirstlane(t >> 6), wr = w >> 1, wc = w & 1;
+    const int nk = K / 16;
+    const int arow = wr * 64 + (lane & 15), bcol = wc * 64 + (lane & 15), kq = lane >> 4;
+    auto rsrc = [](const double* p) {
+        return __builtin_amdgcn_make_buffer_rsrc(const_cast<double*>(p), 0, 0x7fffffff, 0x00020000);
+    };
+    int va[2], vb[2], oa[4], ob[4];
+    gt1_src_offsets<AK>(lda, lane, w, va, oa);
+    gt1_src_offsets<BK>(ldb, lane, w, vb, ob);
+    const long sa = AK ? 16 : 16 * lda, sb = BK ? 16 : 16 * ldb;
+    int fa0[4], fb0[4];
+#pragma unroll
+    for (int mi = 0; mi < 4; ++mi) {
+        const int r = arow + mi * 16, c = bcol + mi * 16;
+        fa0[mi] = AK ? r * 16 : r;
+        fb0[mi] = BK ? c * 16 : c;
+    }
+    const int ha = gt3_h(arow), hb = gt3_h(bcol);
+    double* a_w = smem;
+    double* b_w = smem + GT3_OP;
+    const double* a_s = a_w;
+    const double* b_s = b_w;
+    auto frags = [&](int e, d2 (&af)[4], d2 (&bf)[4]) __attribute__((always_inline)) {
+#pragma unroll
+        for (int mi = 0; mi < 4; ++mi) {
+            if (AK) af[mi] = *reinterpret_cast<const d2*>(a_s + fa0[mi] + 2 * ((2 * kq + e) ^ ha));
+            else af[mi] = (d2){a_s[(4 * kq + 2 * e) * GT3_SMN + fa0[mi]], a_s[(4 * kq + 2 * e + 1) * GT3_SMN + fa0[mi]]};
+        }
+#pragma unroll
+        for (int ni = 0; ni < 4; ++ni) {
+            if (BK) bf[ni] = *reinterpret_cast<const d2*>(b_s + fb0[ni] + 2 * ((2 * kq + e) ^ hb));
+            else bf[ni] = (d2){b_s[(4 * kq + 2 * e) * GT3_SMN + fb0[ni]], b_s[(4 * kq + 2 * e + 1) * GT3_SMN + fb0[ni]]};
+        }
+    };
+    auto mfmas = [&](const d2 (&af)[4], const d2 (&bf)[4]) __attribute__((always_inline)) {
+#pragma unroll
+        for (int s = 0; s < 2; ++s)
+#pragma unroll
+            for (int mi = 0; mi < 4; ++mi)
+#pragma unroll
+                for (int ni = 0; ni < 4; ++ni)
+                    acc[mi][ni] = mfma_f64(NEGA ? -af[mi][s] : af[mi][s], bf[ni][s], acc[mi][ni]);
+    };
+    gt1_issue<AK>(rsrc(A), va, oa, a_w, w);
+    gt1_issue<BK>(rsrc(B), vb, ob, b_w, w);
+    __builtin_amdgcn_s_waitcnt(0x0F70);
+    __syncthreads();
+    auto slab = [&](auto refill, const double* An, const double* Bn) __attribute__((always_inline)) {
+        d2 af[4], bf[4], ag[4], bg[4];
+        frags(0, af, bf);
+        mfmas(af, bf);
+        __builtin_amdgcn_sched_barrier(0);
+        frags(1, ag, bg);
+        __builtin_amdgcn_s_waitcnt(0xC07F);
+        __syncthreads();
+        if (decltype(refill)::value) {
+            gt1_issue<AK>(rsrc(An), va, oa, a_w, w);
+            gt1_issue<BK>(rsrc(Bn), vb, ob, b_w, w);
+        }
+        __builtin_amdgcn_sched_barrier(0);
+        mfmas(ag, bg);
+        __builtin_amdgcn_sched_barrier(0);
+        __builtin_amdgcn_s_waitcnt(0x0F70);
+        __syncthreads();
+    };
+    for (int kt = 1; kt <= nk; ++kt) {
+        const int kn = kt < nk ? kt : nk - 1;
+        slab(std::true_type{}, A + kn * sa, B + kn * sb);
+    }
+}
 
 template <bool AK, bool BK, bool NEGA>
 __device__ __forceinline__ void gemm_tile_128_v3_multi(const double* const* __restrict__ Atab, long aoff, long lda,
diff --git a/gpy_amd/csrc/internal.h b/gpy_amd/csrc/internal.h
--- a/gpy_amd/csrc/internal.h
+++ b/gpy_amd/csrc/internal.h
@@ -13,13 +13,15 @@
                       int K, int ntr, int ntc, int row0t, int col0t);
 void launch_trtri_level(hipStream_t st, const double* L, double* X, double* T, long ld, int nt, int level,
                         int stages = 3);
-void launch_lauum(hipStream_t st, const double* X, double* W, long ld, int nt);
+void launch_lauum(hipStream_t st, const double* X, double* W, long ld, int nt, int wgs = 2);
+int tile_wgs_default(int set = -2);
+int tile_wgs_residency(int* out, int cap);
 struct LauumItem { int ti, tj, q, k0, klen, part; };
 struct LauumSum { int ti, tj, q, first, n; };
 void lauum_split_plan(int nt, std::vector<LauumItem>& items, std::vector<LauumSum>& sums, int* nparts);
 int lauum_split_tile(int nt);
 void launch_lauum_split(hipStream_t st, const double* X, double* W, long ld, int nt, const LauumItem* items_dev, int nitems,
-                        const LauumSum* sums_dev, int nsums, double* part);
+                        const LauumSum* sums_dev, int nsums, double* part, int wgs = 2);
 bool lauum_uses_64(int nt);
 void launch_trmm_lower(hipStream_t st, const double* X, long ldx, const double* B, long ldb, double* Out, long ldo,
                        int ntr, int ntc);
@@ -80,6 +82,7 @@
     int upd_queue_probe = 0;
     UpdTask* upd_tasks = nullptr;
     int part1_on_panel = 1;
+    int tile_wgs = 2;
     int lookahead = 1;
     int nbo_override = 0;
     long nbo_for(long npad) const {
diff --git a/gpy_amd/csrc/peaks.hip b/gpy_amd/csrc/peaks.hip
--- a/gpy_amd/csrc/peaks.hip
+++ b/gpy_amd/csrc/peaks.hip
@@ -57,8 +57,8 @@
     float ms;
     long long h[2];
     const int iters = 20000;
-    for (int pass = 0; pass < 2; ++pass) {
-        const int blocks = pass == 0 ? 256 : 256 * 8;
+    for (int pass = 0; pass < 4; ++pass) {
+        const int blocks = pass == 0 ? 256 : pass == 1 ? 256 * 8 : 256 * pass;
         hipLaunchKernelGGL(k_peak_mfma, dim3(blocks), dim3(256), 0, 0, dummy, dclk, 200, 0.5);
         HIP_CHECK(hipEventRecord(e0, 0));
         hipLaunchKernelGGL(k_peak_mfma, dim3(blocks), dim3(256), 0, 0, dummy, dclk, iters, 0.5);
@@ -70,6 +70,8 @@
         if (pass == 0) {
             out8[4] = (double)h[0] / ((double)iters * 8);
             out8[6] = tf;
+        } else if (pass >= 2) {
+            out8[6 + pass] = tf;
         } else {
             out8[0] = tf;
             out8[5] = (double)h[0] / (double)h[1] * 100.0;
diff --git a/include/mi355gp.h b/include/mi355gp.h
--- a/include/mi355gp.h
+++ b/include/mi355gp.h
@@ -125,8 +125,9 @@
        MI355GP_OPT_TRI_H = 4, MI355GP_OPT_TRI_WGS = 5, MI355GP_OPT_TRI_HALF = 6, MI355GP_OPT_PART1_ON_PANEL = 7,
        MI355GP_OPT_NBO = 8, MI355GP_OPT_SOLVE_OVERLAP = 9, MI355GP_OPT_DIAG_EXCL_FIRST = 10, MI355GP_OPT_GRAPH = 11,
        MI355GP_OPT_PERSIST = 12, MI355GP_OPT_AGG2 = 13, MI355GP_OPT_PERSIST_TEST = 14, MI355GP_OPT_PERSIST_ABORTS = 15,
-       MI355GP_OPT_PERSIST_SKIP = 16, MI355GP_OPT_PERSIST_SCHED = 17, MI355GP_OPT_NUM = 18 };
+       MI355GP_OPT_PERSIST_SKIP = 16, MI355GP_OPT_PERSIST_SCHED = 17, MI355GP_OPT_TILE_WGS = 18, MI355GP_OPT_NUM = 19 };
 int mi355gp_set_option(mi355gp_ctx* ctx, int option, int value);
+int mi355gp_set_tile_wgs_default(int value);
 int mi355gp_get_option(mi355gp_ctx* ctx, int option, int* value);
 enum { MI355GP_PF_UPDATE = 0 , MI355GP_PF_TRTRI = 1, MI355GP_PF_LAUUM = 2,
        MI355GP_PF_DIAG = 3 , MI355GP_PF_TRSM = 4 ,
diff --git a/include/mi355gp_debug.h b/include/mi355gp_debug.h
--- a/include/mi355gp_debug.h
+++ b/include/mi355gp_debug.h
@@ -18,6 +18,7 @@
 int mi355gp_dbg_gemm(int device, int a_mcontig, int b_ncontig, int64_t M, int64_t N, int64_t K,
                      const double* A, const double* B, double* C, double alpha, double beta, int reps, double* ms);
 int mi355gp_dbg_peaks(int device, double* out8);
+int mi355gp_dbg_tile_wgs_residency(int device, int* out, int cap);
 int mi355gp_dbg_gemm_clock(double* mhz, double* cycles);
 int mi355gp_dbg_cu_map(int device, int nwg, int mask_bit, unsigned* out);
 int mi355gp_dbg_pipe_share(int device, double* out4);
```

Result: no change. 14.15 iters/s (median of 6 runs) (+0.7%).
